# plai-group/latent-flexible-video-diffusion-modeling

Hardware: AMD Instinct MI355X
Metric: denoising steps/sec on 20-frame 4x16x16 latents (sampling; training reported alongside) (higher is better)
Workload: dtype f32

## Files before the change

include/lfvdm_hip.h:

```cpp
#ifndef LFVDM_HIP_H
#define LFVDM_HIP_H

#include <stddef.h>
#include <stdint.h>

#ifdef __cplusplus
extern "C" {
#endif

#define LFVDM_OK 0
#define LFVDM_E_SHAPE 1
#define LFVDM_E_LAUNCH 2
#define LFVDM_E_UNSUPPORTED 3

#define LFVDM_ACT_NONE 0
#define LFVDM_ACT_SILU 1

#define LFVDM_OUT_ROWS 0
#define LFVDM_OUT_NCHW 1

int lfvdm_abi_version(void);

typedef struct lfvdm_conv_args {
    const float* src0;
    const float* src1;
    int32_t C0, C1;
    int32_t N;
    int32_t Hs, Ws;
    int32_t up;
    int32_t stride;
    int32_t ksize;
    int32_t Ho, Wo;
    const float* coefA;
    const float* coefB;
    int32_t act;
    const float* W;
    const float* bias;
    int32_t Cout;
    const float* s2src0;
    const float* s2src1;
    int32_t s2C0, s2C1;
    const float* W2;
    const float* bias2;
    const float* res;
    int32_t ldr;
    const float* resA;
    const float* resB;
    float* out;
    int32_t ldo;
    int32_t out_mode;
    int32_t tune;
    float* splitk_ws;
    int32_t* splitk_cnt;
    int64_t splitk_ws_floats;
    int64_t splitk_cnt_ints;
    const float* gn_gamma;
    const float* gn_beta;
    const float* gn_film;
    float* gn_out;
    int32_t gn_film_ld;
    int32_t gn_film_div;
    int32_t gn_act;
    int32_t gn_skip_raw;
    float gn_eps;
    int32_t gn_general;
    int32_t gn_gw;
    int32_t gn_ld;
} lfvdm_conv_args;

int lfvdm_conv_igemm(const lfvdm_conv_args* a, void* stream);
int lfvdm_conv_igemm_config(const lfvdm_conv_args* a, int* nt, int* nwaves);
int lfvdm_conv_igemm_candidates(const lfvdm_conv_args* a, int* codes, int max_codes);

typedef struct lfvdm_wgrad_job {
    lfvdm_conv_args a;
    int32_t msplit;
    int32_t task0;
} lfvdm_wgrad_job;
int lfvdm_conv_wgrad_grouped(const lfvdm_wgrad_job* jobs_dev, int njobs, int total_tasks, void* stream);

int lfvdm_pack_conv_weight(const float* w_oihw, float* w_packed, int Cout, int Cin, int ksize, void* stream);
int lfvdm_pack_conv_weight_up2x(const float* w_oihw, float* w_packed, int Cout, int Cin, void* stream);

int lfvdm_conv_wgrad(const lfvdm_conv_args* a, void* stream);

int lfvdm_det_reduce(float* dst, const float* slab, long n, long parts, void* stream);
int lfvdm_pack_conv_weight_t(const float* w_oihw, float* w_packed_t, int Cout, int Cin, int ksize, void* stream);
int lfvdm_unpack_conv_grad(const float* g_packed, float* g_oihw, int Cout, int Cin, int ksize, int accumulate, void* stream);

typedef struct lfvdm_pack_job {
    const float* src;
    float* dst;
    int32_t Cout, Cin, taps, transposed, blk0;
    int32_t ld;
} lfvdm_pack_job;
int lfvdm_pack_conv_weights(const lfvdm_pack_job* jobs_dev, int njobs, int total_blocks, void* stream);

typedef struct lfvdm_unpack_job {
    float* gp;
    float* g;
    int32_t Cout, Cin, taps, row0;
    int32_t ldp;
    int32_t pad_;
} lfvdm_unpack_job;
int lfvdm_unpack_conv_grads(const lfvdm_unpack_job* jobs_dev, int njobs, int total_rows, int max_row_floats, void* stream);

int lfvdm_conv_in(const float* x, const float* x0, const float* obs, const float* w, const float* bias,
                  float* out, int N, int C, int H, int W, int Cout, void* stream);
int lfvdm_conv_in_tick(const float* x, const float* x0, const float* obs, const float* w, const float* bias, float* out,
                       int N, int C, int H, int W, int Cout, int64_t* t, const float* model_timestep_table, float* model_t,
                       int B, const float* rows_all, int rows_ld, float* rows, int row_floats, void* stream);

int lfvdm_gn_coef(const float* src0, const float* src1, int C0, int C1, int N, int P,
                  const float* gamma, const float* beta, const float* film, int film_div, int film_ld,
                  float eps, float* coefA, float* coefB, void* stream);

int lfvdm_gn_apply(const float* src0, const float* src1, int C0, int C1, int N, int P,
                   const float* gamma, const float* beta, const float* film, int film_div, int film_ld,
                   float eps, int act, float* out, float* coefA, float* coefB, float* stats, void* stream);
int lfvdm_gn_apply_part(const float* src, int C, int N, int P, int cg, const float* gamma, const float* beta, float eps, int act,
                        float* out, int ldo, void* stream);
long lfvdm_gn_apply_ws_floats(int C, int N, int P);
int lfvdm_gn_apply_ws(const float* src0, const float* src1, int C0, int C1, int N, int P, const float* gamma,
                      const float* beta, const float* film, int film_div, int film_ld, float eps, int act, float* out,
                      float* coefA, float* coefB, float* stats, float* ws, long ws_floats, void* stream);

int lfvdm_gn_coef_stats(const float* src0, const float* src1, int C0, int C1, int N, int P,
                        const float* gamma, const float* beta, const float* film, int film_div, int film_ld,
                        float eps, float* coefA, float* coefB, float* stats, void* stream);

int lfvdm_gn_bwd_stats(const float* da, const float* src0, const float* src1, int C0, int C1, int N, int P,
                       const float* coefA, const float* coefB, const float* stats, int act, float* sums, void* stream);
int lfvdm_gn_bwd_apply(const float* da, const float* src0, const float* src1, int C0, int C1, int N, int P,
                       const float* coefA, const float* coefB, const float* stats, const float* sums, int act,
                       float* out0, float* out1, int acc0, int acc1, void* stream);
int lfvdm_gn_bwd_apply_params(const float* da, const float* src0, const float* src1, int C0, int C1, int N, int P,
                              const float* coefA, const float* coefB, const float* stats, const float* sums, int act,
                              float* out0, float* out1, int acc0, int acc1, const float* gamma, const float* beta,
                              const float* film, int film_ld, int T, float* dgamma, float* dbeta, float* dfilm,
                              int dfilm_ld, const float* add, int add_ld, void* stream);
typedef struct lfvdm_gn_bwd_args {
    const float* da;
    const float* src0;
    const float* src1;
    const float* coefA;
    const float* coefB;
    const float* stats;
    float* out0;
    float* out1;
    const float* add;
    const float* add2;
    const float* gamma;
    const float* beta;
    const float* film;
    float* dgamma;
    float* dbeta;
    float* dfilm;
    float* sums_out;
    float* ws;
    int64_t ws_floats;
    int32_t C0, C1, N, P, act;
    int32_t add_ld, add2_ld, film_ld, T, dfilm_ld;
} lfvdm_gn_bwd_args;
long lfvdm_gn_bwd_ws_floats(int C, int N, int P);
int lfvdm_gn_bwd(const lfvdm_gn_bwd_args* a, void* stream);
int lfvdm_gn_param_grads(const float* sums, const float* gamma, const float* beta, const float* film, int film_ld, int T,
                         float* dgamma, float* dbeta, float* dfilm, int dfilm_ld, int N, int C, void* stream);
int lfvdm_gn_temporal_bwd(const float* x, const float* dy, const float* gamma, float eps, float* dx, float* dgamma,
                          float* dbeta, int B, int T, int P, int C, int accumulate, void* stream);
int lfvdm_gn_temporal_bwd_det(const float* x, const float* dy, const float* gamma, float eps, float* dx, float* dgamma,
                              float* dbeta, int B, int T, int P, int C, int accumulate, float* det_ws, int64_t det_ws_floats,
                              void* stream);

int lfvdm_gn_temporal(const float* x, const float* gamma, const float* beta, float eps, float* y,
                      int B, int T, int P, int C, void* stream);

int lfvdm_gn_temporal_qkv_ok(int B, int T, int P, int C);
int lfvdm_gn_temporal_qkv(const float* x, const float* gamma, const float* beta, float eps, float* xn_out,
                          const float* Wqkv, const float* bqkv, float* qkv, int B, int T, int P, int C, void* stream);

int lfvdm_proj_gn_ok(int N, int P, int C);
int lfvdm_proj_gn(const float* o, const float* W, const float* bias, const float* res, const float* gamma, const float* beta,
                  float eps, int act, float* out, float* raw_out, int N, int P, int C, void* stream);

typedef struct lfvdm_rowdot_job {
    const float* W;
    const float* b;
    const float* in;
    float* out;
    int32_t K, O, M, ldin, ldout, in_mode;
    int32_t row0;
    int32_t pad_;
} lfvdm_rowdot_job;

int lfvdm_rowdot(const lfvdm_rowdot_job* jobs_dev, int njobs, int total_rows, void* stream);
int lfvdm_silu(const float* in, float* out, int64_t n, void* stream);

typedef struct lfvdm_rowdot_bwd_job {
    const float* W;
    const float* in;
    const float* dout;
    float* dW;
    float* db;
    float* din;
    int32_t K, O, M, ldin, lddout, lddin, in_mode, task0;
} lfvdm_rowdot_bwd_job;
int lfvdm_rowdot_bwd(const lfvdm_rowdot_bwd_job* jobs_dev, int njobs, int total_tasks, void* stream);
int lfvdm_rowdot_bwd_det(const lfvdm_rowdot_bwd_job* jobs_dev, int njobs, int total_tasks, float* din_base, int64_t din_n,
                         float* det_ws, int64_t det_ws_floats, void* stream);

typedef struct lfvdm_rpe_job {
    const float* tproj;
    const float* Wd;
    const float* bd;
    const float* Wout;
    const float* bout;
    float* R;
    int32_t C;
    int32_t tile0;
    int32_t tproj_ld;
    int32_t pad_;
    float* act;
} lfvdm_rpe_job;

int lfvdm_rpe_nets(const lfvdm_rpe_job* jobs_dev, int njobs, int total_tiles, const int64_t* frame_indices_i64,
                   int B, int T, void* stream);
int lfvdm_rpe_nets_maxc(const lfvdm_rpe_job* jobs_dev, int njobs, int total_tiles, const int64_t* frame_indices_i64,
                        int B, int T, int max_channels, void* stream);

typedef struct lfvdm_rpe_bwd_job {
    const float* tproj;
    const float* Wd;
    const float* bd;
    const float* Wout_t;
    const float* dR;
    float* dtproj;
    float* dWd;
    float* dbd;
    int32_t C;
    int32_t tile0;
    int32_t tproj_ld;
    int32_t dtproj_ld;
} lfvdm_rpe_bwd_job;

int lfvdm_rpe_nets_bwd(const lfvdm_rpe_bwd_job* jobs_dev, int njobs, int total_tiles, const int64_t* frame_indices_i64,
                       int B, int T, void* stream);
int lfvdm_rpe_nets_bwd_det(const lfvdm_rpe_bwd_job* jobs_dev, int njobs, int total_tiles, const int64_t* frame_indices_i64,
                           int B, int T, float* det_ws, int64_t det_ws_floats, void* stream);

int lfvdm_rpe_front(const float* tproj, int tproj_ld, const float* feats, const float* Wd, const float* bd, float* act, int B,
                    int rows_per_b, int C, void* stream);
int lfvdm_rpe_front_bwd(const float* tproj, int tproj_ld, const float* feats, const float* Wd, const float* bd,
                        const float* d_act, float* dtproj, int dtproj_ld, float* dWd, float* dbd, int B, int rows_per_b,
                        int C, void* stream);

int lfvdm_attn_spatial(const float* qkv, float* o, float* attn_out, float* lse_out, int N, int P, int C, int heads,
                       void* stream);

int lfvdm_attn_spatial_fused_ok(int N, int P, int C, int heads);
int lfvdm_attn_spatial_fused(const float* xn, const float* Wqkv, const float* bqkv, float* o, int N, int P, int C, int heads,
                             void* stream);

int lfvdm_attn_spatial_bwd(const float* qkv, const float* o, const float* d_o, const float* lse, float* delta_ws,
                           float* dqkv, int N, int P, int C, int heads, void* stream);

int lfvdm_attn_temporal(const float* qkv, const float* Rq, const float* Rk, const float* Rv,
                        const float* mask , float* o, float* attn_out,
                        int B, int T, int P, int C, int heads, void* stream);
int lfvdm_attn_temporal_sel(const float* qkv, const float* Rq, const float* Rk, const float* Rv, const float* mask,
                            float* o, float* attn_out, int B, int T, int P, int C, int heads, const int64_t* rsel,
                            void* stream);
int lfvdm_attn_temporal_ring(const float* qkv, const float* Rq, const float* Rk, const float* Rv, const float* mask,
                             float* o, float* attn_out, int B, int T, int P, int C, int heads, const int64_t* rsel,
                             int ring, void* stream);

int lfvdm_attn_temporal_bwd(const float* qkv, const float* d_o, const float* Rq, const float* Rk, const float* Rv,
                            const float* mask, float* ws_p, float* ws_ds, float* dqkv, float* dRq, float* dRk,
                            float* dRv, int B, int T, int P, int C, int heads, void* stream);

int lfvdm_q_sample(const float* x0, const float* noise, const int64_t* t, const float* sqrt_acp,
                   const float* sqrt_1macp, float* out, int B, int inner, void* stream);
#define LFVDM_RULE_ANCESTRAL 0
#define LFVDM_RULE_DDIM 1
#define LFVDM_MEAN_EPS 0
#define LFVDM_MEAN_X0 1
int lfvdm_update_x0(const float* x, const float* model_out, const float* noise, const int64_t* t, const float* sqrt_recip_acp,
                    const float* sqrt_recipm1_acp, const float* c1, const float* c2, const float* sg, int rule, int mean_type,
                    int clip, float* sample, float* pred_xstart, float* mean_out, int B, int inner, void* stream);
int lfvdm_update_rng_x0(const float* x, const float* model_out, float* noise_out, const int64_t* t, const float* sqrt_recip_acp,
                        const float* sqrt_recipm1_acp, const float* c1, const float* c2, const float* sg, int rule,
                        int mean_type, int clip, float* sample, float* pred_xstart, float* mean_out, int B, int inner,
                        const int64_t* seed, void* stream);
int lfvdm_conv_out_psample_ok(int N, int H, int W, int C, int Cout);
int lfvdm_conv_out_update_x0(const float* act, const float* Wp, const float* bias, float* out, const float* x,
                             const float* noise_in, float* noise_out, const int64_t* t, const float* sqrt_recip_acp,
                             const float* sqrt_recipm1_acp, const float* c1, const float* c2, const float* sg, int rule,
                             int mean_type, int clip, float* sample, float* pred_xstart, float* mean_out, int B, int T, int H,
                             int W, int C, int Cout, const int64_t* seed, void* stream);
int lfvdm_update_ms_x0(const float* x, const float* model_out, const float* hist, const int64_t* t, const float* sqrt_recip_acp,
                       const float* sqrt_recipm1_acp, const float* k1, const float* k2, const float* k3, int mean_type, int clip,
                       float* sample, float* pred_xstart, int B, int inner, void* stream);
int lfvdm_conv_out_update_ms_x0(const float* act, const float* Wp, const float* bias, float* out, const float* x,
                                const float* hist, const int64_t* t, const float* sqrt_recip_acp, const float* sqrt_recipm1_acp,
                                const float* k1, const float* k2, const float* k3, int mean_type, int clip, float* sample,
                                float* pred_xstart, int B, int T, int H, int W, int C, int Cout, void* stream);
int lfvdm_known_blend(float* x, const float* known, const float* mask, const float* eps, float* noise_out, const int64_t* t,
                      const float* sqrt_acp_prev, const float* sqrt_1macp_prev, const int64_t* seed, int B, int T, int C,
                      int HW, void* stream);
int lfvdm_renoise(float* x, float* noise_out, const int64_t* t, const float* sqrt_1mbeta, const float* sqrt_beta,
                  const int64_t* seed, int B, int inner, void* stream);
int lfvdm_dyn_threshold_workspace(int B, int64_t inner, size_t* bytes);
int lfvdm_dyn_threshold(const float* x, const float* model_out, const int64_t* t, const float* sqrt_recip_acp,
                        const float* sqrt_recipm1_acp, int mean_type, int x0hat_fma, const float* frame_mask, int B, int T,
                        int64_t frame_inner, double percentile, float max_value, float* xhat, float* stats, void* workspace,
                        void* stream);
int lfvdm_noise_prior_factor(const int64_t* frame_indices, double a, double c, double rho, float* L_out, int B, int T,
                             void* stream);
int lfvdm_noise_prior_fill(const float* L, const float* xi, const int64_t* seed, const int64_t* t, float* out, int B, int T,
                           int64_t E, void* stream);
int lfvdm_sampler_tick(int64_t* t, const float* model_timestep_table, float* model_t, int B, void* stream);
int lfvdm_sampler_tick_fetch(int64_t* t, const float* model_timestep_table, float* model_t, int B, const float* rows_all,
                             int rows_ld, float* rows, int row_floats, void* stream);
int lfvdm_masked_mse(const float* a, const float* b, const float* mask, float* out, int B, int T,
                     int frame_inner, void* stream);
int lfvdm_masked_mse_bwd(const float* target, const float* pred, const float* mask, const float* g, float* dpred, int B, int T,
                         int frame_inner, void* stream);

int lfvdm_train_loss(const float* target, const float* pred, const float* mask, const float* eval_mask, const int64_t* t,
                     const float* wtab, int n_t, float* mse, float* eval_mse, float* loss, int B, int T, int frame_inner,
                     void* stream);
int lfvdm_train_loss_bwd(const float* target, const float* pred, const float* mask, const int64_t* t, const float* wtab, int n_t,
                         const float* g, float* dpred, int B, int T, int frame_inner, void* stream);

int lfvdm_vb_terms(const float* x_start, const float* x_t, const float* model_out, const float* noise, const int64_t* t,
                   const float* sqrt_recip_acp, const float* sqrt_recipm1_acp, const float* c1, const float* c2,
                   const float* post_log_var, const float* model_log_var, const float* mask, int mean_type, int clip, float* vb,
                   float* xstart_mse, float* eps_mse, float* pred_xstart, int B, int T, int frame_inner, int out_ld,
                   int col_base, void* stream);
int lfvdm_vb_terms_bwd(const float* x_start, const float* x_t, const float* model_out, const int64_t* t,
                       const float* sqrt_recip_acp, const float* sqrt_recipm1_acp, const float* c1, const float* c2,
                       const float* model_log_var, const float* mask, const float* g, int mean_type, int clip, float* d_out,
                       int B, int T, int frame_inner, void* stream);

#define LFVDM_PIX_F32 0
#define LFVDM_PIX_U8 1
int lfvdm_frame_metrics(const void* pred, const void* truth, int dtype, float scale, float shift, int K, int N, int C, int H,
                        int W, float* mse, float* ssim, float* partials, long partials_floats, void* stream);
long lfvdm_frame_metrics_workspace(int K, int N, int C, int H, int W);

int lfvdm_frame_dist_rows(const float* x, int B, int T, int C, int H, int W, int L, const int32_t* new_idx, int n_new,
                          const int32_t* cand_idx, int n_cand, float* dist, void* stream);
int lfvdm_fps_select(const float* dist, int B, int T, const int32_t* cand_idx, int n_cand, const int32_t* forced_pos, int n_forced,
                     int n, int32_t* picks, void* stream);

typedef struct lfvdm_adamw_args {
    float* p;
    const float* g;
    float* m;
    float* v;
    float* ema[4];
    float ema_rate[4];
    int32_t n_ema;
    int64_t n;
    float lr, beta1, beta2, eps, weight_decay;
    float bias_corr1, bias_corr2_sqrt;
    float grad_scale;
    float* grad_sqsum;
    const int32_t* skip_flag;
    const int32_t* skip_flag2;
} lfvdm_adamw_args;

int lfvdm_adamw_ema(const lfvdm_adamw_args* a, void* stream);

#define LFVDM_GRAD_NORM_MAX_PARTS 512
int lfvdm_grad_norm_nparts(int64_t n);
int lfvdm_grad_norm_partials(const float* g, int64_t n, float grad_scale, float* partials, int nparts, void* stream);
int lfvdm_grad_norm_finalize(const float* partials, int nparts, float max_norm, float* stat, void* stream);
int lfvdm_adamw_ema_clip(const lfvdm_adamw_args* a, const float* stat, void* stream);

int lfvdm_prepare_batch(const float* pool, const int32_t* table, float* batch, int64_t* frame_indices, float* obs_mask,
                        float* latent_mask, int B, int F, int Tp, int frame_elems, void* stream);

#define LFVDM_WAVELET_RANGE 0
#define LFVDM_WAVELET_ORTHONORMAL 1
int lfvdm_wavelet_encode(const void* pix, int dtype, float scale, float shift, float* coef, const float* mean,
                         const float* rstd, int N, int C, int H, int W, int levels, int norm, void* stream);
int lfvdm_wavelet_decode(const float* coef, const float* mean, const float* std, void* pix, int dtype, int N, int C, int H,
                         int W, int levels, int norm, void* stream);
int lfvdm_prepare_batch_wavelet(const void* pool, int dtype, float scale, float shift, const int32_t* table, float* batch,
                                int64_t* frame_indices, float* obs_mask, float* latent_mask, const float* mean,
                                const float* rstd, int B, int F, int Tp, int C, int H, int W, int levels, int norm,
                                void* stream);

int lfvdm_shapes_trajectories(const int64_t* video_idx, int32_t* traj, int32_t* consts, uint64_t seed, int split, int n_videos,
                              int T, int n_shapes, int H, int W, int stochastic, void* stream);
int lfvdm_shapes_render(const int32_t* traj, const int32_t* consts, const int32_t* table, const float* lut, void* out, int dtype,
                        int64_t* frame_indices, float* obs_mask, float* latent_mask, int B, int F, int Tp, int T, int n_shapes,
                        int H, int W, void* stream);

#define LFVDM_SLOT_PAD 0
#define LFVDM_SLOT_OBS 1
#define LFVDM_SLOT_LATENT 2
int lfvdm_search_assemble(const float* pool, const int32_t* table, const int32_t* role, float* x0, float* x_start,
                          float* obs_mask, float* latent_mask, float* mask, int64_t* frame_indices, int W, int K, int V, int Tv,
                          int frame_elems, void* stream);
int lfvdm_search_noise_qsample(const float* x_start, const int32_t* table, const int64_t* t_list, int32_t* ctl,
                               const int64_t* key, const float* sqrt_acp, const float* sqrt_1macp, float* noise, float* x_t,
                               int64_t* t_buf, int W, int K, int V, int frame_elems, void* stream);
int lfvdm_search_noise_fill(const int32_t* table, uint64_t seed, int step, int j, float* noise, int W, int K, int V,
                            int frame_elems, void* stream);
int lfvdm_search_scores(const float* terms, const int64_t* t_list, float* scores, int G, int V, int n_t, int ld, int col_base,
                        void* stream);

int lfvdm_compose_rows(const float* x, const float* x0, const float* obs, float* rows, int N, int Cx, int H, int W, int ld,
                       void* stream);

#define LFVDM_CHAIN_CONV 0
#define LFVDM_CHAIN_GN 1
#define LFVDM_CHAIN_LOCAL 2
#define LFVDM_CHAIN_MAX_DEPS 64
#define LFVDM_CHAIN_CTL_EPOCH 0
#define LFVDM_CHAIN_CTL_EXIT 32
#define LFVDM_CHAIN_CTL_ABORT 64
#define LFVDM_CHAIN_CTL_INTS 96

typedef struct lfvdm_gn_args {
    const float* src0;
    const float* src1;
    int32_t C0, C1, N, P;
    const float* gamma;
    const float* beta;
    const float* film;
    int32_t film_div, film_ld;
    float eps;
    int32_t act;
    float* out;
    int32_t cg;
    int32_t ldo;
    float* out_base;
    int32_t out_col;
    int32_t pad_;
} lfvdm_gn_args;

typedef struct lfvdm_chain_stage {
    int32_t kind;
    int32_t n_items;
    int32_t flag_base;
    int32_t n_flags;
    int32_t dep_base;
    int32_t dep_stride;
    int32_t cfg;
    int32_t kz;
    int32_t nt2;
    int32_t wg_off;
    int32_t side;
    int32_t wg_lo;
    int32_t wg_count;
    int64_t ws_off;
    int64_t cnt_off;
    lfvdm_conv_args conv;
    lfvdm_gn_args gn;
} lfvdm_chain_stage;

int lfvdm_chain_plan(lfvdm_chain_stage* stages, int n_stages, int32_t* deps, int64_t deps_cap, int64_t* deps_used,
                     int32_t* n_flags, int64_t* ws_floats, int64_t* cnt_ints, int32_t* grid, int32_t* lds_bytes);
int lfvdm_chain_conv_ok(const lfvdm_conv_args* a);
int lfvdm_chain_gn_ok(int C0, int C1, int N, int P);
int lfvdm_chain_local_ok(const lfvdm_conv_args* a, int row_tiles);
int lfvdm_chain_capacity(int lds_bytes);
int lfvdm_level_chain(const lfvdm_chain_stage* stages_dev, int n_stages, const int32_t* deps_dev, int32_t* flags, int32_t* ctl,
                      int grid, int lds_bytes, double timeout_s, void* stream);

int lfvdm_flag_add(int32_t* flag, void* stream);
int lfvdm_flag_wait(const int32_t* flag, int32_t target, double timeout_s, int32_t* timed_out, void* stream);
int lfvdm_flag_wait2(const int32_t* flag, int32_t target, double timeout_s, int32_t* timed_out, float* timed_out_f32, void* stream);

#ifdef __cplusplus
}
#endif
#endif
```

latent-flexible-video-diffusion-modeling_amd/csrc/attention_temporal.h:

```cpp
#pragma once
#include "common_hip.h"

constexpr int TEMPORAL_MAXT = 32;
constexpr int TEMPORAL_MAXT_LONG = 64;

struct TemporalFwd {
    const float *qkv, *Rq, *Rk, *Rv, *mask;
    float *o, *attn_out;
    int B, T, P, C, heads;
    RSel rsel;
    hipStream_t s;
};
struct TemporalBwd {
    const float *qkv, *d_o, *Rq, *Rk, *Rv, *mask;
    float *ws_p, *ws_ds, *dqkv;
    int B, T, P, C, heads;
    hipStream_t s;
};

int lfvdm_attn_temporal2_try(const TemporalFwd& a);
int lfvdm_attn_temporal2_bwd_rows_try(const TemporalBwd& a);
int lfvdm_attn_temporal_long(const TemporalFwd& a);
int lfvdm_attn_temporal_long_bwd(const TemporalBwd& a);
```

latent-flexible-video-diffusion-modeling_amd/csrc/attention_temporal2.hip:

```cpp
#include "attention_temporal.h"
#include "common_hip.h"

namespace {

struct T2Geom {
    int T, P, C, heads, B;
    int TG, TGN, PPW, NW;
    int strips;
    int NL, HL, XPG;
};

template <int F, int TCAP>
struct T2Cfg {
    static constexpr int NQ = F / 4;
    static constexpr int RS = (TCAP * NQ + 15) / 16 * 16;
};

__device__ __forceinline__ void t2_decode(const T2Geom& g, int& b, int& h, int& tg, int& strip) {
    {
        const int id = blockIdx.x;
        if (g.XPG > 0) {
            const int x = id & 7, r = id >> 3;
            const int grp = x % g.NL, sub = x / g.NL;
            const int inner = r % (g.HL * g.TG), sblk = r / (g.HL * g.TG);
            strip = sblk * g.XPG + sub;
            const int hl = inner % g.HL;
            tg = inner / g.HL;
            const int hpb = g.heads / g.HL;
            b = grp / hpb;
            h = (grp % hpb) * g.HL + hl;
        } else {
            const int NP = g.B * g.heads;
            const int pair = id % NP, rest = id / NP;
            b = pair / g.heads;
            h = pair % g.heads;
            tg = rest % g.TG;
            strip = rest / g.TG;
        }
    }
}

template <int F, int TCAP>
__device__ __forceinline__ void t2_stage(const float* __restrict__ qkv, const float* __restrict__ Rq, const float* __restrict__ Rk,
                                         const float* __restrict__ Rv, RSel rsel, const T2Geom& g, int b, int h,
                                         int tq0, int p0, int wave, int lane, float* Rimg, float* KVimg) {
    using CF = T2Cfg<F, TCAP>;
    constexpr int NQ = CF::NQ, RS = CF::RS;
    const int T = g.T, P = g.P, C = g.C;
    const int NPX = g.NW * g.PPW;
    const float invRS = 1.0f / (float)RS;
    {
        const size_t rb = rsel.slice(b, g.B);
        const float* Rsrc[3] = {Rk + rb * T * T * C + h * F, Rq + rb * T * T * C + h * F, Rv + rb * T * T * C + h * F};
        const float* kvsrc = qkv + (size_t)b * T * P * 3 * C + C + h * F;
        const int vpx = min(NPX, P - p0);
        const int nR = (min(g.TGN, T - tq0) * 3 * RS + 63) >> 6, nKV = (vpx * 2 * RS + 63) >> 6;
        const int TNQ = T * NQ;
        auto dma = [](const float* src, float* dst) {
            __builtin_amdgcn_global_load_lds((const __attribute__((address_space(1))) void*)src,
                                             (__attribute__((address_space(3))) void*)dst, 16, 0, 0);
        };
        for (int pc = wave; pc < nR; pc += g.NW) {
            const int ps = pc * 64 + lane;
            const int row3 = (int)(((float)ps + 0.5f) * invRS);
            const int w = ps - row3 * RS;
            const int tq = (int)(((float)row3 + 0.5f) * (1.0f / 3.0f)), arr = row3 - 3 * tq;
            const int c = w ^ (tq & 15);
            const int s = c / NQ, u = c - s * NQ;
            const int t = tq0 + tq;
            const bool ok = tq < g.TGN && t < T && c < TNQ;
            const int row = arr == 1 ? s * T + t : t * T + s;
            const float* base = arr == 0 ? Rsrc[0] : (arr == 1 ? Rsrc[1] : Rsrc[2]);
            dma(ok ? base + (size_t)row * C + 4 * u : qkv, Rimg + (size_t)pc * 256);
        }
        for (int pc = wave; pc < nKV; pc += g.NW) {
            const int ps = pc * 64 + lane;
            const int row2 = (int)(((float)ps + 0.5f) * invRS);
            const int w = ps - row2 * RS;
            const int jw = row2 >> 1, arr = row2 & 1;
            const int c = w ^ (jw & 15);
            const int s = c / NQ, u = c - s * NQ;
            const int p = p0 + jw;
            const bool ok = jw < NPX && p < P && c < TNQ;
            dma(ok ? kvsrc + ((size_t)s * P + p) * 3 * C + arr * C + 4 * u : qkv, KVimg + (size_t)pc * 256);
        }
    }

}

template <int F, int TCAP>
__global__ __launch_bounds__(256, 3)
void attn_temporal2_kernel(const float* __restrict__ qkv, const float* __restrict__ Rq, const float* __restrict__ Rk,
                           const float* __restrict__ Rv, const float* __restrict__ mask, float* __restrict__ o,
                           float* __restrict__ attn_out, RSel rsel, T2Geom g) {
    using CF = T2Cfg<F, TCAP>;
    constexpr int NQ = CF::NQ, RS = CF::RS;
    extern __shared__ __attribute__((aligned(16))) float t2_smem[];
    const int T = g.T, P = g.P, C = g.C;
    const int tid = threadIdx.x, lane = tid & 63;
    const int wave = __builtin_amdgcn_readfirstlane(tid >> 6);
    const int NPX = g.NW * g.PPW;
    int b, h, tg, strip;
    t2_decode(g, b, h, tg, strip);
    if (strip >= g.strips) return;
    const int tq0 = tg * g.TGN;
    const int p0 = strip * NPX;
    float* Rimg = t2_smem;
    float* KVimg = t2_smem + (size_t)((g.TGN * 3 * RS + 63) & ~63) * 4;
    const float invRS = 1.0f / (float)RS;

    t2_stage<F, TCAP>(qkv, Rq, Rk, Rv, rsel, g, b, h, tq0, p0, wave, lane, Rimg, KVimg);

    const float invN = 1.0f / (float)g.TGN;
    const int sq = lane & 3, pair = lane >> 2;
    const int j = (int)(((float)pair + 0.5f) * invN), tq = pair - j * g.TGN;
    const int jw = wave * g.PPW + j;
    const int t = tq0 + tq, p = p0 + jw;
    const bool active = j < g.PPW && p < P && t < T;
    const float scale = rsqrtf((float)F);
    const size_t ld = (size_t)3 * C;
    const float* qrow = active ? qkv + ((size_t)(b * T + t) * P + p) * ld + h * F : qkv;
    f32x4 q4[NQ];
#pragma unroll
    for (int u = 0; u < NQ; ++u) q4[u] = ld4(qrow + 4 * u) * scale;
    constexpr int KQ = (TCAP + 3) / 4;
    constexpr int ISTRIDE = 4 * NQ * 4;
    int kb[NQ], rbs[NQ];
    {
        const int jr = active ? jw : 0, tr = active ? tq : 0;
#pragma unroll
        for (int u = 0; u < NQ; ++u) {
            const int low = (NQ * sq + u) & 15, high = (NQ * sq + u) & ~15;
            kb[u] = (jr * 2 * RS + high + (low ^ (jr & 15))) * 4;
            rbs[u] = (tr * 3 * RS + high + (low ^ (tr & 15))) * 4;
        }
    }
    asm volatile("s_waitcnt vmcnt(0)" ::: "memory");
    __syncthreads();

    auto quad_x1 = [](float v) { return __builtin_bit_cast(float, __builtin_amdgcn_mov_dpp(__builtin_bit_cast(int, v), 0xB1, 0xF, 0xF, true)); };
    auto quad_x2 = [](float v) { return __builtin_bit_cast(float, __builtin_amdgcn_mov_dpp(__builtin_bit_cast(int, v), 0x4E, 0xF, 0xF, true)); };

    {
        float logit[KQ];
#pragma unroll
        for (int i = 0; i < KQ; ++i) {
            f32x2 a0 = {0.f, 0.f}, a1 = {0.f, 0.f};
#pragma unroll
            for (int u = 0; u < NQ; ++u) {
                const f32x4 k4 = ld4(KVimg + kb[u] + i * ISTRIDE);
                const f32x4 r4 = ld4(Rimg + rbs[u] + i * ISTRIDE);
                const f32x4 g4 = ld4(Rimg + rbs[u] + RS * 4 + i * ISTRIDE);
                a0 = __builtin_elementwise_fma(q4[u].xy, k4.xy + r4.xy, a0);
                a0 = __builtin_elementwise_fma(q4[u].zw, k4.zw + r4.zw, a0);
                a1 = __builtin_elementwise_fma(k4.xy, g4.xy, a1);
                a1 = __builtin_elementwise_fma(k4.zw, g4.zw, a1);
            }
            logit[i] = (a0.x + a0.y) + (a1.x + a1.y) * scale;
            asm volatile("" : "+v"(logit[i]) : : "memory");
            __builtin_amdgcn_sched_barrier(0);
        }
        const int tm = active ? t : 0;
        const float mt = mask ? mask[b * T + tm] : 1.f;
        float mx = -INFINITY;
#pragma unroll
        for (int i = 0; i < KQ; ++i) {
            const int sk = sq + 4 * i;
            float v = -INFINITY;
            if (sk < T) {
                v = logit[i];
                if (mask) {
                    const float ms = mask[b * T + sk];
                    const float pen = 1.f - (mt * ms + (1.f - mt) * (1.f - ms));
                    v -= (pen == 1.f) ? INFINITY : pen;
                }
            }
            logit[i] = v;
            mx = fmaxf(mx, v);
        }
        mx = fmaxf(mx, quad_x1(mx));
        mx = fmaxf(mx, quad_x2(mx));
        float sum = 0.f;
#pragma unroll
        for (int i = 0; i < KQ; ++i) {
            const float e = (logit[i] == -INFINITY) ? 0.f : __expf(logit[i] - mx);
            logit[i] = e;
            sum += e;
        }
        sum += quad_x1(sum);
        sum += quad_x2(sum);
        const float inv = 1.0f / sum;
#pragma unroll
        for (int i = 0; i < KQ; ++i) logit[i] *= inv;
        if (attn_out && active) {
            float* ar = attn_out + ((((size_t)b * P + p) * g.heads + h) * T + t) * T;
#pragma unroll
            for (int i = 0; i < KQ; ++i)
                if (sq + 4 * i < T) ar[sq + 4 * i] = logit[i];
        }
        f32x4 acc[NQ];
#pragma unroll
        for (int u = 0; u < NQ; ++u) acc[u] = (f32x4){0.f, 0.f, 0.f, 0.f};
#pragma unroll
        for (int i = 0; i < KQ; ++i) {
            const f32x2 pr = {logit[i], logit[i]};
#pragma unroll
            for (int u = 0; u < NQ; ++u) {
                const f32x4 v4 = ld4(KVimg + kb[u] + RS * 4 + i * ISTRIDE);
                const f32x4 r4 = ld4(Rimg + rbs[u] + 2 * RS * 4 + i * ISTRIDE);
                f32x2 lo = acc[u].xy, hi = acc[u].zw;
                lo = __builtin_elementwise_fma(pr, v4.xy + r4.xy, lo);
                hi = __builtin_elementwise_fma(pr, v4.zw + r4.zw, hi);
                acc[u] = (f32x4){lo.x, lo.y, hi.x, hi.y};
                asm volatile("" : "+v"(acc[u]) : : "memory");
            }
            __builtin_amdgcn_sched_barrier(0);
        }
#pragma unroll
        for (int u = 0; u < NQ; ++u) {
#pragma unroll
            for (int e = 0; e < 4; ++e) {
                float v = acc[u][e];
                v += quad_x1(v);
                v += quad_x2(v);
                acc[u][e] = v;
            }
        }
        if (active) {
            float* orow = o + ((size_t)(b * T + t) * P + p) * C + h * F;
#pragma unroll
            for (int u = 0; u < NQ; ++u)
                if ((u & 3) == sq) st4(orow + 4 * u, acc[u]);
        }
    }
}

template <int F, int TCAP>
__global__ __launch_bounds__(256, 2)
void attn_temporal2_bwd_rows_kernel(const float* __restrict__ qkv, const float* __restrict__ dO, const float* __restrict__ Rq,
                                    const float* __restrict__ Rk, const float* __restrict__ Rv, const float* __restrict__ mask,
                                    float* __restrict__ dqkv, float* __restrict__ Pg, float* __restrict__ dSg, T2Geom g) {
    using CF = T2Cfg<F, TCAP>;
    constexpr int NQ = CF::NQ, RS = CF::RS;
    extern __shared__ __attribute__((aligned(16))) float t2_smem[];
    const int T = g.T, P = g.P, C = g.C;
    const int tid = threadIdx.x, lane = tid & 63;
    const int wave = __builtin_amdgcn_readfirstlane(tid >> 6);
    const int NPX = g.NW * g.PPW;
    int b, h, tg, strip;
    t2_decode(g, b, h, tg, strip);
    if (strip >= g.strips) return;
    const int tq0 = tg * g.TGN;
    const int p0 = strip * NPX;
    float* Rimg = t2_smem;
    float* KVimg = t2_smem + (size_t)((g.TGN * 3 * RS + 63) & ~63) * 4;
    t2_stage<F, TCAP>(qkv, Rq, Rk, Rv, RSel{nullptr, 0}, g, b, h, tq0, p0, wave, lane, Rimg, KVimg);

    const float invN = 1.0f / (float)g.TGN;
    const int sq = lane & 3, pair = lane >> 2;
    const int j = (int)(((float)pair + 0.5f) * invN), tq = pair - j * g.TGN;
    const int jw = wave * g.PPW + j;
    const int t = tq0 + tq, p = p0 + jw;
    const bool active = j < g.PPW && p < P && t < T;
    const float scale = rsqrtf((float)F);
    const size_t ld = (size_t)3 * C;
    const size_t tok = active ? (size_t)(b * T + t) * P + p : 0;
    const float* qrow = qkv + tok * ld + h * F;
    const float* dorow = dO + tok * C + h * F;
    f32x4 q4[NQ];
#pragma unroll
    for (int u = 0; u < NQ; ++u) q4[u] = ld4(qrow + 4 * u) * scale;
    constexpr int KQ = (TCAP + 3) / 4;
    constexpr int ISTRIDE = 4 * NQ * 4;
    int kb[NQ], rbs[NQ];
    {
        const int jr = active ? jw : 0, tr = active ? tq : 0;
#pragma unroll
        for (int u = 0; u < NQ; ++u) {
            const int low = (NQ * sq + u) & 15, high = (NQ * sq + u) & ~15;
            kb[u] = (jr * 2 * RS + high + (low ^ (jr & 15))) * 4;
            rbs[u] = (tr * 3 * RS + high + (low ^ (tr & 15))) * 4;
        }
    }
    asm volatile("s_waitcnt vmcnt(0)" ::: "memory");
    __syncthreads();

    auto quad_x1 = [](float v) { return __builtin_bit_cast(float, __builtin_amdgcn_mov_dpp(__builtin_bit_cast(int, v), 0xB1, 0xF, 0xF, true)); };
    auto quad_x2 = [](float v) { return __builtin_bit_cast(float, __builtin_amdgcn_mov_dpp(__builtin_bit_cast(int, v), 0x4E, 0xF, 0xF, true)); };

    float pr[KQ];
#pragma unroll
    for (int i = 0; i < KQ; ++i) {
        f32x2 a0 = {0.f, 0.f}, a1 = {0.f, 0.f};
#pragma unroll
        for (int u = 0; u < NQ; ++u) {
            const f32x4 k4 = ld4(KVimg + kb[u] + i * ISTRIDE);
            const f32x4 r4 = ld4(Rimg + rbs[u] + i * ISTRIDE);
            const f32x4 g4 = ld4(Rimg + rbs[u] + RS * 4 + i * ISTRIDE);
            a0 = __builtin_elementwise_fma(q4[u].xy, k4.xy + r4.xy, a0);
            a0 = __builtin_elementwise_fma(q4[u].zw, k4.zw + r4.zw, a0);
            a1 = __builtin_elementwise_fma(k4.xy, g4.xy, a1);
            a1 = __builtin_elementwise_fma(k4.zw, g4.zw, a1);
        }
        pr[i] = (a0.x + a0.y) + (a1.x + a1.y) * scale;
        asm volatile("" : "+v"(pr[i]) : : "memory");
        __builtin_amdgcn_sched_barrier(0);
    }
    {
        const int tm = active ? t : 0;
        const float mt = mask ? mask[b * T + tm] : 1.f;
        float mx = -INFINITY;
#pragma unroll
        for (int i = 0; i < KQ; ++i) {
            const int sk = sq + 4 * i;
            float v = -INFINITY;
            if (sk < T) {
                v = pr[i];
                if (mask) {
                    const float ms = mask[b * T + sk];
                    const float pen = 1.f - (mt * ms + (1.f - mt) * (1.f - ms));
                    v -= (pen == 1.f) ? INFINITY : pen;
                }
            }
            pr[i] = v;
            mx = fmaxf(mx, v);
        }
        mx = fmaxf(mx, quad_x1(mx));
        mx = fmaxf(mx, quad_x2(mx));
        float sum = 0.f;
#pragma unroll
        for (int i = 0; i < KQ; ++i) {
            const float e = (pr[i] == -INFINITY) ? 0.f : __expf(pr[i] - mx);
            pr[i] = e;
            sum += e;
        }
        sum += quad_x1(sum);
        sum += quad_x2(sum);
        const float inv = 1.0f / sum;
#pragma unroll
        for (int i = 0; i < KQ; ++i) pr[i] *= inv;
    }
    f32x4 d4[NQ];
#pragma unroll
    for (int u = 0; u < NQ; ++u) d4[u] = ld4(dorow + 4 * u);
    float dp[KQ];
#pragma unroll
    for (int i = 0; i < KQ; ++i) {
        f32x2 a0 = {0.f, 0.f};
#pragma unroll
        for (int u = 0; u < NQ; ++u) {
            const f32x4 v4 = ld4(KVimg + kb[u] + RS * 4 + i * ISTRIDE);
            const f32x4 r4 = ld4(Rimg + rbs[u] + 2 * RS * 4 + i * ISTRIDE);
            a0 = __builtin_elementwise_fma(d4[u].xy, v4.xy + r4.xy, a0);
            a0 = __builtin_elementwise_fma(d4[u].zw, v4.zw + r4.zw, a0);
        }
        dp[i] = a0.x + a0.y;
        asm volatile("" : "+v"(dp[i]) : : "memory");
        __builtin_amdgcn_sched_barrier(0);
    }
    float dsum = 0.f;
#pragma unroll
    for (int i = 0; i < KQ; ++i) dsum += pr[i] * dp[i];
    dsum += quad_x1(dsum);
    dsum += quad_x2(dsum);
    {
        const size_t wid = ((size_t)b * P + (active ? p : 0)) * g.heads + h;
        float* prow = Pg + (wid * T + (active ? t : 0)) * T;
        float* srow = dSg + (wid * T + (active ? t : 0)) * T;
#pragma unroll
        for (int i = 0; i < KQ; ++i) {
            dp[i] = pr[i] * (dp[i] - dsum);
            if (active && sq + 4 * i < T) {
                prow[sq + 4 * i] = pr[i];
                srow[sq + 4 * i] = dp[i];
            }
        }
    }
    f32x4 acc[NQ];
#pragma unroll
    for (int u = 0; u < NQ; ++u) acc[u] = (f32x4){0.f, 0.f, 0.f, 0.f};
#pragma unroll
    for (int i = 0; i < KQ; ++i) {
        const f32x2 w = {dp[i], dp[i]};
#pragma unroll
        for (int u = 0; u < NQ; ++u) {
            const f32x4 k4 = ld4(KVimg + kb[u] + i * ISTRIDE);
            const f32x4 r4 = ld4(Rimg + rbs[u] + i * ISTRIDE);
            f32x2 lo = acc[u].xy, hi = acc[u].zw;
            lo = __builtin_elementwise_fma(w, k4.xy + r4.xy, lo);
            hi = __builtin_elementwise_fma(w, k4.zw + r4.zw, hi);
            acc[u] = (f32x4){lo.x, lo.y, hi.x, hi.y};
            asm volatile("" : "+v"(acc[u]) : : "memory");
        }
        __builtin_amdgcn_sched_barrier(0);
    }
#pragma unroll
    for (int u = 0; u < NQ; ++u) {
#pragma unroll
        for (int e = 0; e < 4; ++e) {
            float v = acc[u][e];
            v += quad_x1(v);
            v += quad_x2(v);
            acc[u][e] = v * scale;
        }
    }
    if (active) {
        float* orow = dqkv + tok * ld + h * F;
#pragma unroll
        for (int u = 0; u < NQ; ++u)
            if ((u & 3) == sq) st4(orow + 4 * u, acc[u]);
    }
}

inline size_t t2_lds_bytes(int TGN, int NPX, int RS) {
    return ((size_t)((TGN * 3 * RS + 63) & ~63) + (size_t)((NPX * 2 * RS + 63) & ~63)) * 16;
}

inline unsigned t2_geometry(T2Geom& g, int F, int RS, size_t& lds) {
    const int B = g.B, T = g.T, P = g.P, heads = g.heads;
    int best_tg = (T + 4) / 5, best_nw = 0;
    {
        const int TGN = (T + best_tg - 1) / best_tg, PPW = 16 / TGN;
        for (int NW = 4; NW >= 1 && best_nw == 0; NW /= 2)
            if (t2_lds_bytes(TGN, NW * PPW, RS) <= 160 * 1024) best_nw = NW;
        if (best_nw == 0) best_tg = 0;
    }
    if (best_tg == 0) return 0;
    g.TG = best_tg; g.NW = best_nw;
    g.TGN = (T + g.TG - 1) / g.TG;
    g.PPW = 16 / g.TGN;
    const int NPX = g.NW * g.PPW;
    g.strips = (P + NPX - 1) / NPX;
    lds = t2_lds_bytes(g.TGN, NPX, RS);
    g.HL = F >= 32 ? 1 : 32 / F;
    if (g.HL > heads || heads % g.HL) g.HL = 1;
    g.NL = B * (heads / g.HL);
    g.XPG = (g.NL <= 8 && 8 % g.NL == 0) ? 8 / g.NL : 0;
    if (g.XPG > 0) {
        const int sblks = (g.strips + g.XPG - 1) / g.XPG;
        return 8u * (unsigned)(g.HL * g.TG) * (unsigned)sblks;
    }
    return (unsigned)(B * heads) * (unsigned)g.TG * (unsigned)g.strips;
}

template <int F, int TCAP>
int launch_t2(const TemporalFwd& a) {
    T2Geom g = {a.T, a.P, a.C, a.heads, a.B};
    size_t lds;
    const unsigned grid = t2_geometry(g, F, T2Cfg<F, TCAP>::RS, lds);
    if (!grid) return LFVDM_E_UNSUPPORTED;
    static DynLdsLimit limit;
    if (int rc = limit.ensure(reinterpret_cast<const void*>(&attn_temporal2_kernel<F, TCAP>), lds)) return rc;
    hipLaunchKernelGGL((attn_temporal2_kernel<F, TCAP>), dim3(grid), dim3(64 * g.NW), lds, a.s, a.qkv, a.Rq, a.Rk, a.Rv, a.mask, a.o,
                       a.attn_out, a.rsel, g);
    LFVDM_CHECK_LAUNCH();
    return LFVDM_OK;
}

template <int F, int TCAP>
int launch_t2(const TemporalBwd& a) {
    T2Geom g = {a.T, a.P, a.C, a.heads, a.B};
    size_t lds;
    const unsigned grid = t2_geometry(g, F, T2Cfg<F, TCAP>::RS, lds);
    if (!grid) return LFVDM_E_UNSUPPORTED;
    static DynLdsLimit limit;
    if (int rc = limit.ensure(reinterpret_cast<const void*>(&attn_temporal2_bwd_rows_kernel<F, TCAP>), lds)) return rc;
    hipLaunchKernelGGL((attn_temporal2_bwd_rows_kernel<F, TCAP>), dim3(grid), dim3(64 * g.NW), lds, a.s, a.qkv, a.d_o, a.Rq, a.Rk,
                       a.Rv, a.mask, a.dqkv, a.ws_p, a.ws_ds, g);
    LFVDM_CHECK_LAUNCH();
    return LFVDM_OK;
}

template <int F, class Args>
int launch_t2_t(const Args& a) {
    if (a.T <= 8) return launch_t2<F, 8>(a);
    if (a.T <= 16) return launch_t2<F, 16>(a);
    if (a.T <= 20) return launch_t2<F, 20>(a);
    if (a.T <= 24) return launch_t2<F, 24>(a);
    return launch_t2<F, 32>(a);
}

template <class Args>
int launch_t2_f(const Args& a) {
    const int F = a.C / a.heads;
    if (F == 16) return launch_t2_t<16>(a);
    if (F == 32) return launch_t2_t<32>(a);
    if (F == 64) return launch_t2_t<64>(a);
    return LFVDM_E_UNSUPPORTED;
}

}

int lfvdm_attn_temporal2_try(const TemporalFwd& a) {
    if ((long)a.B * a.P * (a.C / a.heads) >= 16384) return LFVDM_E_UNSUPPORTED;
    return launch_t2_f(a);
}

int lfvdm_attn_temporal2_bwd_rows_try(const TemporalBwd& a) {
    if (a.T > TEMPORAL_MAXT) return LFVDM_E_UNSUPPORTED;
    return launch_t2_f(a);
}
```

latent-flexible-video-diffusion-modeling_amd/csrc/gn_temporal_qkv.hip:

```cpp
#include <cstdlib>
#include <type_traits>

#include "common_hip.h"

namespace {

constexpr int TQ_TF = 3;

struct TqGeom {
    int B, T, P;
    int NSPLIT, NCT;
    int ngroups;
};

template <int C_>
struct TqCfg {
    static constexpr int SPR = C_ / 4;
    static constexpr int NSL = SPR > 32 ? SPR / 32 : 1;
    static constexpr int PX = 32 * NSL / SPR;
    static constexpr int RT = (PX * 24 + 15) / 16;
    static constexpr int KG = C_ / 16;
    static constexpr int CG = C_ / 32;
};

__device__ __forceinline__ float tq_dpp_b1(float v) { return __builtin_bit_cast(float, __builtin_amdgcn_mov_dpp(__builtin_bit_cast(int, v), 0xB1, 0xF, 0xF, true)); }
__device__ __forceinline__ float tq_dpp_4e(float v) { return __builtin_bit_cast(float, __builtin_amdgcn_mov_dpp(__builtin_bit_cast(int, v), 0x4E, 0xF, 0xF, true)); }
__device__ __forceinline__ float tq_dpp_hm(float v) { return __builtin_bit_cast(float, __builtin_amdgcn_mov_dpp(__builtin_bit_cast(int, v), 0x141, 0xF, 0xF, true)); }
__device__ __forceinline__ float tq_dpp_r8(float v) { return __builtin_bit_cast(float, __builtin_amdgcn_mov_dpp(__builtin_bit_cast(int, v), 0x128, 0xF, 0xF, true)); }

template <int CG>
__device__ __forceinline__ float tq_reduce(float v) {
    v += tq_dpp_b1(v);
    v += tq_dpp_4e(v);
    v += tq_dpp_hm(v);
    if constexpr (CG == 8) v += tq_dpp_r8(v);
    return v;
}

template <int CG>
__device__ __forceinline__ f32x4 tq_group(f32x4 s) {
    if constexpr (CG == 2) {
        const float a = tq_reduce<CG>(s.x + s.y), b = tq_reduce<CG>(s.z + s.w);
        return (f32x4){a, a, b, b};
    } else {
        const float a = tq_reduce<CG>((s.x + s.y) + (s.z + s.w));
        return (f32x4){a, a, a, a};
    }
}

template <int C_>
__global__ __launch_bounds__(256) void gn_temporal_qkv_kernel(const float* __restrict__ x, const float* __restrict__ gamma,
                                                              const float* __restrict__ beta, float eps,
                                                              float* __restrict__ xn_out, const float* __restrict__ W,
                                                              const float* __restrict__ bias, float* __restrict__ qkv,
                                                              TqGeom g) {
    using CF = TqCfg<C_>;
    constexpr int SPR = CF::SPR, NSL = CF::NSL, PX = CF::PX, RT = CF::RT, KG = CF::KG, CG = CF::CG;
    __shared__ __attribute__((aligned(16))) float As[RT * 16 * C_];
    const int id = blockIdx.x;
    const int xcd = id & 7, r8 = id >> 3;
    const int grp = (r8 / g.NSPLIT) * 8 + xcd, sp = r8 % g.NSPLIT;
    if (grp >= g.ngroups) return;
    const int T = g.T, P = g.P;
    const int col0 = grp * PX;
    const int b = col0 / P, p0 = col0 - b * P;
    const int tid = threadIdx.x, lane = tid & 63;
    const int wave = __builtin_amdgcn_readfirstlane(tid >> 6);
    const int lq = lane & 15, kk = lane >> 4;

    const int tp = tid & 7, rest = tid >> 3;
    f32x4 xk[NSL][TQ_TF];
#pragma unroll
    for (int sl = 0; sl < NSL; ++sl) {
        const int s = rest + 32 * sl;
        const int quad = s % SPR, pix = s / SPR;
#pragma unroll
        for (int i = 0; i < TQ_TF; ++i) {
            const int t = tp + 8 * i;
            xk[sl][i] = t < T ? ld4(x + ((size_t)(b * T + t) * P + p0 + pix) * C_ + 4 * quad) : (f32x4){0.f, 0.f, 0.f, 0.f};
        }
    }
    const int NCT = g.NCT;
    auto wrow = [&](int ct) -> const float* { return W + (size_t)((sp * NCT + ct) * 16 + lq) * C_ + 4 * kk; };
    f32x4 wf[KG];
    {
        const float* wr = wrow(wave);
#pragma unroll
        for (int k = 0; k < KG; ++k) wf[k] = ld4(wr + 16 * k);
    }
    f32x4 gam[NSL], bet[NSL];
#pragma unroll
    for (int sl = 0; sl < NSL; ++sl) {
        const int quad = (rest + 32 * sl) % SPR;
        gam[sl] = ld4(gamma + 4 * quad);
        bet[sl] = ld4(beta + 4 * quad);
    }
    const float inv = 1.0f / (float)(CG * T);
#pragma unroll
    for (int sl = 0; sl < NSL; ++sl) {
        const int s = rest + 32 * sl;
        const int quad = s % SPR, pix = s / SPR;
        f32x4 a = {0.f, 0.f, 0.f, 0.f};
#pragma unroll
        for (int i = 0; i < TQ_TF; ++i) a += xk[sl][i];
        const f32x4 mu = tq_group<CG>(a) * inv;
        f32x4 q = {0.f, 0.f, 0.f, 0.f};
#pragma unroll
        for (int i = 0; i < TQ_TF; ++i) {
            if (tp + 8 * i < T) {
                const f32x4 d = xk[sl][i] - mu;
                q += d * d;
            }
        }
        const f32x4 var = tq_group<CG>(q) * inv;
        f32x4 rs;
        rs.x = 1.0f / sqrtf(var.x + eps);
        rs.z = CG == 2 ? 1.0f / sqrtf(var.z + eps) : rs.x;
        rs.y = rs.x;
        rs.w = rs.z;
#pragma unroll
        for (int i = 0; i < TQ_TF; ++i) {
            const int t = tp + 8 * i;
            if (t < T) {
                const f32x4 v = (xk[sl][i] - mu) * rs * gam[sl] + bet[sl];
                const int row = pix * T + t;
                st4(As + ((size_t)row * SPR + ((quad & ~15) | ((quad ^ row) & 15))) * 4, v);
                if (sp == 0 && xn_out != nullptr) st4(xn_out + ((size_t)(b * T + t) * P + p0 + pix) * C_ + 4 * quad, v);
            }
        }
    }
    __syncthreads();

    const int rows = PX * T;
    for (int ct = wave; ct < NCT; ct += 4) {
        f32x4 wn[KG];
        const bool more = ct + 4 < NCT;
        if (more) {
            const float* wr = wrow(ct + 4);
#pragma unroll
            for (int k = 0; k < KG; ++k) wn[k] = ld4(wr + 16 * k);
        }
        const int colq = (sp * NCT + ct) * 16 + 4 * kk;
        const f32x4 bv = ld4(bias + colq);
        f32x4 acc[RT];
#pragma unroll
        for (int rt = 0; rt < RT; ++rt) acc[rt] = (f32x4){0.f, 0.f, 0.f, 0.f};
#pragma unroll
        for (int k = 0; k < KG; ++k) {
            f32x4 a4[RT];
            const int s = 4 * k + kk;
#pragma unroll
            for (int rt = 0; rt < RT; ++rt) {
                const int row = 16 * rt + lq;
                a4[rt] = ld4(As + ((size_t)row * SPR + ((s & ~15) | ((s ^ row) & 15))) * 4);
            }
#pragma unroll
            for (int e = 0; e < 4; ++e)
#pragma unroll
                for (int rt = 0; rt < RT; ++rt) acc[rt] = __builtin_amdgcn_mfma_f32_16x16x4f32(wf[k][e], a4[rt][e], acc[rt], 0, 0, 0);
        }
#pragma unroll
        for (int rt = 0; rt < RT; ++rt) {
            const int row = 16 * rt + lq;
            if (row < rows) {
                const int pix = (PX > 1 && row >= T) ? 1 : 0;
                const int t = row - pix * T;
                st4(qkv + ((size_t)(b * T + t) * P + p0 + pix) * (3 * C_) + colq, acc[rt] + bv);
            }
        }
        if (more) {
#pragma unroll
            for (int k = 0; k < KG; ++k) wf[k] = wn[k];
        }
    }
}

int tq_split(int C, long ngroups, int& nct) {
    const int tiles = 3 * C / 16;
    int best = 1;
    static const int force = getenv("LFVDM_TQ_SPLIT") ? atoi(getenv("LFVDM_TQ_SPLIT")) : 0;
    for (int ns : {1, 2, 3, 6, 12}) {
        if (tiles % ns || (tiles / ns) % 4) continue;
        best = ns;
        if (force ? ns >= force : ngroups * ns >= 256) break;
    }
    nct = tiles / best;
    return best;
}

}

extern "C" int lfvdm_gn_temporal_qkv_ok(int B, int T, int P, int C) {
    if (B <= 0 || T <= 0 || P <= 0 || C <= 0) return LFVDM_E_SHAPE;
    if (C != 64 && C != 128 && C != 256) return LFVDM_E_UNSUPPORTED;
    const int PX = C == 64 ? 2 : 1;
    if (T > 24 || P % PX) return LFVDM_E_UNSUPPORTED;
    if ((long)B * T * P * 3 * C * 4 >= (1L << 31)) return LFVDM_E_UNSUPPORTED;
    const bool always = [] { const char* e = getenv("LFVDM_TQ_ALWAYS"); return e && e[0] == '1'; }();
    if (C != 64 && !always && 2.0 * B * T * P * 3.0 * C * C > 0.5e9) return LFVDM_E_UNSUPPORTED;
    return LFVDM_OK;
}

extern "C" int lfvdm_gn_temporal_qkv(const float* x, const float* gamma, const float* beta, float eps, float* xn_out,
                                     const float* Wqkv, const float* bqkv, float* qkv, int B, int T, int P, int C, void* stream) {
    if (!x || !gamma || !beta || !Wqkv || !bqkv || !qkv || x == xn_out) return LFVDM_E_SHAPE;
    if (B <= 0 || T <= 0 || P <= 0) return LFVDM_E_SHAPE;
    if (C != 64 && C != 128 && C != 256) return LFVDM_E_UNSUPPORTED;
    const int PX = C == 64 ? 2 : 1;
    if (T > 24 || P % PX || (long)B * T * P * 3 * C * 4 >= (1L << 31)) return LFVDM_E_UNSUPPORTED;
    TqGeom g;
    g.B = B; g.T = T; g.P = P;
    g.ngroups = B * P / PX;
    g.NSPLIT = tq_split(C, g.ngroups, g.NCT);
    const unsigned grid = 8u * (unsigned)((g.ngroups + 7) / 8) * (unsigned)g.NSPLIT;
    hipStream_t s = (hipStream_t)stream;
    if (C == 64) hipLaunchKernelGGL(gn_temporal_qkv_kernel<64>, dim3(grid), dim3(256), 0, s, x, gamma, beta, eps, xn_out, Wqkv, bqkv, qkv, g);
    else if (C == 128) hipLaunchKernelGGL(gn_temporal_qkv_kernel<128>, dim3(grid), dim3(256), 0, s, x, gamma, beta, eps, xn_out, Wqkv, bqkv, qkv, g);
    else hipLaunchKernelGGL(gn_temporal_qkv_kernel<256>, dim3(grid), dim3(256), 0, s, x, gamma, beta, eps, xn_out, Wqkv, bqkv, qkv, g);
    LFVDM_CHECK_LAUNCH();
    return LFVDM_OK;
}
```

latent-flexible-video-diffusion-modeling_amd/improved_diffusion/_engine.py:

```python
import ctypes as C
import json
import os
import sys
import weakref

import torch as th
import torch.nn as nn

from . import _chains, _native as nat
from ._chains import CHAIN_MAX_M, CHAIN_TIMEOUT_S, chain_local_enabled, level_chain_enabled
from .nn import timestep_freqs


def _p(t):
    return t.data_ptr()


def update_args(tables, ddim=None, predict_xstart=False):
    if ddim is not None and "k3" in ddim:
        c1, c2, sg, rule = ddim["k1"], ddim["k2"], ddim["k3"], nat.RULE_DPMPP2M
    elif ddim is not None:
        c1, c2, sg, rule = ddim["k1"], ddim["k2"], ddim["sigma"], nat.RULE_DDIM
    else:
        c1, c2, sg = tables["posterior_mean_coef1"], tables["posterior_mean_coef2"], tables["model_log_variance"]
        rule = nat.RULE_ANCESTRAL
    if predict_xstart:
        return None, None, c1, c2, sg, rule, nat.MEAN_X0
    return tables["sqrt_recip_alphas_cumprod"], tables["sqrt_recipm1_alphas_cumprod"], c1, c2, sg, rule, nat.MEAN_EPS


SPATIAL_FUSED = os.environ.get("LFVDM_SPATIAL_FUSED", "1") != "0"
PROJ_GN = os.environ.get("LFVDM_PROJ_GN", "1") != "0"
TEMPORAL_QKV = os.environ.get("LFVDM_TEMPORAL_QKV", "1") != "0"
GN_EPILOGUE = os.environ.get("LFVDM_GN_EPILOGUE", "1") != "0"
NEXT_GN_EPILOGUE = os.environ.get("LFVDM_NEXT_GN_EPILOGUE", "1") != "0"
MAX_FRAMES = 64


class _TableBudget:

    def __init__(self):
        self._held = {}
        self._logged = set()

    def limit(self):
        return float(os.environ.get("LFVDM_TIME_TABLE_GB", "12")) * 2 ** 30

    def used(self):
        return sum(self._held.values())

    def remaining(self):
        return max(0.0, self.limit() - self.used())

    def reserve(self, plan, nbytes):
        if nbytes > self.remaining():
            import gc
            gc.collect()
        if nbytes > self.remaining():
            return False
        key = id(plan)
        self._held[key] = nbytes
        weakref.finalize(plan, self._held.pop, key, None)
        return True

    def log(self, msg):
        if os.environ.get("LFVDM_QUIET", "0") != "1" and msg not in self._logged:
            self._logged.add(msg)
            print("[lfvdm] " + msg, file=sys.stderr, flush=True)


_table_budget = _TableBudget()


class Plan:

    def __init__(self, engine, B, T, H, W, want_attn, time_steps=None):
        self.time_steps = int(time_steps) if time_steps else 0
        self.engine = engine
        self.model = engine.model
        self.B, self.T, self.H, self.W = B, T, H, W
        self.want_attn = want_attn
        self.dev = next(self.model.parameters()).device
        self.keep = []
        self.steps = []
        self.packs = []
        self.attn_t, self.attn_s = [], []
        self.chains = []
        self.chains_off = False
        self.skip_side = []
        self.part_bases = {}
        self._build()

    def buf(self, *shape, dtype=th.float32):
        t = th.empty(*shape, device=self.dev, dtype=dtype)
        self.keep.append(t)
        return t

    def scratch(self, key, rows, cols):
        if level_chain_enabled() and rows <= CHAIN_MAX_M:
            return self.buf(rows * cols).view(rows, cols)
        pool = self.__dict__.setdefault("_scratch", {})
        t = pool.get(key)
        if t is None or t.numel() < rows * cols:
            t = pool[key] = self.buf(rows * cols)
        return t[:rows * cols].view(rows, cols)

    def gn_apply(self, a, b, C0, C1, N, P, gn, film, act, key):
        out = self.scratch(key, N * P, C0 + C1)
        fkw = dict(film=_p(film), film_div=self.T, film_ld=self.rows_ld) if film is not None else {}
        fn, args = nat.gn_fwd_call(lambda need: _p(self.scratch("gn_ws", 1, need)), src0=_p(a), C0=C0, C1=C1, N=N, P=P,
                                   src1=_p(b) if b is not None else None, gamma=_p(gn.weight), beta=_p(gn.bias), eps=gn.eps,
                                   act=act, out=_p(out), **fkw)
        self.add(fn, *args)
        return out

    def packed(self, weight, c0=0, c1=None):
        Cout, Cin, k, _ = weight.shape
        c1 = Cin if c1 is None else c1
        out = self.buf(Cout, k * k, c1 - c0)
        self.packs.append((weight, out) if (c0, c1) == (0, Cin) else (weight, out, c0, c1))
        return out

    def packed_up2x(self, weight):
        Cout, Cin, k, _ = weight.shape
        assert k == 3
        out = self.buf(4, Cout, 4, Cin)
        self.packs.append((weight, out, "up2x"))
        return out

    def add(self, fn, *args):
        self.steps.append((fn, args))

    def add_conv(self, **kw):
        self.add_conv_args(self.conv_args(**kw))

    def add_conv_args(self, a):
        self.keep.append(a)
        self.add(nat.lib().lfvdm_conv_igemm, C.byref(a))

    def conv_fused_gn(self, **kw):
        if not GN_EPILOGUE:
            return False
        a = self.conv_args(**kw)
        nt, nw = C.c_int(), C.c_int()
        if nat.lib().lfvdm_conv_igemm_config(C.byref(a), C.byref(nt), C.byref(nw)) != 0:
            return False
        self.add_conv_args(a)
        return True

    def conv_args(self, **kw):
        a = nat.ConvArgs()
        g = kw.get
        a.src0 = _p(kw["src0"]); a.src1 = _p(g("src1")) if g("src1") is not None else None
        a.C0 = kw["C0"]; a.C1 = g("C1", 0); a.N = kw["N"]; a.Hs = kw["Hs"]; a.Ws = kw["Ws"]
        a.up = g("up", 0); a.stride = g("stride", 1); a.ksize = g("ksize", 3); a.Ho = kw["Ho"]; a.Wo = kw["Wo"]
        a.coefA = _p(g("coefA")) if g("coefA") is not None else None
        a.coefB = _p(g("coefB")) if g("coefB") is not None else None
        a.act = g("act", nat.ACT_NONE)
        a.W = _p(kw["W"]); a.bias = _p(g("bias")) if g("bias") is not None else None; a.Cout = kw["Cout"]
        a.s2src0 = _p(g("s2src0")) if g("s2src0") is not None else None
        a.s2src1 = _p(g("s2src1")) if g("s2src1") is not None else None
        a.s2C0 = g("s2C0", 0); a.s2C1 = g("s2C1", 0)
        a.W2 = _p(g("W2")) if g("W2") is not None else None
        a.bias2 = _p(g("bias2")) if g("bias2") is not None else None
        a.res = _p(g("res")) if g("res") is not None else None
        a.ldr = g("ldr", kw["Cout"])
        a.resA = _p(g("resA")) if g("resA") is not None else None
        a.resB = _p(g("resB")) if g("resB") is not None else None
        a.out = _p(kw["out"]); a.ldo = kw["ldo"]; a.out_mode = g("out_mode", nat.OUT_ROWS)
        if g("gn_out") is not None:
            gn, film = kw["gn"], g("gn_film")
            a.gn_gamma, a.gn_beta, a.gn_out = _p(gn.weight), _p(gn.bias), _p(kw["gn_out"])
            a.gn_film = _p(film) if film is not None else None
            a.gn_film_ld = self.rows_ld if film is not None else 0
            a.gn_film_div = self.T if film is not None else 1
            a.gn_act, a.gn_skip_raw, a.gn_eps = g("gn_act", nat.ACT_NONE), int(g("gn_skip_raw", 0)), gn.eps
            a.gn_gw, a.gn_ld = int(g("gn_gw", 0)), int(g("gn_ld", 0))
        if getattr(self, "splitk_ws", None) is None:
            self.splitk_ws = self.buf(2 * 1024 * 1024)
            self.splitk_cnt = self.buf(4096, dtype=th.int32).zero_()
        a.splitk_ws, a.splitk_cnt = _p(self.splitk_ws), _p(self.splitk_cnt)
        a.splitk_ws_floats, a.splitk_cnt_ints = self.splitk_ws.numel(), self.splitk_cnt.numel()
        return a

    def _build(self):
        m, L = self.model, nat.lib()
        B, T, H, W = self.B, self.T, self.H, self.W
        N = B * T
        if T > MAX_FRAMES:
            raise RuntimeError(f"native temporal attention supports at most {MAX_FRAMES} frames per window (got {T}); "
                               f"use --max_frames {MAX_FRAMES} or less")
        if m.dims != 2:
            raise NotImplementedError("only dims=2 is on the native path (the reference scripts use 2)")
        if not m.use_scale_shift_norm:
            raise NotImplementedError("use_scale_shift_norm=False is not on the native path (default True)")
        ch = m.model_channels
        ted = 4 * ch
        Cx = m.in_channels - 1

        self.x_in = self.buf(B, T, Cx, H, W)
        self.x0_in = self.buf(B, T, Cx, H, W)
        self.obs = self.buf(N)
        self.mask = self.buf(B, T)
        self.fi = self.buf(B, T, dtype=th.int64)
        half = ch // 2
        self.Bpad = (B + 3) // 4 * 4
        self.tin = self.buf(self.Bpad + half)
        self.tin.zero_()
        self.tin[self.Bpad:] = timestep_freqs(ch).to(self.dev)

        from .unet import ResBlock, FactorizedAttentionBlock
        e0, self.emb = self.buf(B, ted), self.buf(B, ted)
        te0, te2 = m.time_embed[0], m.time_embed[2]
        heads = []
        for mod in m.modules():
            if isinstance(mod, ResBlock):
                heads.append((mod, mod.emb_layers[1], 1))
        self.film_floats = sum(lin.weight.shape[0] for _, lin, _ in heads)
        for mod in m.modules():
            if isinstance(mod, FactorizedAttentionBlock):
                ta = mod.temporal_attention
                for r in (ta.rpe_q, ta.rpe_k, ta.rpe_v):
                    heads.append((r, r.rpe_net.embed_diffusion_time, 0))
        self.rows_ld = sum(lin.weight.shape[0] for _, lin, _ in heads)
        assert self.film_floats % 4 == 0 and self.rows_ld % 4 == 0
        self.rows = self.buf(B, self.rows_ld)
        self.film, self.tproj, self.row_off = {}, {}, {}
        off = 0
        for key, lin, mode in heads:
            O = lin.weight.shape[0]
            (self.film if mode == 1 else self.tproj)[key] = self.rows[:, off:off + O]
            self.row_off[key] = off
            off += O
        self._heads = heads

        def emb_jobs(M, tin, ldin, e0_, emb_, rows_, se0_=None, semb_=None):
            j0 = [nat.RowdotJob(_p(te0.weight), _p(te0.bias), _p(tin), _p(e0_), ch, ted, M, ldin, ted, 2, 0, 0)]
            j1 = [nat.RowdotJob(_p(te2.weight), _p(te2.bias), _p(se0_ if se0_ is not None else e0_), _p(emb_), ted, ted, M, ted, ted,
                                0 if se0_ is not None else 1, 0, 0)]
            jg, row0 = [], 0
            for key, lin, mode in heads:
                O = lin.weight.shape[0]
                src, md = (semb_, 0) if (mode == 1 and semb_ is not None) else (emb_, mode)
                jg.append(nat.RowdotJob(_p(lin.weight), _p(lin.bias), _p(src), _p(rows_) + 4 * self.row_off[key], ted, O, M, ted,
                                        self.rows_ld, md, row0, 0))
                row0 += O
            return [nat.jobs_to_device(j, self.dev) for j in (j0, j1, jg)], len(jg), row0

        self._emb_jobs = emb_jobs

        def rpe_jobs(Bn, tproj_base, R_of):
            jobs, tile0 = [], 0
            tiles_per = (Bn * T * T + 31) // 32
            for mod in m.modules():
                if isinstance(mod, FactorizedAttentionBlock):
                    ta = mod.temporal_attention
                    for r in (ta.rpe_q, ta.rpe_k, ta.rpe_v):
                        net = r.rpe_net
                        jobs.append(nat.RpeJob(_p(tproj_base) + 4 * self.row_off[r], _p(net.embed_distances.weight),
                                               _p(net.embed_distances.bias), _p(net.out.weight), _p(net.out.bias), _p(R_of[r]),
                                               net.channels, tile0, self.rows_ld, 0, None))
                        tile0 += tiles_per
            return (nat.jobs_to_device(jobs, self.dev) if jobs else None), len(jobs), tile0

        self._rpe_jobs = rpe_jobs
        rpe_mods = [r for mod in m.modules() if isinstance(mod, FactorizedAttentionBlock)
                    for r in (mod.temporal_attention.rpe_q, mod.temporal_attention.rpe_k, mod.temporal_attention.rpe_v)]
        for r in rpe_mods:
            if r.rpe_net.channels > 512:
                raise RuntimeError("RPE nets support at most 512 channels natively")

        self._time_params = [te0.weight, te0.bias, te2.weight, te2.bias] + [t for _, lin, _ in heads for t in (lin.weight, lin.bias)]
        for r in rpe_mods:
            net = r.rpe_net
            self._time_params += [net.embed_distances.weight, net.embed_distances.bias, net.out.weight, net.out.bias]

        self.t_sel = None
        self.time_table_bytes = 0
        self.time_table_fallback = None
        self.time_ring = 0
        if self.time_steps:
            ring = int(os.environ.get("LFVDM_TIME_RING", "128")) // 16 * 16
            if 0 < ring < self.time_steps:
                self.time_ring = ring
            Bv = self.time_steps * B
            table_bytes = 4 * B * (self.time_steps * self.rows_ld +
                                   (self.time_ring or self.time_steps) * T * T * sum(r.rpe_net.channels for r in rpe_mods))
            if os.environ.get("LFVDM_TIME_TABLES", "1") == "0":
                self.time_table_fallback = "disabled (LFVDM_TIME_TABLES=0)"
            elif B > 64:
                self.time_table_fallback = "batch > 64"
            elif not _table_budget.reserve(self, table_bytes):
                self.time_table_fallback = (f"{table_bytes / 2 ** 30:.1f} GiB of tables do not fit the remaining "
                                            f"{_table_budget.remaining() / 2 ** 30:.1f} GiB of LFVDM_TIME_TABLE_GB")
            if self.time_table_fallback:
                self.time_steps = 0
                _table_budget.log(f"timestep tables off for plan (B={B}, T={T}, {H}x{W}): {self.time_table_fallback}; "
                                  "+4 launches per step")
            else:
                self.time_table_bytes = table_bytes
                _table_budget.log(f"timestep tables on for plan (B={B}, T={T}, {H}x{W}): {table_bytes / 2 ** 30:.2f} GiB "
                                  f"({_table_budget.used() / 2 ** 30:.2f} of {_table_budget.limit() / 2 ** 30:.1f} GiB in use)")
        self.R = {}
        if self.time_steps:
            Bv = self.time_steps * B
            self.t_sel = self.buf(B, dtype=th.int64).zero_()
            self.rows_all = self.buf(Bv, self.rows_ld)
            for r in rpe_mods:
                self.R[r] = self.buf((self.time_ring or self.time_steps) * B, T, T, r.rpe_net.channels)
            self.tables_sig = None
            self._fill_jobs = {}
            self._loaded = {}
            self._fi_rep = None
        else:
            (j0, j1, jg), n_g, rows_g = emb_jobs(B, self.tin, self.Bpad, e0, self.emb, self.rows)
            self.keep += [j0, j1, jg]
            self.add(L.lfvdm_rowdot, _p(j0), 1, ted)
            self.add(L.lfvdm_rowdot, _p(j1), 1, ted)
            self.add(L.lfvdm_rowdot, _p(jg), n_g, rows_g)
            for r in rpe_mods:
                self.R[r] = self.buf(B, T, T, r.rpe_net.channels)
            jr, n_r, tiles_r = rpe_jobs(B, self.rows, self.R)
            if jr is not None:
                self.keep.append(jr)
                self.add(L.lfvdm_rpe_nets_maxc, _p(jr), n_r, tiles_r, _p(self.fi), B, T, max(r.rpe_net.channels for r in rpe_mods))

        maxC = max(mod.channels for mod in m.modules() if isinstance(mod, FactorizedAttentionBlock))
        maxCin = max(mod.channels for mod in m.modules() if isinstance(mod, ResBlock))
        Mmax = N * H * W
        self.s_qkv = self.buf(Mmax * 3 * maxC)
        self.s_o = self.buf(Mmax * maxC)
        self.s_xn = self.buf(Mmax * maxC)

        conv0 = m.input_blocks[0][0]
        conv_in_lds = (Cx + 1) * 9 * (ch + 4) * 4
        if conv_in_lds > 64 * 1024:
            raise NotImplementedError(
                f"the native input convolution holds (in_channels + 1) * 9 * (model_channels + 4) floats in 64 KiB of LDS; "
                f"in_channels={Cx} with model_channels={ch} needs {conv_in_lds} bytes.  A two-level wavelet space on RGB "
                "(48 channels) is over that limit: use wavelet_levels=1 (12 channels, up to 128 filters)")
        h0 = self.buf(N * H * W, ch)
        self.add(L.lfvdm_conv_in, _p(self.x_in), _p(self.x0_in), _p(self.obs), _p(conv0.weight), _p(conv0.bias), _p(h0),
                 N, Cx, H, W, ch)
        cur = dict(parts=[(h0, ch)], H=H, W=W)
        hs = [cur]
        stages = list(m.input_blocks)[1:] + [m.middle_block]
        outs = list(m.output_blocks)
        for i, blk in enumerate(stages):
            nxt = stages[i + 1][0] if i + 1 < len(stages) else None
            if blk is m.middle_block:
                cur = self._stage(blk, cur, after_cat=(outs[0][0], hs[-1]) if outs else None)
            else:
                cur = self._stage(blk, cur, after=nxt)
                hs.append(dict(parts=cur["parts"], H=cur["H"], W=cur["W"]))
        for i, blk in enumerate(outs):
            skip = hs.pop()
            assert skip["H"] == cur["H"] and len(cur["parts"]) == 1 and len(skip["parts"]) == 1
            cat_act = cur.get("act1cat")
            nxt_cat = (outs[i + 1][0], hs[-1]) if i + 1 < len(outs) and hs else None
            last_blk = i + 1 == len(outs)
            cur = self._stage(blk, dict(parts=cur["parts"] + skip["parts"], H=cur["H"], W=cur["W"],
                                        **({"act1": cat_act} if cat_act is not None else {})), after_cat=nxt_cat,
                              after_gn=m.out[0] if last_blk and NEXT_GN_EPILOGUE else None)
            if not last_blk:
                cur.pop("act1", None)
        (hb, hc), = cur["parts"]
        gn, conv = m.out[0], m.out[2]
        self.out = self.buf(B, T, m.out_channels, H, W)
        act = cur.get("act1")
        if act is None:
            act = self.gn_apply(hb, None, hc, 0, N, H * W, gn, None, nat.ACT_SILU, "act1")
        wp = self.packed(conv.weight)
        self.add_conv(src0=act, C0=hc, N=N, Hs=H, Ws=W, Ho=H, Wo=W, W=wp, bias=conv.bias,
                      Cout=m.out_channels, out=self.out, ldo=m.out_channels, out_mode=nat.OUT_NCHW)
        self.head = dict(act=act, Wp=wp, bias=conv.bias, C=hc, Cout=m.out_channels, step=len(self.steps) - 1)
        self.head_fused = False

    def _stage(self, blk, cur, after=None, after_cat=None, after_gn=None):
        from .unet import ResBlock, FactorizedAttentionBlock, Downsample, Upsample
        layers = list(blk)
        for i, layer in enumerate(layers):
            last = i + 1 == len(layers)
            nxt = layers[i + 1] if not last else after
            ngn = nxt.in_layers[0] if (isinstance(nxt, ResBlock) and NEXT_GN_EPILOGUE) else None
            if last and after_gn is not None:
                ngn = after_gn
            self._cat_next = None
            if last and after_cat is not None and isinstance(after_cat[0], ResBlock) and NEXT_GN_EPILOGUE:
                self._cat_next = after_cat
            if isinstance(layer, ResBlock):
                cur = self._res(layer, cur, ngn)
            elif isinstance(layer, FactorizedAttentionBlock):
                cur = self._attn(layer, cur, ngn)
            elif isinstance(layer, Downsample):
                cur = self._resample(layer.op, cur, True, ngn)
            elif isinstance(layer, Upsample):
                cur = self._resample(layer.conv, cur, False, None)
            else:
                raise NotImplementedError(type(layer))
        self._cat_next = None
        return cur

    def _final_conv(self, kw, next_gn, M):
        if next_gn is not None and next_gn.weight.shape[0] == kw["Cout"]:
            actn = self.scratch("actn", M, kw["Cout"])
            if self.conv_fused_gn(gn=next_gn, gn_out=actn, gn_act=nat.ACT_SILU, gn_skip_raw=0, **kw):
                return actn
            P = kw["Ho"] * kw["Wo"]
            if (PROJ_GN and kw.get("ksize") == 1 and kw.get("res") is not None and kw.get("ldr") == kw["Cout"]
                    and kw.get("ldo") == kw["Cout"] and kw["C0"] == kw["Cout"] and not kw.get("src1") and not kw.get("s2src0")
                    and kw["Hs"] * kw["Ws"] == P and nat.lib().lfvdm_proj_gn_ok(kw["N"], P, kw["Cout"]) == 0):
                self.add(nat.lib().lfvdm_proj_gn, _p(kw["src0"]), _p(kw["W"]), _p(kw["bias"]), _p(kw["res"]), _p(next_gn.weight),
                         _p(next_gn.bias), next_gn.eps, nat.ACT_SILU, _p(actn), _p(kw["out"]), kw["N"], P, kw["Cout"])
                return actn
        cat = getattr(self, "_cat_next", None)
        if cat is not None and self._final_conv_cat(kw, cat, M):
            return None
        self.add_conv(**kw)
        return None

    def _final_conv_cat(self, kw, cat, M):
        rb, skip = cat
        (sb, C1), = skip["parts"]
        C0, L = kw["Cout"], nat.lib()
        N, P = kw["N"], kw["Ho"] * kw["Wo"]
        Ccat = C0 + C1
        gw = Ccat // 32
        gn = rb.in_layers[0]
        if (not level_chain_enabled() or M > CHAIN_MAX_M or gn.weight.shape[0] != Ccat or Ccat % 32 or C0 % gw or C1 % gw
                or gw not in (2, 4, 8, 16) or C1 % 64 or P > 256 or skip["H"] * skip["W"] != P):
            return False
        if self._cat_split_ok(rb, C0, C1, N, kw["Ho"], kw["Wo"]):
            actL, actR = self.buf(M, C0), self.buf(M, C1)
            a = self.conv_args(gn=gn, gn_out=actL, gn_act=nat.ACT_SILU, gn_skip_raw=0, gn_gw=gw, gn_ld=C0, **kw)
            nt, nw = C.c_int(), C.c_int()
            if GN_EPILOGUE and L.lfvdm_conv_igemm_config(C.byref(a), C.byref(nt), C.byref(nw)) == 0:
                self.part_bases[_p(actR)] = (_p(actR), 0)
                self.add(L.lfvdm_gn_apply_part, _p(sb), C1, N, P, gw, _p(gn.weight) + 4 * C0, _p(gn.bias) + 4 * C0, gn.eps,
                         nat.ACT_SILU, _p(actR), C1)
                self.skip_side.append((self.steps[-1], _p(sb)))
                self.add_conv_args(a)
                self._cat_done = (actL, actR)
                return True
        act = self.buf(M, Ccat)
        a = self.conv_args(gn=gn, gn_out=act, gn_act=nat.ACT_SILU, gn_skip_raw=0, gn_gw=gw, gn_ld=Ccat, **kw)
        nt, nw = C.c_int(), C.c_int()
        if not GN_EPILOGUE or L.lfvdm_conv_igemm_config(C.byref(a), C.byref(nt), C.byref(nw)) != 0:
            return False
        out_ptr = _p(act) + 4 * C0
        self.part_bases[out_ptr] = (_p(act), C0)
        self.add(L.lfvdm_gn_apply_part, _p(sb), C1, N, P, gw, _p(gn.weight) + 4 * C0, _p(gn.bias) + 4 * C0, gn.eps, nat.ACT_SILU,
                 out_ptr, Ccat)
        self.add_conv_args(a)
        self._cat_done = act
        return True

    def _cat_split_ok(self, rb, C0, C1, N, H, W):
        if not (chain_local_enabled() and level_chain_enabled()) or os.environ.get("LFVDM_CAT_SPLIT", "1") == "0":
            return False
        L = nat.lib()

        def ok(Cin):
            a = nat.ConvArgs()
            a.src0, a.W, a.out = 0x1000, 0x1000, 0x1000
            a.C0, a.N, a.Hs, a.Ws, a.Ho, a.Wo, a.stride, a.ksize, a.Cout, a.ldo, a.ldr = Cin, N, H, W, H, W, 1, 3, rb.out_channels, rb.out_channels, rb.out_channels
            a.out_mode = nat.OUT_ROWS
            return any(L.lfvdm_chain_local_ok(C.byref(a), rt) == 0 for rt in (1, 2))

        return N * H * W <= CHAIN_MAX_M and not ok(C0 + C1) and ok(C0) and ok(C1)

    def _res(self, rb, cur, next_gn=None):
        L = nat.lib()
        N, H, W = self.B * self.T, cur["H"], cur["W"]
        P = H * W
        parts = cur["parts"]
        (a, C0) = parts[0]
        (b, C1) = parts[1] if len(parts) > 1 else (None, 0)
        Cin, Cout = C0 + C1, rb.out_channels
        assert Cin == rb.channels
        if rb.use_conv:
            raise NotImplementedError("ResBlock(use_conv=True) skip is not used by the reference factory")
        gn1, conv1 = rb.in_layers[0], rb.in_layers[2]
        gn2, conv2 = rb.out_layers[0], rb.out_layers[3]
        pb = _p(b) if b is not None else None
        h1 = self.buf(N * P, Cout)
        film = self.film[rb]
        out = self.buf(N * P, Cout)
        act1 = cur.get("act1")
        if act1 is None:
            act1 = self.gn_apply(a, b, C0, C1, N, P, gn1, None, nat.ACT_SILU, "act1")
        if isinstance(act1, tuple):
            actL, actR = act1
            part = self.buf(N * P, Cout)
            self.add_conv(src0=actR, C0=C1, N=N, Hs=H, Ws=W, Ho=H, Wo=W, W=self.packed(conv1.weight, C0, C0 + C1), Cout=Cout,
                          out=part, ldo=Cout)
            self.skip_side.append((self.steps[-1], _p(actR)))
            c1 = dict(src0=actL, C0=C0, N=N, Hs=H, Ws=W, Ho=H, Wo=W, W=self.packed(conv1.weight, 0, C0), bias=conv1.bias,
                      Cout=Cout, out=h1, ldo=Cout, res=part, ldr=Cout)
        else:
            c1 = dict(src0=act1, C0=Cin, N=N, Hs=H, Ws=W, Ho=H, Wo=W, W=self.packed(conv1.weight), bias=conv1.bias,
                      Cout=Cout, out=h1, ldo=Cout)
        act2 = self.scratch("act2", N * P, Cout)
        if not self.conv_fused_gn(gn=gn2, gn_film=film, gn_out=act2, gn_act=nat.ACT_SILU, gn_skip_raw=1, **c1):
            self.add_conv(**c1)
            act2 = self.gn_apply(h1, None, Cout, 0, N, P, gn2, film, nat.ACT_SILU, "act2")
        kw = dict(src0=act2, C0=Cout, N=N, Hs=H, Ws=W, Ho=H, Wo=W, W=self.packed(conv2.weight), bias=conv2.bias,
                  Cout=Cout, out=out, ldo=Cout)
        if isinstance(rb.skip_connection, nn.Identity):
            assert b is None
            kw.update(res=a, ldr=Cout)
        else:
            sk = rb.skip_connection
            kw.update(s2src0=a, s2src1=b, s2C0=C0, s2C1=C1, W2=sk.weight, bias2=sk.bias)
        nact = self._final_conv(kw, next_gn, N * P)
        res = dict(parts=[(out, Cout)], H=H, W=W)
        if nact is not None:
            res["act1"] = nact
        if getattr(self, "_cat_done", None) is not None:
            res["act1cat"], self._cat_done = self._cat_done, None
        return res

    def _attn(self, ab, cur, next_gn=None):
        L = nat.lib()
        B, T = self.B, self.T
        N, H, W = B * T, cur["H"], cur["W"]
        P = H * W
        (x, Cc), = cur["parts"]
        M = N * P
        heads = ab.num_heads
        ta, sa = ab.temporal_attention, ab.spatial_attention
        if TEMPORAL_QKV and L.lfvdm_gn_temporal_qkv_ok(B, T, P, Cc) == 0:
            self.add(L.lfvdm_gn_temporal_qkv, _p(x), _p(ta.norm.weight), _p(ta.norm.bias), ta.norm.eps, _p(self.s_xn),
                     _p(ta.qkv.weight), _p(ta.qkv.bias), _p(self.s_qkv), B, T, P, Cc)
        else:
            self.add(L.lfvdm_gn_temporal, _p(x), _p(ta.norm.weight), _p(ta.norm.bias), ta.norm.eps, _p(self.s_xn), B, T, P, Cc)
            self.add_conv(src0=self.s_xn, C0=Cc, N=N, Hs=P, Ws=1, Ho=P, Wo=1, ksize=1, W=ta.qkv.weight, bias=ta.qkv.bias,
                          Cout=3 * Cc, out=self.s_qkv, ldo=3 * Cc)
        at = None
        if self.want_attn:
            at = self.buf(B * P, heads, T, T)
            self.attn_t.append(at)
        if self.time_steps:
            self.add(L.lfvdm_attn_temporal_ring, _p(self.s_qkv), _p(self.R[ta.rpe_q]), _p(self.R[ta.rpe_k]), _p(self.R[ta.rpe_v]),
                     _p(self.mask), _p(self.s_o), _p(at) if at is not None else None, B, T, P, Cc, heads, _p(self.t_sel),
                     self.time_ring)
        else:
            self.add(L.lfvdm_attn_temporal, _p(self.s_qkv), _p(self.R[ta.rpe_q]), _p(self.R[ta.rpe_k]), _p(self.R[ta.rpe_v]),
                     _p(self.mask), _p(self.s_o), _p(at) if at is not None else None, B, T, P, Cc, heads)
        yt = self.buf(M, Cc)
        proj = dict(src0=self.s_o, C0=Cc, N=N, Hs=P, Ws=1, Ho=P, Wo=1, ksize=1, W=ta.proj_out.weight,
                    bias=ta.proj_out.bias, Cout=Cc, res=self.s_xn, ldr=Cc, out=yt, ldo=Cc)
        ysn = self.scratch("act1", M, Cc)
        if PROJ_GN and M > CHAIN_MAX_M and L.lfvdm_proj_gn_ok(N, P, Cc) == 0:
            self.add(L.lfvdm_proj_gn, _p(self.s_o), _p(ta.proj_out.weight), _p(ta.proj_out.bias), _p(self.s_xn),
                     _p(sa.norm.weight), _p(sa.norm.bias), sa.norm.eps, nat.ACT_NONE, _p(ysn), None, N, P, Cc)
        elif not self.conv_fused_gn(gn=sa.norm, gn_out=ysn, gn_act=nat.ACT_NONE, gn_skip_raw=1, **proj):
            self.add_conv(**proj)
            ysn = self.gn_apply(yt, None, Cc, 0, N, P, sa.norm, None, nat.ACT_NONE, "act1")
        fused_sa = (SPATIAL_FUSED and not self.want_attn and L.lfvdm_attn_spatial_fused_ok(N, P, Cc, heads) == 0)
        if fused_sa:
            self.add(L.lfvdm_attn_spatial_fused, _p(ysn), _p(sa.qkv.weight), _p(sa.qkv.bias), _p(self.s_o), N, P, Cc, heads)
        else:
            self.add_conv(src0=ysn, C0=Cc, N=N, Hs=P, Ws=1, Ho=P, Wo=1, ksize=1, W=sa.qkv.weight, bias=sa.qkv.bias,
                          Cout=3 * Cc, out=self.s_qkv, ldo=3 * Cc)
            asp = None
            if self.want_attn:
                asp = self.buf(N, heads, P, P)
                self.attn_s.append(asp)
            self.add(L.lfvdm_attn_spatial, _p(self.s_qkv), _p(self.s_o), _p(asp) if asp is not None else None, None, N, P, Cc, heads)
        ys = self.buf(M, Cc)
        nact = self._final_conv(dict(src0=self.s_o, C0=Cc, N=N, Hs=P, Ws=1, Ho=P, Wo=1, ksize=1, W=sa.proj_out.weight,
                                     bias=sa.proj_out.bias, Cout=Cc, res=ysn, ldr=Cc, out=ys, ldo=Cc), next_gn, M)
        res = dict(parts=[(ys, Cc)], H=H, W=W)
        if nact is not None:
            res["act1"] = nact
        if getattr(self, "_cat_done", None) is not None:
            res["act1cat"], self._cat_done = self._cat_done, None
        return res

    def _resample(self, conv, cur, down, next_gn=None):
        if not isinstance(conv, nn.Conv2d):
            raise NotImplementedError("conv_resample=False (pooling) is not on the native path")
        N, H, W = self.B * self.T, cur["H"], cur["W"]
        (x, Cc), = cur["parts"]
        Ho, Wo = (((H + 2 - 3) // 2 + 1, (W + 2 - 3) // 2 + 1) if down else (2 * H, 2 * W))
        out = self.buf(N * Ho * Wo, Cc)
        kw = dict(src0=x, C0=Cc, N=N, Hs=H, Ws=W, up=0 if down else 1, stride=2 if down else 1, Ho=Ho, Wo=Wo, bias=conv.bias,
                  Cout=Cc, out=out, ldo=Cc)
        if not down and N * Ho * Wo > CHAIN_MAX_M:
            codes = (C.c_int * 4)()
            if nat.lib().lfvdm_conv_igemm_candidates(C.byref(self.conv_args(**dict(kw, up=3, W=x))), codes, 4) > 0:
                kw.update(up=3, W=self.packed_up2x(conv.weight))
        if "W" not in kw:
            kw["W"] = self.packed(conv.weight)
        nact = self._final_conv(kw, next_gn, N * Ho * Wo)
        res = dict(parts=[(out, Cc)], H=Ho, W=Wo)
        if nact is not None:
            res["act1"] = nact
        if getattr(self, "_cat_done", None) is not None:
            res["act1cat"], self._cat_done = self._cat_done, None
        return res

    def build_time_tables(self, ts_table):
        L, m = nat.lib(), self.model
        n_t, B = self.time_steps, self.B
        assert ts_table.numel() == n_t
        Bv, ch = n_t * B, m.model_channels
        ted, half = 4 * ch, ch // 2
        Bvp = (Bv + 3) // 4 * 4
        tin = th.zeros(Bvp + half, device=self.dev, dtype=th.float32)
        tin[:Bv] = ts_table.to(self.dev, th.float32).repeat_interleave(B)
        tin[Bvp:] = timestep_freqs(ch).to(self.dev)
        e0, emb = th.empty(Bv, ted, device=self.dev), th.empty(Bv, ted, device=self.dev)
        se0, semb = th.empty_like(e0), th.empty_like(emb)
        (j0, j1, jg), n_g, rows_g = self._emb_jobs(Bv, tin, Bvp, e0, emb, self.rows_all, se0, semb)
        s = nat.stream()
        nat.check(L.lfvdm_rowdot(_p(j0), 1, ted, s), "lfvdm_rowdot")
        nat.check(L.lfvdm_silu(_p(e0), _p(se0), e0.numel(), s), "lfvdm_silu")
        nat.check(L.lfvdm_rowdot(_p(j1), 1, ted, s), "lfvdm_rowdot")
        nat.check(L.lfvdm_silu(_p(emb), _p(semb), emb.numel(), s), "lfvdm_silu")
        nat.check(L.lfvdm_rowdot(_p(jg), n_g, rows_g, s), "lfvdm_rowdot")
        th.cuda.current_stream().synchronize()
        self.tables_sig = (self.time_signature(), tuple(ts_table.tolist()))

    def build_R_tables(self, frame_indices):
        if not self.R:
            return
        n_t, B, T = self.time_steps, self.B, self.T
        steps = (self.time_ring // 2) if self.time_ring else n_t
        self._fi_rep = frame_indices.to(self.dev, th.int64).reshape(B, T).repeat(steps, 1).contiguous()
        self._loaded = {}
        if not self.time_ring:
            self._fill_R(0, n_t, 0)

    def _fill_R(self, t0, t1, slot0):
        B, T = self.B, self.T
        key = (t0, t1, slot0)
        ent = self._fill_jobs.get(key)
        if ent is None:
            views = {r: buf[slot0 * B:] for r, buf in self.R.items()}
            ent = self._rpe_jobs((t1 - t0) * B, self.rows_all[t0 * B:], views)
            self._fill_jobs[key] = ent
        jr, n_r, tiles_r = ent
        nat.check(nat.lib().lfvdm_rpe_nets_maxc(_p(jr), n_r, tiles_r, _p(self._fi_rep), (t1 - t0) * B, T,
                                                max(r.rpe_net.channels for r in self.R), nat.stream()), "lfvdm_rpe_nets")

    def ensure_R(self, t_hi, t_lo=None):
        if not self.time_ring or not self.R:
            return
        H = self.time_ring // 2
        t_hi = min(max(int(t_hi), 0), self.time_steps - 1)
        t_lo = t_hi if t_lo is None else min(max(int(t_lo), 0), t_hi)
        assert t_hi - t_lo < H, "a graph launch walks less than half a ring of timesteps"
        for blk in {t_hi // H, t_lo // H}:
            if self._loaded.get(blk % 2) != blk:
                self._fill_R(blk * H, min((blk + 1) * H, self.time_steps), (blk % 2) * H)
                self._loaded[blk % 2] = blk

    def fill_whole_chain(self):
        if not self.R:
            return
        if not self.time_ring:
            self._fill_R(0, self.time_steps, 0)
            return
        H = self.time_ring // 2
        for blk in range((self.time_steps + H - 1) // H):
            self._fill_R(blk * H, min((blk + 1) * H, self.time_steps), (blk % 2) * H)
        self._loaded = {}

    def fuse_head_update(self, t_buf, tables, clip, seed, noise, pred, inject_noise, ddim=None, predict_xstart=False):
        L = nat.lib()
        h = self.head
        if self.head_fused:
            return True
        if h["step"] != len(self.steps) - 1 or L.lfvdm_conv_out_psample_ok(self.B * self.T, self.H, self.W, h["C"], h["Cout"]) != 0:
            return False
        self.keep.append((t_buf, tables, seed, noise, pred, ddim))
        recip, recipm1, c1, c2, sg, rule, mean_type = update_args(tables, ddim, predict_xstart)
        det, x0 = sg is None, recip is None
        if rule == nat.RULE_DPMPP2M:
            args = (_p(h["act"]), _p(h["Wp"]), _p(h["bias"]), _p(self.out), _p(self.x_in), _p(pred), _p(t_buf),
                    None if x0 else _p(recip), None if x0 else _p(recipm1), _p(c1), _p(c2), _p(sg), mean_type, int(bool(clip)),
                    _p(self.x_in), _p(pred), self.B, self.T, self.H, self.W, h["C"], h["Cout"])
            self.steps[h["step"]] = (L.lfvdm_conv_out_update_ms_x0, args)
            self.head_fused = True
            return True
        args = (_p(h["act"]), _p(h["Wp"]), _p(h["bias"]), _p(self.out), _p(self.x_in),
                _p(noise) if inject_noise and not det else None, None if inject_noise or det else _p(noise), _p(t_buf),
                None if x0 else _p(recip), None if x0 else _p(recipm1), _p(c1), _p(c2), None if det else _p(sg), rule, mean_type,
                int(bool(clip)), _p(self.x_in), _p(pred), None, self.B, self.T, self.H, self.W, h["C"], h["Cout"],
                None if det else _p(seed))
        self.steps[h["step"]] = (L.lfvdm_conv_out_update_x0, args)
        self.head_fused = True
        return True

    def tick(self, t_buf, ts_table):
        L = nat.lib()
        if self.time_steps:
            nat.check(L.lfvdm_sampler_tick_fetch(_p(t_buf), _p(ts_table), _p(self.tin), self.B, _p(self.rows_all), self.rows_ld,
                                                 _p(self.rows), self.film_floats, nat.stream()), "lfvdm_sampler_tick_fetch")
        else:
            nat.check(L.lfvdm_sampler_tick(_p(t_buf), _p(ts_table), _p(self.tin), self.B, nat.stream()), "lfvdm_sampler_tick")

    def autotune(self, rounds=3, reps=6):
        L = nat.lib()
        cache = nat.tune_cache()
        tuned = 0
        for fn, args in self.steps:
            if fn is not L.lfvdm_conv_igemm:
                continue
            a = args[0]._obj
            key = nat.tune_key(a)
            if _chains.tile_stage_candidate(a):
                ckey = key + (nat.TUNE_CHAIN,)
                if ckey not in cache:
                    cache[ckey] = nat.autotune_launch(a, rounds, reps, chain_only=True)
                if cache[ckey]:
                    a.tune = cache[ckey]
                    tuned += 1
                    continue
            if key not in cache:
                cache[key] = nat.autotune_launch(a, rounds, reps)
            a.tune = cache[key]
            tuned += 1
        self.tuned = True
        nat.tune_cache_save()
        n_chains = self.build_chains()
        for fn, args in self.steps:
            if fn is L.lfvdm_conv_igemm:
                a = args[0]._obj
                key = nat.tune_key(a)
                if cache.get(key + (nat.TUNE_CHAIN,)) and a.tune == cache[key + (nat.TUNE_CHAIN,)]:
                    if key not in cache:
                        cache[key] = nat.autotune_launch(a, rounds, reps)
                    a.tune = cache[key]
        nat.tune_cache_save()
        if n_chains and os.environ.get("LFVDM_CHAIN_TUNE", "1") != "0":
            self.tune_chains()
        return tuned

    build_chains, tune_chains = _chains.build, _chains.tune
    disable_chains, split_chains, chains_aborted = _chains.disable, _chains.split, _chains.aborted

    def weight_signature(self):
        return (self.engine.epoch,) + tuple(e[0]._version for e in self.packs)

    def time_signature(self):
        return self.weight_signature() + tuple(t._version for t in self._time_params)

    def refresh_weights(self):
        s = nat.stream()
        L = nat.lib()
        for w, out, *part in self.packs:
            if part == ["up2x"]:
                nat.check(L.lfvdm_pack_conv_weight_up2x(_p(w), _p(out), w.shape[0], w.shape[1], s), "pack_up2x")
                continue
            if part:
                w = w.detach()[:, part[0]:part[1]].contiguous()
            nat.check(L.lfvdm_pack_conv_weight(_p(w), _p(out), w.shape[0], w.shape[1], w.shape[2], s), "pack")
        self._sig = self.weight_signature()

    def launch(self, tick=None):
        L = nat.lib()
        s = nat.stream()
        for fn, args in self.steps:
            if tick is not None and fn is L.lfvdm_conv_in:
                rc = L.lfvdm_conv_in_tick(*args, _p(tick[0]), _p(tick[1]), _p(self.tin), self.B, _p(self.rows_all),
                                          self.rows_ld, _p(self.rows), self.film_floats, s)
                tick = None
            else:
                rc = fn(*args, s)
            if rc:
                nat.check(rc, getattr(fn, "__name__", "kernel"))
        assert tick is None, "the plan has no lfvdm_conv_in launch to carry the clock"

    def set_inputs(self, x, x0, timesteps, frame_indices, obs_mask, latent_mask):
        B, T = self.B, self.T
        if x.data_ptr() != self.x_in.data_ptr():
            self.x_in.copy_(x)
        if x0.data_ptr() != self.x0_in.data_ptr():
            self.x0_in.copy_(x0)
        ob = obs_mask.reshape(B, T).to(th.float32)
        self.obs.copy_(ob.reshape(-1))
        th.clamp(ob + latent_mask.reshape(B, T).to(th.float32), max=1.0, out=self.mask)
        self.fi.copy_(frame_indices)
        self.tin[:B].copy_(timesteps)


class Engine:

    def __init__(self, model):
        nat.lib()
        self.model = model
        self.plans = {}
        self.epoch = 0
        for p in model.parameters():
            if p.dtype != th.float32:
                raise RuntimeError("the native path is fp32 (use_fp16 is off in the reference defaults)")

    def plan(self, B, T, H, W, want_attn=False):
        key = (B, T, H, W, bool(want_attn))
        pl = self.plans.get(key)
        if pl is None:
            pl = Plan(self, B, T, H, W, bool(want_attn))
            pl.refresh_weights()
            self.plans[key] = pl
        elif pl._sig != pl.weight_signature():
            pl.refresh_weights()
        return pl

    def invalidate(self):
        self.epoch += 1
        nat.param_epoch[0] += 1

    def forward(self, x, x0, timesteps, frame_indices, obs_mask, latent_mask, return_attn_weights=False):
        B, T, Cx, H, W = x.shape
        grad_needed = th.is_grad_enabled() and (x.requires_grad or any(p.requires_grad for p in self.model.parameters()))
        if grad_needed or (self.model.training and self.model.dropout > 0):
            from ._autograd import unet_apply
            return unet_apply(self, x, x0, timesteps, frame_indices, obs_mask, latent_mask, return_attn_weights)
        pl = self.plan(B, T, H, W, return_attn_weights)
        pl.set_inputs(x.detach(), x0.detach(), timesteps, frame_indices, obs_mask, latent_mask)
        pl.launch()
        out = pl.out.clone()
        attns = None
        if return_attn_weights:
            attns = {"spatial": [a.mean(dim=1).abs() for a in pl.attn_s],
                     "temporal": [a.mean(dim=1).abs() for a in pl.attn_t], "mixed": []}
        return out, attns
```

latent-flexible-video-diffusion-modeling_amd/improved_diffusion/_native.py:

```python
import atexit
import ctypes as C
import json
import os

import torch

_HERE = os.path.dirname(os.path.abspath(__file__))
LIB_PATH = os.environ.get("LFVDM_LIB_PATH") or os.path.join(os.path.dirname(_HERE), "lib", "liblfvdm_hip.so")

ACT_NONE, ACT_SILU = 0, 1
OUT_ROWS, OUT_NCHW = 0, 1

_lib = None

c_fp = C.c_void_p
c_i = C.c_int


class ConvArgs(C.Structure):
    _fields_ = [
        ("src0", c_fp), ("src1", c_fp), ("C0", C.c_int32), ("C1", C.c_int32), ("N", C.c_int32),
        ("Hs", C.c_int32), ("Ws", C.c_int32), ("up", C.c_int32), ("stride", C.c_int32), ("ksize", C.c_int32),
        ("Ho", C.c_int32), ("Wo", C.c_int32), ("coefA", c_fp), ("coefB", c_fp), ("act", C.c_int32),
        ("W", c_fp), ("bias", c_fp), ("Cout", C.c_int32),
        ("s2src0", c_fp), ("s2src1", c_fp), ("s2C0", C.c_int32), ("s2C1", C.c_int32), ("W2", c_fp), ("bias2", c_fp),
        ("res", c_fp), ("ldr", C.c_int32), ("resA", c_fp), ("resB", c_fp),
        ("out", c_fp), ("ldo", C.c_int32), ("out_mode", C.c_int32), ("tune", C.c_int32),
        ("splitk_ws", c_fp), ("splitk_cnt", c_fp), ("splitk_ws_floats", C.c_int64), ("splitk_cnt_ints", C.c_int64),
        ("gn_gamma", c_fp), ("gn_beta", c_fp), ("gn_film", c_fp), ("gn_out", c_fp), ("gn_film_ld", C.c_int32),
        ("gn_film_div", C.c_int32), ("gn_act", C.c_int32), ("gn_skip_raw", C.c_int32), ("gn_eps", C.c_float),
        ("gn_general", C.c_int32), ("gn_gw", C.c_int32), ("gn_ld", C.c_int32),
    ]


class GnArgs(C.Structure):
    _fields_ = [("src0", c_fp), ("src1", c_fp), ("C0", C.c_int32), ("C1", C.c_int32), ("N", C.c_int32), ("P", C.c_int32),
                ("gamma", c_fp), ("beta", c_fp), ("film", c_fp), ("film_div", C.c_int32), ("film_ld", C.c_int32),
                ("eps", C.c_float), ("act", C.c_int32), ("out", c_fp), ("cg", C.c_int32), ("ldo", C.c_int32), ("out_base", c_fp),
                ("out_col", C.c_int32), ("pad_", C.c_int32)]


class GnBwdArgs(C.Structure):
    _fields_ = ([(n, c_fp) for n in ("da", "src0", "src1", "coefA", "coefB", "stats", "out0", "out1", "add", "add2", "gamma", "beta",
                                     "film", "dgamma", "dbeta", "dfilm", "sums_out", "ws")] + [("ws_floats", C.c_int64)]
                + [(n, C.c_int32) for n in ("C0", "C1", "N", "P", "act", "add_ld", "add2_ld", "film_ld", "T", "dfilm_ld")])


class ChainStage(C.Structure):
    _fields_ = [("kind", C.c_int32), ("n_items", C.c_int32), ("flag_base", C.c_int32), ("n_flags", C.c_int32),
                ("dep_base", C.c_int32), ("dep_stride", C.c_int32), ("cfg", C.c_int32), ("kz", C.c_int32), ("nt2", C.c_int32),
                ("wg_off", C.c_int32), ("side", C.c_int32), ("wg_lo", C.c_int32), ("wg_count", C.c_int32), ("ws_off", C.c_int64), ("cnt_off", C.c_int64), ("conv", ConvArgs), ("gn", GnArgs)]


CHAIN_CONV, CHAIN_GN, CHAIN_LOCAL = 0, 1, 2
CHAIN_CTL_EPOCH, CHAIN_CTL_EXIT, CHAIN_CTL_ABORT, CHAIN_CTL_INTS = 0, 32, 64, 96


class AdamWArgs(C.Structure):
    _fields_ = [("p", c_fp), ("g", c_fp), ("m", c_fp), ("v", c_fp), ("ema", c_fp * 4), ("ema_rate", C.c_float * 4),
                ("n_ema", C.c_int32), ("n", C.c_int64), ("lr", C.c_float), ("beta1", C.c_float), ("beta2", C.c_float),
                ("eps", C.c_float), ("weight_decay", C.c_float), ("bias_corr1", C.c_float), ("bias_corr2_sqrt", C.c_float),
                ("grad_scale", C.c_float), ("grad_sqsum", c_fp), ("skip_flag", c_fp), ("skip_flag2", c_fp)]


class RowdotJob(C.Structure):
    _fields_ = [("W", c_fp), ("b", c_fp), ("inp", c_fp), ("out", c_fp), ("K", C.c_int32), ("O", C.c_int32),
                ("M", C.c_int32), ("ldin", C.c_int32), ("ldout", C.c_int32), ("in_mode", C.c_int32),
                ("row0", C.c_int32), ("pad_", C.c_int32)]


class RowdotBwdJob(C.Structure):
    _fields_ = [("W", c_fp), ("inp", c_fp), ("dout", c_fp), ("dW", c_fp), ("db", c_fp), ("din", c_fp), ("K", C.c_int32),
                ("O", C.c_int32), ("M", C.c_int32), ("ldin", C.c_int32), ("lddout", C.c_int32), ("lddin", C.c_int32),
                ("in_mode", C.c_int32), ("task0", C.c_int32)]


class PackJob(C.Structure):
    _fields_ = [("src", c_fp), ("dst", c_fp), ("Cout", C.c_int32), ("Cin", C.c_int32), ("taps", C.c_int32),
                ("transposed", C.c_int32), ("blk0", C.c_int32), ("ld", C.c_int32)]


param_epoch = [0]


class UnpackJob(C.Structure):
    _fields_ = [("gp", c_fp), ("g", c_fp), ("Cout", C.c_int32), ("Cin", C.c_int32), ("taps", C.c_int32), ("row0", C.c_int32),
                ("ldp", C.c_int32), ("pad_", C.c_int32)]


class RpeJob(C.Structure):
    _fields_ = [("tproj", c_fp), ("Wd", c_fp), ("bd", c_fp), ("Wout", c_fp), ("bout", c_fp), ("R", c_fp),
                ("C", C.c_int32), ("tile0", C.c_int32), ("tproj_ld", C.c_int32), ("pad_", C.c_int32), ("act", c_fp)]


class RpeBwdJob(C.Structure):
    _fields_ = [("tproj", c_fp), ("Wd", c_fp), ("bd", c_fp), ("Wout_t", c_fp), ("dR", c_fp), ("dtproj", c_fp),
                ("dWd", c_fp), ("dbd", c_fp), ("C", C.c_int32), ("tile0", C.c_int32), ("tproj_ld", C.c_int32),
                ("dtproj_ld", C.c_int32)]


class WgradJob(C.Structure):
    _fields_ = [("a", ConvArgs), ("msplit", C.c_int32), ("task0", C.c_int32)]


_SIGS = {
    "lfvdm_abi_version": ([], c_i),
    "lfvdm_conv_igemm": ([C.POINTER(ConvArgs), c_fp], c_i),
    "lfvdm_conv_igemm_config": ([C.POINTER(ConvArgs), C.POINTER(c_i), C.POINTER(c_i)], c_i),
    "lfvdm_conv_igemm_candidates": ([C.POINTER(ConvArgs), C.POINTER(c_i), c_i], c_i),
    "lfvdm_pack_conv_weight": ([c_fp, c_fp, c_i, c_i, c_i, c_fp], c_i),
    "lfvdm_pack_conv_weight_up2x": ([c_fp, c_fp, c_i, c_i, c_fp], c_i),
    "lfvdm_conv_wgrad": ([C.POINTER(ConvArgs), c_fp], c_i),
    "lfvdm_pack_conv_weight_t": ([c_fp, c_fp, c_i, c_i, c_i, c_fp], c_i),
    "lfvdm_unpack_conv_grad": ([c_fp, c_fp, c_i, c_i, c_i, c_i, c_fp], c_i),
    "lfvdm_unpack_conv_grads": ([c_fp, c_i, c_i, c_i, c_fp], c_i),
    "lfvdm_pack_conv_weights": ([c_fp, c_i, c_i, c_fp], c_i),
    "lfvdm_conv_in": ([c_fp] * 6 + [c_i] * 5 + [c_fp], c_i),
    "lfvdm_gn_coef": ([c_fp, c_fp, c_i, c_i, c_i, c_i, c_fp, c_fp, c_fp, c_i, c_i, C.c_float, c_fp, c_fp, c_fp], c_i),
    "lfvdm_gn_coef_stats": ([c_fp, c_fp, c_i, c_i, c_i, c_i, c_fp, c_fp, c_fp, c_i, c_i, C.c_float, c_fp, c_fp, c_fp, c_fp], c_i),
    "lfvdm_gn_apply": ([c_fp, c_fp, c_i, c_i, c_i, c_i, c_fp, c_fp, c_fp, c_i, c_i, C.c_float, c_i, c_fp, c_fp, c_fp, c_fp, c_fp], c_i),
    "lfvdm_gn_apply_part": ([c_fp, c_i, c_i, c_i, c_i, c_fp, c_fp, C.c_float, c_i, c_fp, c_i, c_fp], c_i),
    "lfvdm_gn_apply_ws_floats": ([c_i, c_i, c_i], C.c_long),
    "lfvdm_gn_apply_ws": ([c_fp, c_fp, c_i, c_i, c_i, c_i, c_fp, c_fp, c_fp, c_i, c_i, C.c_float, c_i, c_fp, c_fp, c_fp, c_fp, c_fp,
                           C.c_long, c_fp], c_i),
    "lfvdm_compose_rows": ([c_fp, c_fp, c_fp, c_fp, c_i, c_i, c_i, c_i, c_i, c_fp], c_i),
    "lfvdm_conv_in_tick": ([c_fp, c_fp, c_fp, c_fp, c_fp, c_fp, c_i, c_i, c_i, c_i, c_i, c_fp, c_fp, c_fp, c_i, c_fp, c_i, c_fp, c_i,
                            c_fp], c_i),
    "lfvdm_conv_out_psample_ok": ([c_i] * 5, c_i),
    "lfvdm_update_x0": ([c_fp] * 9 + [c_i, c_i, c_i] + [c_fp] * 3 + [c_i, c_i, c_fp], c_i),
    "lfvdm_update_rng_x0": ([c_fp] * 9 + [c_i, c_i, c_i] + [c_fp] * 3 + [c_i, c_i, c_fp, c_fp], c_i),
    "lfvdm_conv_out_update_x0": ([c_fp] * 13 + [c_i, c_i, c_i] + [c_fp] * 3 + [c_i] * 6 + [c_fp, c_fp], c_i),
    "lfvdm_update_ms_x0": ([c_fp] * 9 + [c_i, c_i] + [c_fp] * 2 + [c_i, c_i, c_fp], c_i),
    "lfvdm_conv_out_update_ms_x0": ([c_fp] * 12 + [c_i, c_i] + [c_fp] * 2 + [c_i] * 6 + [c_fp], c_i),
    "lfvdm_known_blend": ([c_fp] * 9 + [c_i] * 4 + [c_fp], c_i),
    "lfvdm_renoise": ([c_fp] * 6 + [c_i, c_i, c_fp], c_i),
    "lfvdm_dyn_threshold_workspace": ([c_i, C.c_int64, C.POINTER(C.c_size_t)], c_i),
    "lfvdm_dyn_threshold": ([c_fp] * 5 + [c_i, c_i, c_fp, c_i, c_i, C.c_int64, C.c_double, C.c_float] + [c_fp] * 4, c_i),
    "lfvdm_noise_prior_factor": ([c_fp, C.c_double, C.c_double, C.c_double, c_fp, c_i, c_i, c_fp], c_i),
    "lfvdm_noise_prior_fill": ([c_fp] * 5 + [c_i, c_i, C.c_int64, c_fp], c_i),
    "lfvdm_masked_mse_bwd": ([c_fp, c_fp, c_fp, c_fp, c_fp, c_i, c_i, c_i, c_fp], c_i),
    "lfvdm_vb_terms": ([c_fp] * 12 + [c_i, c_i] + [c_fp] * 4 + [c_i] * 5 + [c_fp], c_i),
    "lfvdm_vb_terms_bwd": ([c_fp] * 11 + [c_i, c_i, c_fp, c_i, c_i, c_i, c_fp], c_i),
    "lfvdm_frame_metrics": ([c_fp, c_fp, c_i, C.c_float, C.c_float] + [c_i] * 5 + [c_fp, c_fp, c_fp, C.c_long, c_fp], c_i),
    "lfvdm_frame_metrics_workspace": ([c_i] * 5, C.c_long),
    "lfvdm_frame_dist_rows": ([c_fp] + [c_i] * 6 + [c_fp, c_i, c_fp, c_i, c_fp, c_fp], c_i),
    "lfvdm_fps_select": ([c_fp, c_i, c_i, c_fp, c_i, c_fp, c_i, c_i, c_fp, c_fp], c_i),
    "lfvdm_gn_bwd_stats": ([c_fp, c_fp, c_fp, c_i, c_i, c_i, c_i, c_fp, c_fp, c_fp, c_i, c_fp, c_fp], c_i),
    "lfvdm_gn_bwd_apply": ([c_fp, c_fp, c_fp, c_i, c_i, c_i, c_i, c_fp, c_fp, c_fp, c_fp, c_i, c_fp, c_fp, c_i, c_i, c_fp], c_i),
    "lfvdm_gn_bwd_apply_params": ([c_fp, c_fp, c_fp, c_i, c_i, c_i, c_i, c_fp, c_fp, c_fp, c_fp, c_i, c_fp, c_fp, c_i, c_i,
                                   c_fp, c_fp, c_fp, c_i, c_i, c_fp, c_fp, c_fp, c_i, c_fp, c_i, c_fp], c_i),
    "lfvdm_gn_bwd_ws_floats": ([c_i, c_i, c_i], C.c_long),
    "lfvdm_gn_bwd": ([C.POINTER(GnBwdArgs), c_fp], c_i),
    "lfvdm_gn_param_grads": ([c_fp, c_fp, c_fp, c_fp, c_i, c_i, c_fp, c_fp, c_fp, c_i, c_i, c_i, c_fp], c_i),
    "lfvdm_rowdot_bwd": ([c_fp, c_i, c_i, c_fp], c_i),
    "lfvdm_gn_temporal_bwd": ([c_fp, c_fp, c_fp, C.c_float, c_fp, c_fp, c_fp, c_i, c_i, c_i, c_i, c_i, c_fp], c_i),
    "lfvdm_gn_temporal": ([c_fp, c_fp, c_fp, C.c_float, c_fp, c_i, c_i, c_i, c_i, c_fp], c_i),
    "lfvdm_gn_temporal_qkv_ok": ([c_i, c_i, c_i, c_i], c_i),
    "lfvdm_proj_gn_ok": ([c_i, c_i, c_i], c_i),
    "lfvdm_proj_gn": ([c_fp, c_fp, c_fp, c_fp, c_fp, c_fp, C.c_float, c_i, c_fp, c_fp, c_i, c_i, c_i, c_fp], c_i),
    "lfvdm_gn_temporal_qkv": ([c_fp, c_fp, c_fp, C.c_float, c_fp, c_fp, c_fp, c_fp, c_i, c_i, c_i, c_i, c_fp], c_i),
    "lfvdm_rowdot": ([c_fp, c_i, c_i, c_fp], c_i),
    "lfvdm_silu": ([c_fp, c_fp, C.c_int64, c_fp], c_i),
    "lfvdm_rpe_nets": ([c_fp, c_i, c_i, c_fp, c_i, c_i, c_fp], c_i),
    "lfvdm_rpe_nets_maxc": ([c_fp, c_i, c_i, c_fp, c_i, c_i, c_i, c_fp], c_i),
    "lfvdm_rpe_nets_bwd": ([c_fp, c_i, c_i, c_fp, c_i, c_i, c_fp], c_i),
    "lfvdm_conv_wgrad_grouped": ([c_fp, c_i, c_i, c_fp], c_i),
    "lfvdm_attn_spatial": ([c_fp, c_fp, c_fp, c_fp, c_i, c_i, c_i, c_i, c_fp], c_i),
    "lfvdm_attn_spatial_fused_ok": ([c_i, c_i, c_i, c_i], c_i),
    "lfvdm_attn_spatial_fused": ([c_fp, c_fp, c_fp, c_fp, c_i, c_i, c_i, c_i, c_fp], c_i),
    "lfvdm_det_reduce": ([c_fp, c_fp, C.c_long, C.c_long, c_fp], c_i),
    "lfvdm_gn_temporal_bwd_det": ([c_fp, c_fp, c_fp, C.c_float, c_fp, c_fp, c_fp, c_i, c_i, c_i, c_i, c_i, c_fp, C.c_int64, c_fp], c_i),
    "lfvdm_rowdot_bwd_det": ([c_fp, c_i, c_i, c_fp, C.c_int64, c_fp, C.c_int64, c_fp], c_i),
    "lfvdm_rpe_nets_bwd_det": ([c_fp, c_i, c_i, c_fp, c_i, c_i, c_fp, C.c_int64, c_fp], c_i),
    "lfvdm_rpe_front": ([c_fp, c_i, c_fp, c_fp, c_fp, c_fp, c_i, c_i, c_i, c_fp], c_i),
    "lfvdm_rpe_front_bwd": ([c_fp, c_i, c_fp, c_fp, c_fp, c_fp, c_fp, c_i, c_fp, c_fp, c_i, c_i, c_i, c_fp], c_i),
    "lfvdm_sampler_tick": ([c_fp, c_fp, c_fp, c_i, c_fp], c_i),
    "lfvdm_sampler_tick_fetch": ([c_fp, c_fp, c_fp, c_i, c_fp, c_i, c_fp, c_i, c_fp], c_i),
    "lfvdm_attn_temporal_sel": ([c_fp] * 7 + [c_i] * 5 + [c_fp, c_fp], c_i),
    "lfvdm_attn_temporal_ring": ([c_fp] * 7 + [c_i] * 5 + [c_fp, c_i, c_fp], c_i),
    "lfvdm_attn_temporal_bwd": ([c_fp] * 12 + [c_i] * 5 + [c_fp], c_i),
    "lfvdm_attn_spatial_bwd": ([c_fp] * 6 + [c_i, c_i, c_i, c_i, c_fp], c_i),
    "lfvdm_attn_temporal": ([c_fp] * 7 + [c_i] * 5 + [c_fp], c_i),
    "lfvdm_adamw_ema": ([C.POINTER(AdamWArgs), c_fp], c_i),
    "lfvdm_grad_norm_nparts": ([C.c_int64], c_i),
    "lfvdm_grad_norm_partials": ([c_fp, C.c_int64, C.c_float, c_fp, c_i, c_fp], c_i),
    "lfvdm_grad_norm_finalize": ([c_fp, c_i, C.c_float, c_fp, c_fp], c_i),
    "lfvdm_adamw_ema_clip": ([C.POINTER(AdamWArgs), c_fp, c_fp], c_i),
    "lfvdm_q_sample": ([c_fp] * 6 + [c_i, c_i, c_fp], c_i),
    "lfvdm_masked_mse": ([c_fp] * 4 + [c_i, c_i, c_i, c_fp], c_i),
    "lfvdm_train_loss": ([c_fp] * 6 + [c_i] + [c_fp] * 3 + [c_i, c_i, c_i, c_fp], c_i),
    "lfvdm_train_loss_bwd": ([c_fp] * 5 + [c_i, c_fp, c_fp, c_i, c_i, c_i, c_fp], c_i),
    "lfvdm_prepare_batch": ([c_fp] * 6 + [c_i] * 4 + [c_fp], c_i),
    "lfvdm_wavelet_encode": ([c_fp, c_i, C.c_float, C.c_float, c_fp, c_fp, c_fp] + [c_i] * 6 + [c_fp], c_i),
    "lfvdm_wavelet_decode": ([c_fp, c_fp, c_fp, c_fp] + [c_i] * 7 + [c_fp], c_i),
    "lfvdm_prepare_batch_wavelet": ([c_fp, c_i, C.c_float, C.c_float] + [c_fp] * 7 + [c_i] * 8 + [c_fp], c_i),
    "lfvdm_shapes_trajectories": ([c_fp, c_fp, c_fp, C.c_uint64] + [c_i] * 7 + [c_fp], c_i),
    "lfvdm_shapes_render": ([c_fp] * 5 + [c_i] + [c_fp] * 3 + [c_i] * 7 + [c_fp], c_i),
    "lfvdm_search_assemble": ([c_fp] * 9 + [c_i] * 5 + [c_fp], c_i),
    "lfvdm_search_noise_qsample": ([c_fp] * 10 + [c_i] * 4 + [c_fp], c_i),
    "lfvdm_search_noise_fill": ([c_fp, C.c_uint64, c_i, c_i, c_fp] + [c_i] * 4 + [c_fp], c_i),
    "lfvdm_search_scores": ([c_fp, c_fp, c_fp] + [c_i] * 5 + [c_fp], c_i),
    "lfvdm_chain_plan": ([C.POINTER(ChainStage), c_i, C.POINTER(C.c_int32), C.c_int64, C.POINTER(C.c_int64), C.POINTER(C.c_int32),
                          C.POINTER(C.c_int64), C.POINTER(C.c_int64), C.POINTER(C.c_int32), C.POINTER(C.c_int32)], c_i),
    "lfvdm_chain_conv_ok": ([C.POINTER(ConvArgs)], c_i),
    "lfvdm_chain_gn_ok": ([c_i, c_i, c_i, c_i], c_i),
    "lfvdm_chain_local_ok": ([C.POINTER(ConvArgs), c_i], c_i),
    "lfvdm_chain_capacity": ([c_i], c_i),
    "lfvdm_level_chain": ([c_fp, c_i, c_fp, c_fp, c_fp, c_i, c_i, C.c_double, c_fp], c_i),
    "lfvdm_flag_add": ([c_fp, c_fp], c_i),
    "lfvdm_flag_wait": ([c_fp, c_i, C.c_double, c_fp, c_fp], c_i),
    "lfvdm_flag_wait2": ([c_fp, c_i, C.c_double, c_fp, c_fp, c_fp], c_i),
}

EXPORTS = tuple(_SIGS)

GN_APPLY_ARGS = ("src0", "src1", "C0", "C1", "N", "P", "gamma", "beta", "film", "film_div", "film_ld", "eps", "act", "out",
                 "coefA", "coefB", "stats")
GN_APPLY_PART_ARGS = ("src0", "C0", "N", "P", "cg", "gamma", "beta", "eps", "act", "out", "ldo")


def gn_fwd_call(alloc_ws=None, **kw):
    L = lib()
    kw = dict(dict(src1=None, C1=0, film=None, film_div=1, film_ld=0, act=ACT_NONE, out=None, coefA=None, coefB=None,
                   stats=None), **kw)
    if kw["out"] is None:
        return L.lfvdm_gn_coef_stats, tuple(kw[k] for k in GN_APPLY_ARGS if k not in ("act", "out"))
    args = tuple(kw[k] for k in GN_APPLY_ARGS)
    need = int(L.lfvdm_gn_apply_ws_floats(kw["C0"] + kw["C1"], kw["N"], kw["P"]))
    return (L.lfvdm_gn_apply_ws, args + (alloc_ws(need), need)) if need else (L.lfvdm_gn_apply, args)


def lib():
    global _lib
    if _lib is None:
        if not os.path.exists(LIB_PATH):
            raise RuntimeError(
                f"native library {LIB_PATH} is missing - build it with "
                "`python latent-flexible-video-diffusion-modeling_amd/build.py` (there is no fallback path)")
        L = C.CDLL(LIB_PATH)
        for name, (argt, rest) in _SIGS.items():
            fn = getattr(L, name)
            fn.argtypes = argt
            fn.restype = rest
        _lib = L
    return _lib


_ERR = {1: "invalid shape", 2: "HIP launch error", 3: "unsupported configuration"}


def check(rc, what):
    if rc != 0:
        raise RuntimeError(f"{what} failed: {_ERR.get(rc, rc)}")


def stream():
    return torch.cuda.current_stream().cuda_stream


def ptr(t, dtype=torch.float32):
    if t is None:
        return None
    if not t.is_cuda:
        raise RuntimeError("native ops need device (HIP) tensors; the product has no CPU path")
    if t.dtype != dtype:
        raise RuntimeError(f"expected {dtype}, got {t.dtype}")
    if not t.is_contiguous():
        raise RuntimeError("expected a contiguous tensor")
    return t.data_ptr()


def conv_igemm(**kw):
    a = fill_conv_args(**kw)
    ws, cnt = splitk_workspace(kw["out"].device)
    a.splitk_ws, a.splitk_cnt, a.splitk_ws_floats, a.splitk_cnt_ints = ws.data_ptr(), cnt.data_ptr(), ws.numel(), cnt.numel()
    a.tune = tuned_code(a)
    check(lib().lfvdm_conv_igemm(C.byref(a), stream()), "lfvdm_conv_igemm")


_splitk = {}


def splitk_workspace(device):
    ent = _splitk.get(device)
    if ent is None:
        ent = _splitk[device] = (torch.empty(2 * 1024 * 1024, device=device, dtype=torch.float32),
                                 torch.zeros(4096, device=device, dtype=torch.int32))
    return ent


_tune = None
_tune_saved = 0


TUNE_CHAIN, TUNE_IN_CHAIN, TUNE_LOCAL_RT = -101, -102, -103


def tune_key(a):
    return (a.N, a.Hs, a.Ws, a.up, a.stride, a.ksize, a.Ho, a.Wo, a.C0, a.C1, a.Cout, a.s2C0, a.s2C1, bool(a.coefA), a.act,
            bool(a.res), bool(a.resA), a.out_mode, bool(a.splitk_ws),
            (1 + bool(a.gn_film) + 2 * bool(a.gn_skip_raw) + 4 * bool(a.gn_gw)) if a.gn_out else 0)


def tune_cache():
    global _tune, _tune_saved
    if _tune is None:
        _tune = {}
        for path in (os.environ.get("LFVDM_TUNE_CACHE", ""), os.environ.get("LFVDM_TUNE_CACHE_OUT", "")):
            if path and os.path.exists(path):
                try:
                    with open(path) as f:
                        blob = json.load(f)
                    if blob.get("abi") == int(lib().lfvdm_abi_version()):
                        _tune.update({tuple(json.loads(k)): int(v) for k, v in blob["entries"].items()})
                except (OSError, ValueError, KeyError):
                    pass
        _tune_saved = len(_tune)
        atexit.register(tune_cache_save)
    return _tune


def tune_cache_save():
    global _tune_saved
    path = os.environ.get("LFVDM_TUNE_CACHE_OUT", "")
    if not path or _tune is None or len(_tune) == _tune_saved or os.environ.get("RANK", "0") != "0":
        return
    try:
        os.makedirs(os.path.dirname(os.path.abspath(path)), exist_ok=True)
        tmp = f"{path}.{os.getpid()}.tmp"
        with open(tmp, "w") as f:
            json.dump({"abi": int(lib().lfvdm_abi_version()),
                       "entries": {json.dumps([int(x) for x in k]): int(v) for k, v in sorted(_tune.items())}}, f, indent=0)
        os.replace(tmp, path)
        _tune_saved = len(_tune)
    except OSError:
        pass


def autotune_launch(a, rounds=3, reps=6, chain_only=False):
    rounds = int(os.environ.get("LFVDM_TUNE_ROUNDS", rounds))
    reps = int(os.environ.get("LFVDM_TUNE_REPS", reps))
    L, s = lib(), stream()
    codes = (C.c_int * 256)()
    n = L.lfvdm_conv_igemm_candidates(C.byref(a), codes, 256)
    ev0, ev1 = torch.cuda.Event(enable_timing=True), torch.cuda.Event(enable_timing=True)
    best, best_t = 0, float("inf")
    for code in ([] if chain_only else [0]) + [codes[i] for i in range(n)]:
        a.tune = code
        if chain_only and L.lfvdm_chain_conv_ok(C.byref(a)) != 0:
            continue
        if L.lfvdm_conv_igemm(C.byref(a), s) != 0:
            continue
        t_min = float("inf")
        for _ in range(rounds):
            ev0.record()
            for _ in range(reps):
                L.lfvdm_conv_igemm(C.byref(a), s)
            ev1.record()
            ev1.synchronize()
            t_min = min(t_min, ev0.elapsed_time(ev1))
        if t_min < best_t * 0.98:
            best, best_t = code, t_min
    a.tune = best
    return best


def tuned_code(a):
    cache = tune_cache()
    key = tune_key(a)
    code = cache.get(key)
    if code is None:
        if os.environ.get("LFVDM_AUTOTUNE", "1") == "0" or torch.cuda.is_current_stream_capturing():
            return 0
        code = cache[key] = autotune_launch(a)
    return code


def fill_conv_args(**kw):
    a = ConvArgs()
    g = kw.get
    a.src0 = ptr(kw["src0"]); a.src1 = ptr(g("src1")); a.C0 = kw["C0"]; a.C1 = g("C1", 0)
    a.N = kw["N"]; a.Hs = kw["Hs"]; a.Ws = kw["Ws"]; a.up = g("up", 0); a.stride = g("stride", 1)
    a.ksize = g("ksize", 3); a.Ho = kw["Ho"]; a.Wo = kw["Wo"]
    a.coefA = ptr(g("coefA")); a.coefB = ptr(g("coefB")); a.act = g("act", ACT_NONE)
    a.W = ptr(g("W")); a.bias = ptr(g("bias")); a.Cout = kw["Cout"]
    a.s2src0 = ptr(g("s2src0")); a.s2src1 = ptr(g("s2src1")); a.s2C0 = g("s2C0", 0); a.s2C1 = g("s2C1", 0)
    a.W2 = ptr(g("W2")); a.bias2 = ptr(g("bias2"))
    a.res = ptr(g("res")); a.ldr = g("ldr", kw["Cout"]); a.resA = ptr(g("resA")); a.resB = ptr(g("resB"))
    a.out = ptr(kw["out"]); a.ldo = g("ldo", kw["Cout"]); a.out_mode = g("out_mode", OUT_ROWS)
    if g("gn_out") is not None:
        film = g("gn_film")
        a.gn_gamma = ptr(kw["gn_gamma"]); a.gn_beta = ptr(kw["gn_beta"]); a.gn_out = ptr(kw["gn_out"])
        a.gn_film = film.data_ptr() if film is not None else None
        a.gn_film_ld = film.stride(0) if film is not None else 0
        a.gn_film_div = g("gn_film_div", 1); a.gn_act = g("gn_act", ACT_NONE); a.gn_skip_raw = int(g("gn_skip_raw", 0))
        a.gn_eps = g("gn_eps", 1e-5)
    return a


def deterministic():
    return os.environ.get("LFVDM_DETERMINISTIC", "0") == "1"


_det_ws = {}


def det_workspace(device):
    ws = _det_ws.get(device)
    if ws is None:
        if torch.cuda.is_current_stream_capturing():
            raise RuntimeError("deterministic workspace missing under stream capture: run the step eagerly once first")
        ws = _det_ws[device] = torch.empty(int(os.environ.get("LFVDM_DET_WS_MB", "1024")) * 2 ** 18, device=device, dtype=torch.float32)
    return ws


def _wgrad_codes(a):
    Cin, M = a.C0 + a.C1, a.N * a.Ho * a.Wo
    if Cin % 64 or a.C0 % 64 or a.Cout < 64 or a.coefA:
        return []
    nchunks = (M + 31) // 32
    codes = []
    for tile, cot in ((1, 2), (2, 4), (3, 4)):
        if cot == 4 and a.Cout < 128:
            continue
        kt = 4 if tile == 3 else 2
        if tile == 3 and (Cin % 128 or a.C0 % 128):
            continue
        tiles = a.ksize * a.ksize * (Cin // (32 * kt)) * ((a.Cout + 32 * cot - 1) // (32 * cot))
        for stages in (2, 1, 3):
            for target in (256, 320, 384, 448, 512, 640, 768, 1024):
                ms = max(1, min((target + tiles - 1) // tiles, (nchunks // 2 if stages == 3 else nchunks) // 2))
                code = 1 + tile + 4 * stages + 16 * ms
                if code not in codes:
                    codes.append(code)
    HW = a.Ho * a.Wo
    if (a.ksize == 3 and a.stride == 1 and a.up == 0 and HW % 32 == 0 and (a.Wo % 32 == 0 or a.Wo in (8, 16))
            and a.Hs == a.Ho and a.Ws == a.Wo and a.out_mode == 0):
        for tile, rows in ((1, 3), (2, 1)):
            tiles = rows * (Cin // 64) * ((a.Cout + 63) // 64)
            for target in (128, 192, 256, 320, 384, 512):
                ms = max(1, min((target + tiles - 1) // tiles, (M // 32) // 2))
                code = 1 + tile + 16 * ms
                if code not in codes:
                    codes.append(code)
    return codes


def _capturing():
    return torch.cuda.is_available() and torch.cuda.is_current_stream_capturing()


def _tuned_wgrad_code(a, out_floats):
    cache = tune_cache()
    key = _wgrad_key(a)
    store = _rank_store()
    skey = "lfvdm/wgrad/" + json.dumps([int(x) for x in key])

    def publish(code):
        if store is not None and store[1] == 0 and key not in _wgrad_published:
            store[0].set(skey, str(int(code)))
            _wgrad_published.add(key)

    code = _wgrad_agreed.get(key)
    if code is not None:
        publish(code)
        return code
    if store is not None and store[1] != 0:
        if _capturing():
            return cache.get(key, 0)
        import datetime
        try:
            store[0].wait([skey], datetime.timedelta(seconds=float(os.environ.get("LFVDM_WGRAD_AGREE_S", "60"))))
            code = int(store[0].get(skey).decode())
        except Exception:
            code = cache.get(key, 0)
            import sys
            print(f"[lfvdm] rank {store[1]}: no weight-gradient launch code from rank 0 for {skey}; using {code}", file=sys.stderr,
                  flush=True)
        _wgrad_agreed[key] = code
        return code
    code = cache.get(key)
    if code is None:
        if _capturing() or os.environ.get("LFVDM_AUTOTUNE", "1") == "0" or deterministic():
            code = 0
        else:
            code = _measure_wgrad_code(a, out_floats)
            cache[key] = code
    _wgrad_agreed[key] = code
    publish(code)
    return code


_wgrad_agreed = {}
_wgrad_published = set()
_store_memo = []


def _wgrad_key(a):
    return (-1,) + tune_key(a) + (int(bool(a.bias)), int(a.ldr != a.Cout and a.ldr != 0))


def _rank_store():
    if not _store_memo:
        import torch.distributed as dist
        st = None
        if dist.is_available() and dist.is_initialized() and dist.get_world_size() > 1:
            try:
                st = (dist.distributed_c10d._get_default_store(), dist.get_rank())
            except Exception:
                st = None
        if not (dist.is_available() and dist.is_initialized()):
            return None
        _store_memo.append(st)
    return _store_memo[0]


def _measure_wgrad_code(a, out_floats):
    codes = _wgrad_codes(a)
    if not codes:
        return 0
    L, s = lib(), stream()
    dev = torch.device("cuda", torch.cuda.current_device())
    scratch, sb = torch.zeros(out_floats, device=dev), torch.zeros(max(a.Cout, 1), device=dev)
    real_out, real_bias = a.out, a.bias
    a.out = scratch.data_ptr()
    if real_bias:
        a.bias = sb.data_ptr()
    ev0, ev1 = torch.cuda.Event(enable_timing=True), torch.cuda.Event(enable_timing=True)
    best, best_t = 0, float("inf")
    for code in [0] + codes:
        a.tune = code
        if L.lfvdm_conv_wgrad(C.byref(a), s) != 0:
            continue
        t_min = float("inf")
        for _ in range(int(os.environ.get("LFVDM_TUNE_ROUNDS", 3))):
            ev0.record()
            for _ in range(int(os.environ.get("LFVDM_TUNE_REPS", 4))):
                L.lfvdm_conv_wgrad(C.byref(a), s)
            ev1.record()
            ev1.synchronize()
            t_min = min(t_min, ev0.elapsed_time(ev1))
        if t_min < best_t * 0.98:
            best, best_t = code, t_min
    a.out, a.bias, a.tune = real_out, real_bias, 0
    return best


def conv_wgrad(**kw):
    a = fill_conv_args(**kw)
    if deterministic():
        key = _wgrad_key(a)
        ws = det_workspace(kw["out"].device)
        a.splitk_ws, a.splitk_ws_floats = ws.data_ptr(), ws.numel()
        a.tune = tune_cache().get(key, 0)
    else:
        a.tune = _tuned_wgrad_code(a, kw["out"].numel())
    check(lib().lfvdm_conv_wgrad(C.byref(a), stream()), "lfvdm_conv_wgrad")


def pack_conv_weight_t(w, out):
    Cout, Cin, k = w.shape[0], w.shape[1], (w.shape[2] if w.dim() == 4 else 1)
    check(lib().lfvdm_pack_conv_weight_t(ptr(w), ptr(out), Cout, Cin, k, stream()), "lfvdm_pack_conv_weight_t")


def unpack_conv_grad(gp, g, accumulate):
    Cout, Cin, k = g.shape[0], g.shape[1], (g.shape[2] if g.dim() == 4 else 1)
    check(lib().lfvdm_unpack_conv_grad(ptr(gp), ptr(g), Cout, Cin, k, int(bool(accumulate)), stream()), "lfvdm_unpack_conv_grad")


def conv_igemm_struct(a):
    check(lib().lfvdm_conv_igemm(C.byref(a), stream()), "lfvdm_conv_igemm")


def pack_conv_weight(w, out):
    Cout, Cin, k, _ = w.shape
    check(lib().lfvdm_pack_conv_weight(ptr(w), ptr(out), Cout, Cin, k, stream()), "lfvdm_pack_conv_weight")


def pack_conv_weight_up2x(w, out):
    Cout, Cin, k, _ = w.shape
    if k != 3 or out.numel() != 16 * Cout * Cin:
        raise RuntimeError("lfvdm_pack_conv_weight_up2x needs a 3x3 weight and a [4][Cout][4][Cin] output")
    check(lib().lfvdm_pack_conv_weight_up2x(ptr(w), ptr(out), Cout, Cin, stream()), "lfvdm_pack_conv_weight_up2x")


def conv_in(x, x0, obs, w, bias, out, N, Cc, H, W, Cout):
    check(lib().lfvdm_conv_in(ptr(x), ptr(x0), ptr(obs), ptr(w), ptr(bias), ptr(out), N, Cc, H, W, Cout, stream()),
          "lfvdm_conv_in")


def gn_coef(src0, src1, C0, C1, N, P, gamma, beta, film, film_div, film_ld, eps, coefA, coefB):
    check(lib().lfvdm_gn_coef(ptr(src0), ptr(src1), C0, C1, N, P, ptr(gamma), ptr(beta), ptr(film), film_div, film_ld,
                              eps, ptr(coefA), ptr(coefB), stream()), "lfvdm_gn_coef")


def gn_temporal(x, gamma, beta, eps, y, B, T, P, Cc):
    check(lib().lfvdm_gn_temporal(ptr(x), ptr(gamma), ptr(beta), eps, ptr(y), B, T, P, Cc, stream()), "lfvdm_gn_temporal")


def rowdot(jobs_dev, njobs, total_rows):
    check(lib().lfvdm_rowdot(ptr(jobs_dev, torch.uint8), njobs, total_rows, stream()), "lfvdm_rowdot")


def rpe_nets(jobs_dev, njobs, total_tiles, frame_indices, B, T):
    check(lib().lfvdm_rpe_nets(ptr(jobs_dev, torch.uint8), njobs, total_tiles, ptr(frame_indices, torch.int64), B, T,
                               stream()), "lfvdm_rpe_nets")


def attn_spatial(qkv, o, attn_out, N, P, Cc, heads, lse=None):
    check(lib().lfvdm_attn_spatial(ptr(qkv), ptr(o), ptr(attn_out), ptr(lse), N, P, Cc, heads, stream()),
          "lfvdm_attn_spatial")


def attn_spatial_bwd(qkv, o, d_o, lse, delta_ws, dqkv, N, P, Cc, heads):
    check(lib().lfvdm_attn_spatial_bwd(ptr(qkv), ptr(o), ptr(d_o), ptr(lse), ptr(delta_ws), ptr(dqkv), N, P, Cc, heads,
                                       stream()), "lfvdm_attn_spatial_bwd")


def attn_temporal(qkv, Rq, Rk, Rv, mask, o, attn_out, B, T, P, Cc, heads):
    check(lib().lfvdm_attn_temporal(ptr(qkv), ptr(Rq), ptr(Rk), ptr(Rv), ptr(mask), ptr(o), ptr(attn_out), B, T, P, Cc,
                                    heads, stream()), "lfvdm_attn_temporal")


def attn_temporal_bwd(qkv, d_o, Rq, Rk, Rv, mask, ws_p, ws_ds, dqkv, dRq, dRk, dRv, B, T, P, Cc, heads):
    check(lib().lfvdm_attn_temporal_bwd(ptr(qkv), ptr(d_o), ptr(Rq), ptr(Rk), ptr(Rv), ptr(mask), ptr(ws_p), ptr(ws_ds),
                                        ptr(dqkv), ptr(dRq), ptr(dRk), ptr(dRv), B, T, P, Cc, heads, stream()),
          "lfvdm_attn_temporal_bwd")


def q_sample(x0, noise, t, sa, sb, out):
    B = x0.shape[0]
    check(lib().lfvdm_q_sample(ptr(x0), ptr(noise), ptr(t, torch.int64), ptr(sa), ptr(sb), ptr(out), B,
                               x0.numel() // B, stream()), "lfvdm_q_sample")


RULE_ANCESTRAL, RULE_DDIM = 0, 1
MEAN_EPS, MEAN_X0 = 0, 1
RULE_DPMPP2M = "dpmpp2m"


def update_x0(x, out, noise, t, recip, recipm1, c1, c2, sg, rule, mean_type, clip, sample, pred=None, mean=None):
    B = x.shape[0]
    check(lib().lfvdm_update_x0(ptr(x), ptr(out), ptr(noise), ptr(t, torch.int64), ptr(recip), ptr(recipm1), ptr(c1), ptr(c2),
                                ptr(sg), int(rule), int(mean_type), int(bool(clip)), ptr(sample), ptr(pred), ptr(mean), B,
                                x.numel() // B, stream()), "lfvdm_update_x0")


def update_rng_x0(x, out, noise_out, t, recip, recipm1, c1, c2, sg, rule, mean_type, clip, sample, seed, pred=None, mean=None):
    B = x.shape[0]
    check(lib().lfvdm_update_rng_x0(ptr(x), ptr(out), ptr(noise_out), ptr(t, torch.int64), ptr(recip), ptr(recipm1), ptr(c1),
                                    ptr(c2), ptr(sg), int(rule), int(mean_type), int(bool(clip)), ptr(sample), ptr(pred),
                                    ptr(mean), B, x.numel() // B, ptr(seed, torch.int64) if seed is not None else None, stream()),
          "lfvdm_update_rng_x0")


def conv_out_update_x0(act, wp, bias, out, x, noise_in, noise_out, t, recip, recipm1, c1, c2, sg, rule, mean_type, clip, sample,
                       seed, pred=None, mean=None):
    B, T, Cout, H, W = x.shape
    check(lib().lfvdm_conv_out_update_x0(ptr(act), ptr(wp), ptr(bias), ptr(out), ptr(x), ptr(noise_in), ptr(noise_out),
                                         ptr(t, torch.int64), ptr(recip), ptr(recipm1), ptr(c1), ptr(c2), ptr(sg), int(rule),
                                         int(mean_type), int(bool(clip)), ptr(sample), ptr(pred), ptr(mean), B, T, H, W,
                                         act.shape[-1], Cout, ptr(seed, torch.int64) if seed is not None else None, stream()),
          "lfvdm_conv_out_update_x0")


def update_ms_x0(x, out, hist, t, recip, recipm1, k1, k2, k3, mean_type, clip, sample, pred=None):
    B = x.shape[0]
    check(lib().lfvdm_update_ms_x0(ptr(x), ptr(out), ptr(hist), ptr(t, torch.int64), ptr(recip), ptr(recipm1), ptr(k1), ptr(k2),
                                   ptr(k3), int(mean_type), int(bool(clip)), ptr(sample), ptr(pred), B, x.numel() // B, stream()),
          "lfvdm_update_ms_x0")


def conv_out_update_ms_x0(act, wp, bias, out, x, hist, t, recip, recipm1, k1, k2, k3, mean_type, clip, sample, pred=None):
    B, T, Cout, H, W = x.shape
    check(lib().lfvdm_conv_out_update_ms_x0(ptr(act), ptr(wp), ptr(bias), ptr(out), ptr(x), ptr(hist), ptr(t, torch.int64),
                                            ptr(recip), ptr(recipm1), ptr(k1), ptr(k2), ptr(k3), int(mean_type), int(bool(clip)),
                                            ptr(sample), ptr(pred), B, T, H, W, act.shape[-1], Cout, stream()),
          "lfvdm_conv_out_update_ms_x0")


def known_blend(x, known, mask, t, a, s, eps=None, seed=None, noise_out=None):
    B, T, Cx, H, W = x.shape
    if known.shape != x.shape or tuple(mask.shape) != (B, T, H, W) or (eps is not None and eps.shape != x.shape):
        raise RuntimeError("known_blend: known / eps are shaped like x (B, T, C, H, W) and mask is (B, T, H, W)")
    check(lib().lfvdm_known_blend(ptr(x), ptr(known), ptr(mask), ptr(eps), ptr(noise_out), ptr(t, torch.int64), ptr(a), ptr(s),
                                  ptr(seed, torch.int64) if seed is not None else None, B, T, Cx, H * W, stream()),
          "lfvdm_known_blend")


def renoise(x, t, c, d, seed, noise_out=None):
    B = x.shape[0]
    check(lib().lfvdm_renoise(ptr(x), ptr(noise_out), ptr(t, torch.int64), ptr(c), ptr(d), ptr(seed, torch.int64), B,
                              x.numel() // B, stream()), "lfvdm_renoise")


def dyn_threshold_workspace(B, inner):
    n = C.c_size_t(0)
    check(lib().lfvdm_dyn_threshold_workspace(int(B), int(inner), C.byref(n)), "lfvdm_dyn_threshold_workspace")
    return int(n.value)


def dyn_threshold(x, out, t, recip, recipm1, mean_type, x0hat_fma, frame_mask, percentile, max_value, xhat, stats, workspace):
    B, T = x.shape[0], x.shape[1]
    if out.shape != x.shape or xhat.shape != x.shape or stats.numel() != 3 * B or (
            frame_mask is not None and frame_mask.numel() != B * T):
        raise RuntimeError("dyn_threshold: out / xhat are shaped like x (B, T, ...), frame_mask is (B, T), stats is (B, 3)")
    check(lib().lfvdm_dyn_threshold(ptr(x), ptr(out), ptr(t, torch.int64), ptr(recip), ptr(recipm1), int(mean_type),
                                    int(bool(x0hat_fma)), ptr(frame_mask), B, T, x.numel() // (B * T), float(percentile),
                                    float("inf") if max_value is None else float(max_value), ptr(xhat), ptr(stats),
                                    ptr(workspace, torch.uint8), stream()), "lfvdm_dyn_threshold")


def noise_prior_factor(frame_indices, a, c, rho, out=None):
    B, T = frame_indices.shape
    L = torch.empty(B, T, T, device=frame_indices.device) if out is None else out
    if L.numel() != B * T * T:
        raise RuntimeError("noise_prior_factor: L is (B, T, T)")
    check(lib().lfvdm_noise_prior_factor(ptr(frame_indices, torch.int64), float(a), float(c), float(rho), ptr(L), B, T, stream()),
          "lfvdm_noise_prior_factor")
    return L


def noise_prior_fill(L, out, xi=None, seed=None, t=None):
    B, T = out.shape[0], out.shape[1]
    if L.numel() != B * T * T or (xi is not None and xi.shape != out.shape):
        raise RuntimeError("noise_prior_fill: L is (B, T, T), xi is shaped like out (B, T, ...)")
    if xi is None and (seed is None or t is None or t.numel() != B):
        raise RuntimeError("noise_prior_fill: draw mode needs seed and t (B,)")
    check(lib().lfvdm_noise_prior_fill(ptr(L), ptr(xi), ptr(seed, torch.int64), ptr(t, torch.int64), ptr(out), B, T,
                                       out.numel() // (B * T), stream()), "lfvdm_noise_prior_fill")


def vb_terms(x_start, x_t, out, noise, t, recip, recipm1, c1, c2, post_logvar, model_logvar, mask, mean_type, clip, vb,
             xstart_mse=None, eps_mse=None, pred=None, col_base=-1):
    B, T = x_t.shape[0], x_t.shape[1]
    ld = vb.shape[1] if vb.dim() == 2 else 1
    check(lib().lfvdm_vb_terms(ptr(x_start), ptr(x_t), ptr(out), ptr(noise), ptr(t, torch.int64), ptr(recip), ptr(recipm1), ptr(c1),
                               ptr(c2), ptr(post_logvar), ptr(model_logvar), ptr(mask), int(mean_type), int(bool(clip)), ptr(vb),
                               ptr(xstart_mse), ptr(eps_mse), ptr(pred), B, T, x_t.numel() // (B * T), ld, int(col_base),
                               stream()), "lfvdm_vb_terms")


def vb_terms_bwd(x_start, x_t, out, t, recip, recipm1, c1, c2, model_logvar, mask, g, mean_type, clip, d_out):
    B, T = x_t.shape[0], x_t.shape[1]
    check(lib().lfvdm_vb_terms_bwd(ptr(x_start), ptr(x_t), ptr(out), ptr(t, torch.int64), ptr(recip), ptr(recipm1), ptr(c1), ptr(c2),
                                   ptr(model_logvar), ptr(mask), ptr(g), int(mean_type), int(bool(clip)), ptr(d_out), B, T,
                                   x_t.numel() // (B * T), stream()), "lfvdm_vb_terms_bwd")


PIX_F32, PIX_U8 = 0, 1
_PIX = {torch.float32: PIX_F32, torch.uint8: PIX_U8}


def frame_metrics_workspace(K, N, C, H, W):
    return int(lib().lfvdm_frame_metrics_workspace(K, N, C, H, W))


def frame_metrics(pred, truth, scale, shift, K, N, C, H, W, mse, ssim, partials):
    dt = pred.dtype
    if dt not in _PIX or truth.dtype != dt:
        raise RuntimeError(f"expected float32 or uint8 pixels of one dtype, got {pred.dtype} and {truth.dtype}")
    if pred.numel() != K * N * C * H * W or truth.numel() != N * C * H * W or mse.numel() != K * N or ssim.numel() != K * N:
        raise RuntimeError("frame_metrics: tensor sizes do not match (K, N, C, H, W)")
    check(lib().lfvdm_frame_metrics(ptr(pred, dt), ptr(truth, dt), _PIX[dt], float(scale), float(shift), K, N, C, H, W, ptr(mse),
                                    ptr(ssim), ptr(partials), partials.numel(), stream()), "lfvdm_frame_metrics")


def frame_dist_rows(x, B, T, C, H, W, levels, new_idx, cand_idx, dist):
    if x.numel() != B * T * C * H * W or dist.numel() != B * T * T:
        raise RuntimeError("frame_dist_rows: tensor sizes do not match (B, T, C, H, W)")
    n_cand = 0 if cand_idx is None else cand_idx.numel()
    check(lib().lfvdm_frame_dist_rows(ptr(x), B, T, C, H, W, int(levels), ptr(new_idx, torch.int32), new_idx.numel(),
                                      ptr(cand_idx, torch.int32) if n_cand else None, n_cand, ptr(dist), stream()),
          "lfvdm_frame_dist_rows")


def fps_select(dist, B, T, cand_idx, forced_pos, n, picks):
    if dist.numel() != B * T * T or picks.numel() != B * n:
        raise RuntimeError("fps_select: tensor sizes do not match (B, T, n)")
    check(lib().lfvdm_fps_select(ptr(dist), B, T, ptr(cand_idx, torch.int32), cand_idx.numel(), ptr(forced_pos, torch.int32),
                                 forced_pos.numel(), int(n), ptr(picks, torch.int32), stream()), "lfvdm_fps_select")


def prepare_batch(pool, table, batch, frame_indices, obs_mask, latent_mask):
    B, Tp = pool.shape[:2]
    F = table.shape[1]
    check(lib().lfvdm_prepare_batch(ptr(pool), ptr(table, torch.int32), ptr(batch), ptr(frame_indices, torch.int64), ptr(obs_mask),
                                    ptr(latent_mask), B, F, Tp, pool[0, 0].numel(), stream()), "lfvdm_prepare_batch")


WAVELET_NORMS = {"range": 0, "orthonormal": 1}
_U8_SCALE, _U8_SHIFT = 1.0 / 127.5, -1.0


def _pix_affine(dt):
    if dt not in _PIX:
        raise RuntimeError(f"expected float32 or uint8 pixels, got {dt}")
    return (_U8_SCALE, _U8_SHIFT) if dt == torch.uint8 else (1.0, 0.0)


def wavelet_encode(pix, coef, levels, norm, mean=None, rstd=None):
    N, Cc, H, W = pix.shape
    if coef.numel() != pix.numel():
        raise RuntimeError("wavelet_encode: coef does not hold as many elements as pix")
    scale, shift = _pix_affine(pix.dtype)
    check(lib().lfvdm_wavelet_encode(ptr(pix, pix.dtype), _PIX[pix.dtype], scale, shift, ptr(coef), ptr(mean), ptr(rstd), N, Cc, H,
                                     W, int(levels), WAVELET_NORMS[norm], stream()), "lfvdm_wavelet_encode")


def wavelet_decode(coef, pix, levels, norm, mean=None, std=None):
    N, Cc, H, W = pix.shape
    if coef.numel() != pix.numel() or pix.dtype not in _PIX:
        raise RuntimeError("wavelet_decode: pix must be float32 or uint8 with as many elements as coef")
    check(lib().lfvdm_wavelet_decode(ptr(coef), ptr(mean), ptr(std), ptr(pix, pix.dtype), _PIX[pix.dtype], N, Cc, H, W, int(levels),
                                     WAVELET_NORMS[norm], stream()), "lfvdm_wavelet_decode")


def prepare_batch_wavelet(pool, table, batch, frame_indices, obs_mask, latent_mask, levels, norm, mean=None, rstd=None):
    B, Tp, Cc, H, W = pool.shape
    F = table.shape[1]
    if batch.numel() != B * F * Cc * H * W:
        raise RuntimeError("prepare_batch_wavelet: batch does not hold B * F frames of the pool's size")
    scale, shift = _pix_affine(pool.dtype)
    check(lib().lfvdm_prepare_batch_wavelet(ptr(pool, pool.dtype), _PIX[pool.dtype], scale, shift, ptr(table, torch.int32), ptr(batch),
                                            ptr(frame_indices, torch.int64), ptr(obs_mask), ptr(latent_mask), ptr(mean), ptr(rstd),
                                            B, F, Tp, Cc, H, W, int(levels), WAVELET_NORMS[norm], stream()),
          "lfvdm_prepare_batch_wavelet")


def shapes_trajectories(video_idx, traj, consts, seed, split, stochastic, H, W):
    N, T, S = traj.shape[:3]
    if video_idx.numel() != N or tuple(traj.shape) != (N, T, S, 2) or tuple(consts.shape) != (N, S, 4):
        raise RuntimeError("shapes_trajectories: expected video_idx (N,), traj (N, T, S, 2), consts (N, S, 4)")
    check(lib().lfvdm_shapes_trajectories(ptr(video_idx, torch.int64), ptr(traj, torch.int32), ptr(consts, torch.int32),
                                          int(seed) % (1 << 64), int(split), N, T, S, int(H), int(W), int(bool(stochastic)),
                                          stream()), "lfvdm_shapes_trajectories")


def shapes_render(traj, consts, out, table=None, lut=None, frame_indices=None, obs_mask=None, latent_mask=None):
    N, T, S = traj.shape[:3]
    B, F, Cc, H, W = out.shape
    if Cc != 3 or N % B or N // B not in (1, 2) or tuple(consts.shape) != (N, S, 4) or out.dtype not in _PIX:
        raise RuntimeError("shapes_render: out (B, F, 3, H, W) float32 / uint8 over B or 2 B trajectory videos")
    if table is not None and tuple(table.shape) != (B, F, 4):
        raise RuntimeError("shapes_render: table must be (B, F, 4)")
    for m in (frame_indices, obs_mask, latent_mask):
        if m is not None and m.numel() != B * F:
            raise RuntimeError("shapes_render: index / mask tensors hold B * F elements")
    if lut is not None and lut.numel() != 256:
        raise RuntimeError("shapes_render: the uint8 -> float table has 256 entries")
    check(lib().lfvdm_shapes_render(ptr(traj, torch.int32), ptr(consts, torch.int32), ptr(table, torch.int32), ptr(lut),
                                    ptr(out, out.dtype), _PIX[out.dtype], ptr(frame_indices, torch.int64), ptr(obs_mask),
                                    ptr(latent_mask), B, F, (N // B) * T, T, S, H, W, stream()), "lfvdm_shapes_render")


def masked_mse(a, b, mask, out, B, T, frame_inner):
    check(lib().lfvdm_masked_mse(ptr(a), ptr(b), ptr(mask), ptr(out), B, T, frame_inner, stream()), "lfvdm_masked_mse")


def train_loss(target, pred, mask, eval_mask, t, wtab, mse, eval_mse, loss):
    B, T = pred.shape[0], pred.shape[1]
    check(lib().lfvdm_train_loss(ptr(target), ptr(pred), ptr(mask), ptr(eval_mask), ptr(t, torch.int64), ptr(wtab), wtab.numel(),
                                 ptr(mse), ptr(eval_mse), ptr(loss), B, T, pred.numel() // (B * T), stream()), "lfvdm_train_loss")


def train_loss_bwd(target, pred, mask, t, wtab, g, dpred):
    B, T = pred.shape[0], pred.shape[1]
    check(lib().lfvdm_train_loss_bwd(ptr(target), ptr(pred), ptr(mask), ptr(t, torch.int64), ptr(wtab), wtab.numel(), ptr(g),
                                     ptr(dpred), B, T, pred.numel() // (B * T), stream()), "lfvdm_train_loss_bwd")


def grad_norm_nparts(n):
    return int(lib().lfvdm_grad_norm_nparts(int(n)))


def grad_clip_stat(g, grad_scale, max_norm, partials, stat):
    n = g.numel()
    if partials.numel() != grad_norm_nparts(n) or stat.numel() != 4:
        raise RuntimeError("grad_clip_stat: partials must hold grad_norm_nparts(n) floats and stat four")
    check(lib().lfvdm_grad_norm_partials(ptr(g), n, float(grad_scale), ptr(partials), partials.numel(), stream()),
          "lfvdm_grad_norm_partials")
    check(lib().lfvdm_grad_norm_finalize(ptr(partials), partials.numel(), float(max_norm), ptr(stat), stream()),
          "lfvdm_grad_norm_finalize")


def adamw_ema_clip(a, stat):
    check(lib().lfvdm_adamw_ema_clip(C.byref(a), ptr(stat), stream()), "lfvdm_adamw_ema_clip")


class StreamFlags:

    def __init__(self, n, device):
        self.buf = torch.zeros(n + 1, 32, device=device, dtype=torch.int32)
        self.n = n

    def add(self, k):
        check(lib().lfvdm_flag_add(self.buf[k].data_ptr(), stream()), "lfvdm_flag_add")

    def wait(self, k, target, torch_stream, timeout_s=20.0, also_f32=None):
        wrapped = ((int(target) + 2 ** 31) % 2 ** 32) - 2 ** 31
        check(lib().lfvdm_flag_wait2(self.buf[k].data_ptr(), wrapped, float(timeout_s), self.buf[self.n].data_ptr(), also_f32,
                                     torch_stream.cuda_stream), "lfvdm_flag_wait2")

    def timed_out_ptr(self):
        return self.buf[self.n].data_ptr()

    def timed_out(self):
        return bool(self.buf[self.n, 0].item())


def jobs_to_device(jobs, device):
    if not jobs:
        return None
    arr = (type(jobs[0]) * len(jobs))(*jobs)
    raw = bytes(memoryview(arr))
    return torch.frombuffer(bytearray(raw), dtype=torch.uint8).to(device)


SLOT_PAD, SLOT_OBS, SLOT_LATENT = 0, 1, 2


def search_assemble(pool, table, role, x0, x_start, obs_mask, latent_mask, mask, frame_indices):
    V, Tv = pool.shape[:2]
    W, K = table.shape
    check(lib().lfvdm_search_assemble(ptr(pool), ptr(table, torch.int32), ptr(role, torch.int32), ptr(x0), ptr(x_start),
                                      ptr(obs_mask), ptr(latent_mask), ptr(mask), ptr(frame_indices, torch.int64), W, K, V, Tv,
                                      pool[0, 0].numel(), stream()), "lfvdm_search_assemble")


def search_noise_qsample(x_start, table, t_list, ctl, key, sa, sb, noise, x_t, t_buf, V):
    W, K = table.shape
    check(lib().lfvdm_search_noise_qsample(ptr(x_start), ptr(table, torch.int32), ptr(t_list, torch.int64), ptr(ctl, torch.int32),
                                           ptr(key, torch.int64), ptr(sa), ptr(sb), ptr(noise), ptr(x_t), ptr(t_buf, torch.int64),
                                           W, K, int(V), x_start[0, 0].numel(), stream()), "lfvdm_search_noise_qsample")


def search_noise_fill(table, seed, step, j, noise, V):
    W, K = table.shape
    check(lib().lfvdm_search_noise_fill(ptr(table, torch.int32), int(seed) & (2 ** 64 - 1), int(step), int(j), ptr(noise), W, K,
                                        int(V), noise[0, 0].numel(), stream()), "lfvdm_search_noise_fill")


def search_scores(terms, t_list, scores, G, V, col_base=-1):
    n_t = t_list.numel() if t_list is not None else terms.shape[1]
    check(lib().lfvdm_search_scores(ptr(terms), ptr(t_list, torch.int64) if t_list is not None else None, ptr(scores), int(G),
                                    int(V), n_t, terms.shape[1], int(col_base), stream()), "lfvdm_search_scores")
```

Before: 1265.

## Fuse temporal GroupNorm, QKV projection and temporal attention into one kernel

Adds a fused kernel that runs the temporal group norm, the QKV projection and the relative-position temporal attention in a single launch, so the qkv intermediate never goes through global memory. The engine selects it in sampling when attention maps are not requested and the batch-column count is below a threshold. Shared helpers move into the header so both kernels can reuse them. The trade-off is more LDS and register pressure per block and possibly less parallelism than two separate launches.

New measurement: 1264, median of 2. No clear change (-0.0%).

```diff
diff --git a/include/lfvdm_hip.h b/include/lfvdm_hip.h
--- a/include/lfvdm_hip.h
+++ b/include/lfvdm_hip.h
@@ -273,6 +273,12 @@
 int lfvdm_attn_temporal_ring(const float* qkv, const float* Rq, const float* Rk, const float* Rv, const float* mask,
                              float* o, float* attn_out, int B, int T, int P, int C, int heads, const int64_t* rsel,
                              int ring, void* stream);
+
+int lfvdm_attn_temporal_fused_ok(int B, int T, int P, int C, int heads);
+int lfvdm_attn_temporal_fused(const float* x, const float* gamma, const float* beta, float eps, float* xn_out,
+                              const float* Wqkv, const float* bqkv, const float* Rq, const float* Rk, const float* Rv,
+                              const float* mask, float* o, int B, int T, int P, int C, int heads, const int64_t* rsel,
+                              int ring, void* stream);
 
 int lfvdm_attn_temporal_bwd(const float* qkv, const float* d_o, const float* Rq, const float* Rk, const float* Rv,
                             const float* mask, float* ws_p, float* ws_ds, float* dqkv, float* dRq, float* dRk,
diff --git a/latent-flexible-video-diffusion-modeling_amd/csrc/attention_temporal.h b/latent-flexible-video-diffusion-modeling_amd/csrc/attention_temporal.h
--- a/latent-flexible-video-diffusion-modeling_amd/csrc/attention_temporal.h
+++ b/latent-flexible-video-diffusion-modeling_amd/csrc/attention_temporal.h
@@ -22,3 +22,330 @@
 int lfvdm_attn_temporal2_bwd_rows_try(const TemporalBwd& a);
 int lfvdm_attn_temporal_long(const TemporalFwd& a);
 int lfvdm_attn_temporal_long_bwd(const TemporalBwd& a);
+
+inline bool t2_small_launch(int B, int P, int F) { return (long)B * P * F < 16384; }
+
+namespace {
+
+constexpr int TQ_TF = 3;
+
+__device__ __forceinline__ float tq_dpp_b1(float v) { return __builtin_bit_cast(float, __builtin_amdgcn_mov_dpp(__builtin_bit_cast(int, v), 0xB1, 0xF, 0xF, true)); }
+__device__ __forceinline__ float tq_dpp_4e(float v) { return __builtin_bit_cast(float, __builtin_amdgcn_mov_dpp(__builtin_bit_cast(int, v), 0x4E, 0xF, 0xF, true)); }
+__device__ __forceinline__ float tq_dpp_hm(float v) { return __builtin_bit_cast(float, __builtin_amdgcn_mov_dpp(__builtin_bit_cast(int, v), 0x141, 0xF, 0xF, true)); }
+__device__ __forceinline__ float tq_dpp_r8(float v) { return __builtin_bit_cast(float, __builtin_amdgcn_mov_dpp(__builtin_bit_cast(int, v), 0x128, 0xF, 0xF, true)); }
+
+template <int CG>
+__device__ __forceinline__ float tq_reduce(float v) {
+    v += tq_dpp_b1(v);
+    v += tq_dpp_4e(v);
+    v += tq_dpp_hm(v);
+    if constexpr (CG == 8) v += tq_dpp_r8(v);
+    return v;
+}
+
+template <int CG>
+__device__ __forceinline__ f32x4 tq_group(f32x4 s) {
+    if constexpr (CG == 2) {
+        const float a = tq_reduce<CG>(s.x + s.y), b = tq_reduce<CG>(s.z + s.w);
+        return (f32x4){a, a, b, b};
+    } else {
+        const float a = tq_reduce<CG>((s.x + s.y) + (s.z + s.w));
+        return (f32x4){a, a, a, a};
+    }
+}
+
+template <int CG>
+__device__ __forceinline__ void tq_stats(const f32x4 (&xk)[TQ_TF], int tp, int T, float inv, float eps, f32x4& mu, f32x4& rs) {
+    f32x4 a = {0.f, 0.f, 0.f, 0.f};
+#pragma unroll
+    for (int i = 0; i < TQ_TF; ++i) a += xk[i];
+    mu = tq_group<CG>(a) * inv;
+    f32x4 q = {0.f, 0.f, 0.f, 0.f};
+#pragma unroll
+    for (int i = 0; i < TQ_TF; ++i) {
+        if (tp + 8 * i < T) {
+            const f32x4 d = xk[i] - mu;
+            q += d * d;
+        }
+    }
+    const f32x4 var = tq_group<CG>(q) * inv;
+    rs.x = 1.0f / sqrtf(var.x + eps);
+    rs.z = CG == 2 ? 1.0f / sqrtf(var.z + eps) : rs.x;
+    rs.y = rs.x;
+    rs.w = rs.z;
+}
+
+__device__ __forceinline__ f32x4 tq_apply(f32x4 x, f32x4 mu, f32x4 rs, f32x4 gam, f32x4 bet) { return (x - mu) * rs * gam + bet; }
+
+__device__ __forceinline__ size_t tq_slot(int row, int quad, int SPR) {
+    return ((size_t)row * SPR + ((quad & ~15) | ((quad ^ row) & 15))) * 4;
+}
+
+struct T2Geom {
+    int T, P, C, heads, B;
+    int TG, TGN, PPW, NW;
+    int strips;
+    int NL, HL, XPG;
+};
+
+template <int F, int TCAP>
+struct T2Cfg {
+    static constexpr int NQ = F / 4;
+    static constexpr int RS = (TCAP * NQ + 15) / 16 * 16;
+};
+
+__device__ __forceinline__ void t2_decode(const T2Geom& g, int& b, int& h, int& tg, int& strip) {
+    {
+        const int id = blockIdx.x;
+        if (g.XPG > 0) {
+            const int x = id & 7, r = id >> 3;
+            const int grp = x % g.NL, sub = x / g.NL;
+            const int inner = r % (g.HL * g.TG), sblk = r / (g.HL * g.TG);
+            strip = sblk * g.XPG + sub;
+            const int hl = inner % g.HL;
+            tg = inner / g.HL;
+            const int hpb = g.heads / g.HL;
+            b = grp / hpb;
+            h = (grp % hpb) * g.HL + hl;
+        } else {
+            const int NP = g.B * g.heads;
+            const int pair = id % NP, rest = id / NP;
+            b = pair / g.heads;
+            h = pair % g.heads;
+            tg = rest % g.TG;
+            strip = rest / g.TG;
+        }
+    }
+}
+
+__device__ __forceinline__ void t2_dma(const float* src, float* dst) {
+    __builtin_amdgcn_global_load_lds((const __attribute__((address_space(1))) void*)src,
+                                     (__attribute__((address_space(3))) void*)dst, 16, 0, 0);
+}
+
+template <int F, int TCAP>
+__device__ __forceinline__ void t2_stage_r(const float* __restrict__ filler, const float* __restrict__ Rq, const float* __restrict__ Rk,
+                                           const float* __restrict__ Rv, RSel rsel, const T2Geom& g, int b, int h,
+                                           int tq0, int wave, int nw, int lane, float* Rimg) {
+    using CF = T2Cfg<F, TCAP>;
+    constexpr int NQ = CF::NQ, RS = CF::RS;
+    const int T = g.T, C = g.C;
+    const float invRS = 1.0f / (float)RS;
+    const size_t rb = rsel.slice(b, g.B);
+    const float* Rsrc[3] = {Rk + rb * T * T * C + h * F, Rq + rb * T * T * C + h * F, Rv + rb * T * T * C + h * F};
+    const int nR = (min(g.TGN, T - tq0) * 3 * RS + 63) >> 6;
+    const int TNQ = T * NQ;
+    for (int pc = wave; pc < nR; pc += nw) {
+        const int ps = pc * 64 + lane;
+        const int row3 = (int)(((float)ps + 0.5f) * invRS);
+        const int w = ps - row3 * RS;
+        const int tq = (int)(((float)row3 + 0.5f) * (1.0f / 3.0f)), arr = row3 - 3 * tq;
+        const int c = w ^ (tq & 15);
+        const int s = c / NQ, u = c - s * NQ;
+        const int t = tq0 + tq;
+        const bool ok = tq < g.TGN && t < T && c < TNQ;
+        const int row = arr == 1 ? s * T + t : t * T + s;
+        const float* base = arr == 0 ? Rsrc[0] : (arr == 1 ? Rsrc[1] : Rsrc[2]);
+        t2_dma(ok ? base + (size_t)row * C + 4 * u : filler, Rimg + (size_t)pc * 256);
+    }
+}
+
+template <int F, int TCAP>
+__device__ __forceinline__ void t2_stage_kv(const float* __restrict__ qkv, const T2Geom& g, int b, int h, int p0, int wave,
+                                            int lane, float* KVimg) {
+    using CF = T2Cfg<F, TCAP>;
+    constexpr int NQ = CF::NQ, RS = CF::RS;
+    const int T = g.T, P = g.P, C = g.C;
+    const int NPX = g.NW * g.PPW;
+    const float invRS = 1.0f / (float)RS;
+    const float* kvsrc = qkv + (size_t)b * T * P * 3 * C + C + h * F;
+    const int vpx = min(NPX, P - p0);
+    const int nKV = (vpx * 2 * RS + 63) >> 6;
+    const int TNQ = T * NQ;
+    for (int pc = wave; pc < nKV; pc += g.NW) {
+        const int ps = pc * 64 + lane;
+        const int row2 = (int)(((float)ps + 0.5f) * invRS);
+        const int w = ps - row2 * RS;
+        const int jw = row2 >> 1, arr = row2 & 1;
+        const int c = w ^ (jw & 15);
+        const int s = c / NQ, u = c - s * NQ;
+        const int p = p0 + jw;
+        const bool ok = jw < NPX && p < P && c < TNQ;
+        t2_dma(ok ? kvsrc + ((size_t)s * P + p) * 3 * C + arr * C + 4 * u : qkv, KVimg + (size_t)pc * 256);
+    }
+}
+
+template <int F, int TCAP>
+__device__ __forceinline__ void t2_stage(const float* __restrict__ qkv, const float* __restrict__ Rq, const float* __restrict__ Rk,
+                                         const float* __restrict__ Rv, RSel rsel, const T2Geom& g, int b, int h,
+                                         int tq0, int p0, int wave, int lane, float* Rimg, float* KVimg) {
+    t2_stage_r<F, TCAP>(qkv, Rq, Rk, Rv, rsel, g, b, h, tq0, wave, g.NW, lane, Rimg);
+    t2_stage_kv<F, TCAP>(qkv, g, b, h, p0, wave, lane, KVimg);
+}
+
+template <int F, int TCAP>
+struct T2Lane {
+    int sq, jw, tq, t, p;
+    bool active;
+    int kb[F / 4], rbs[F / 4];
+};
+
+template <int F, int TCAP>
+__device__ __forceinline__ T2Lane<F, TCAP> t2_lane(const T2Geom& g, int wave, int lane, int tq0, int p0) {
+    constexpr int NQ = T2Cfg<F, TCAP>::NQ, RS = T2Cfg<F, TCAP>::RS;
+    T2Lane<F, TCAP> L;
+    const float invN = 1.0f / (float)g.TGN;
+    const int pair = lane >> 2;
+    L.sq = lane & 3;
+    const int j = (int)(((float)pair + 0.5f) * invN);
+    L.tq = pair - j * g.TGN;
+    L.jw = wave * g.PPW + j;
+    L.t = tq0 + L.tq;
+    L.p = p0 + L.jw;
+    L.active = j < g.PPW && L.p < g.P && L.t < g.T;
+    const int jr = L.active ? L.jw : 0, tr = L.active ? L.tq : 0;
+#pragma unroll
+    for (int u = 0; u < NQ; ++u) {
+        const int low = (NQ * L.sq + u) & 15, high = (NQ * L.sq + u) & ~15;
+        L.kb[u] = (jr * 2 * RS + high + (low ^ (jr & 15))) * 4;
+        L.rbs[u] = (tr * 3 * RS + high + (low ^ (tr & 15))) * 4;
+    }
+    return L;
+}
+
+template <int F, int TCAP>
+__device__ __forceinline__ void t2_core(const float* Rimg, const float* KVimg, const f32x4 (&q4)[F / 4], const T2Lane<F, TCAP>& L,
+                                        const float* __restrict__ mask, float* __restrict__ o, float* __restrict__ attn_out,
+                                        const T2Geom& g, int b, int h, float scale) {
+    using CF = T2Cfg<F, TCAP>;
+    constexpr int NQ = CF::NQ, RS = CF::RS;
+    constexpr int KQ = (TCAP + 3) / 4;
+    constexpr int ISTRIDE = 4 * NQ * 4;
+    const int T = g.T, P = g.P, C = g.C;
+    const int sq = L.sq, t = L.t, p = L.p;
+    const bool active = L.active;
+    const int (&kb)[NQ] = L.kb;
+    const int (&rbs)[NQ] = L.rbs;
+    auto quad_x1 = [](float v) { return __builtin_bit_cast(float, __builtin_amdgcn_mov_dpp(__builtin_bit_cast(int, v), 0xB1, 0xF, 0xF, true)); };
+    auto quad_x2 = [](float v) { return __builtin_bit_cast(float, __builtin_amdgcn_mov_dpp(__builtin_bit_cast(int, v), 0x4E, 0xF, 0xF, true)); };
+
+    {
+        float logit[KQ];
+#pragma unroll
+        for (int i = 0; i < KQ; ++i) {
+            f32x2 a0 = {0.f, 0.f}, a1 = {0.f, 0.f};
+#pragma unroll
+            for (int u = 0; u < NQ; ++u) {
+                const f32x4 k4 = ld4(KVimg + kb[u] + i * ISTRIDE);
+                const f32x4 r4 = ld4(Rimg + rbs[u] + i * ISTRIDE);
+                const f32x4 g4 = ld4(Rimg + rbs[u] + RS * 4 + i * ISTRIDE);
+                a0 = __builtin_elementwise_fma(q4[u].xy, k4.xy + r4.xy, a0);
+                a0 = __builtin_elementwise_fma(q4[u].zw, k4.zw + r4.zw, a0);
+                a1 = __builtin_elementwise_fma(k4.xy, g4.xy, a1);
+                a1 = __builtin_elementwise_fma(k4.zw, g4.zw, a1);
+            }
+            logit[i] = (a0.x + a0.y) + (a1.x + a1.y) * scale;
+            asm volatile("" : "+v"(logit[i]) : : "memory");
+            __builtin_amdgcn_sched_barrier(0);
+        }
+        const int tm = active ? t : 0;
+        const float mt = mask ? mask[b * T + tm] : 1.f;
+        float mx = -INFINITY;
+#pragma unroll
+        for (int i = 0; i < KQ; ++i) {
+            const int sk = sq + 4 * i;
+            float v = -INFINITY;
+            if (sk < T) {
+                v = logit[i];
+                if (mask) {
+                    const float ms = mask[b * T + sk];
+                    const float pen = 1.f - (mt * ms + (1.f - mt) * (1.f - ms));
+                    v -= (pen == 1.f) ? INFINITY : pen;
+                }
+            }
+            logit[i] = v;
+            mx = fmaxf(mx, v);
+        }
+        mx = fmaxf(mx, quad_x1(mx));
+        mx = fmaxf(mx, quad_x2(mx));
+        float sum = 0.f;
+#pragma unroll
+        for (int i = 0; i < KQ; ++i) {
+            const float e = (logit[i] == -INFINITY) ? 0.f : __expf(logit[i] - mx);
+            logit[i] = e;
+            sum += e;
+        }
+        sum += quad_x1(sum);
+        sum += quad_x2(sum);
+        const float inv = 1.0f / sum;
+#pragma unroll
+        for (int i = 0; i < KQ; ++i) logit[i] *= inv;
+        if (attn_out && active) {
+            float* ar = attn_out + ((((size_t)b * P + p) * g.heads + h) * T + t) * T;
+#pragma unroll
+            for (int i = 0; i < KQ; ++i)
+                if (sq + 4 * i < T) ar[sq + 4 * i] = logit[i];
+        }
+        f32x4 acc[NQ];
+#pragma unroll
+        for (int u = 0; u < NQ; ++u) acc[u] = (f32x4){0.f, 0.f, 0.f, 0.f};
+#pragma unroll
+        for (int i = 0; i < KQ; ++i) {
+            const f32x2 pr = {logit[i], logit[i]};
+#pragma unroll
+            for (int u = 0; u < NQ; ++u) {
+                const f32x4 v4 = ld4(KVimg + kb[u] + RS * 4 + i * ISTRIDE);
+                const f32x4 r4 = ld4(Rimg + rbs[u] + 2 * RS * 4 + i * ISTRIDE);
+                f32x2 lo = acc[u].xy, hi = acc[u].zw;
+                lo = __builtin_elementwise_fma(pr, v4.xy + r4.xy, lo);
+                hi = __builtin_elementwise_fma(pr, v4.zw + r4.zw, hi);
+                acc[u] = (f32x4){lo.x, lo.y, hi.x, hi.y};
+                asm volatile("" : "+v"(acc[u]) : : "memory");
+            }
+            __builtin_amdgcn_sched_barrier(0);
+        }
+#pragma unroll
+        for (int u = 0; u < NQ; ++u) {
+#pragma unroll
+            for (int e = 0; e < 4; ++e) {
+                float v = acc[u][e];
+                v += quad_x1(v);
+                v += quad_x2(v);
+                acc[u][e] = v;
+            }
+        }
+        if (active) {
+            float* orow = o + ((size_t)(b * T + t) * P + p) * C + h * F;
+#pragma unroll
+            for (int u = 0; u < NQ; ++u)
+                if ((u & 3) == sq) st4(orow + 4 * u, acc[u]);
+        }
+    }
+}
+
+inline void t2_frames(T2Geom& g) {
+    g.TG = (g.T + 4) / 5;
+    g.TGN = (g.T + g.TG - 1) / g.TG;
+    g.PPW = 16 / g.TGN;
+}
+
+inline unsigned t2_place(T2Geom& g, int F) {
+    const int B = g.B, heads = g.heads;
+    const int NPX = g.NW * g.PPW;
+    g.strips = (g.P + NPX - 1) / NPX;
+    g.HL = F >= 32 ? 1 : 32 / F;
+    if (g.HL > heads || heads % g.HL) g.HL = 1;
+    g.NL = B * (heads / g.HL);
+    g.XPG = (g.NL <= 8 && 8 % g.NL == 0) ? 8 / g.NL : 0;
+    if (g.XPG > 0) {
+        const int sblks = (g.strips + g.XPG - 1) / g.XPG;
+        return 8u * (unsigned)(g.HL * g.TG) * (unsigned)sblks;
+    }
+    return (unsigned)(B * heads) * (unsigned)g.TG * (unsigned)g.strips;
+}
+
+inline size_t t2_lds_bytes(int TGN, int NPX, int RS) {
+    return ((size_t)((TGN * 3 * RS + 63) & ~63) + (size_t)((NPX * 2 * RS + 63) & ~63)) * 16;
+}
+
+}
diff --git a/latent-flexible-video-diffusion-modeling_amd/csrc/attention_temporal2.hip b/latent-flexible-video-diffusion-modeling_amd/csrc/attention_temporal2.hip
--- a/latent-flexible-video-diffusion-modeling_amd/csrc/attention_temporal2.hip
+++ b/latent-flexible-video-diffusion-modeling_amd/csrc/attention_temporal2.hip
@@ -2,91 +2,6 @@
 #include "common_hip.h"
 
 namespace {
-
-struct T2Geom {
-    int T, P, C, heads, B;
-    int TG, TGN, PPW, NW;
-    int strips;
-    int NL, HL, XPG;
-};
-
-template <int F, int TCAP>
-struct T2Cfg {
-    static constexpr int NQ = F / 4;
-    static constexpr int RS = (TCAP * NQ + 15) / 16 * 16;
-};
-
-__device__ __forceinline__ void t2_decode(const T2Geom& g, int& b, int& h, int& tg, int& strip) {
-    {
-        const int id = blockIdx.x;
-        if (g.XPG > 0) {
-            const int x = id & 7, r = id >> 3;
-            const int grp = x % g.NL, sub = x / g.NL;
-            const int inner = r % (g.HL * g.TG), sblk = r / (g.HL * g.TG);
-            strip = sblk * g.XPG + sub;
-            const int hl = inner % g.HL;
-            tg = inner / g.HL;
-            const int hpb = g.heads / g.HL;
-            b = grp / hpb;
-            h = (grp % hpb) * g.HL + hl;
-        } else {
-            const int NP = g.B * g.heads;
-            const int pair = id % NP, rest = id / NP;
-            b = pair / g.heads;
-            h = pair % g.heads;
-            tg = rest % g.TG;
-            strip = rest / g.TG;
-        }
-    }
-}
-
-template <int F, int TCAP>
-__device__ __forceinline__ void t2_stage(const float* __restrict__ qkv, const float* __restrict__ Rq, const float* __restrict__ Rk,
-                                         const float* __restrict__ Rv, RSel rsel, const T2Geom& g, int b, int h,
-                                         int tq0, int p0, int wave, int lane, float* Rimg, float* KVimg) {
-    using CF = T2Cfg<F, TCAP>;
-    constexpr int NQ = CF::NQ, RS = CF::RS;
-    const int T = g.T, P = g.P, C = g.C;
-    const int NPX = g.NW * g.PPW;
-    const float invRS = 1.0f / (float)RS;
-    {
-        const size_t rb = rsel.slice(b, g.B);
-        const float* Rsrc[3] = {Rk + rb * T * T * C + h * F, Rq + rb * T * T * C + h * F, Rv + rb * T * T * C + h * F};
-        const float* kvsrc = qkv + (size_t)b * T * P * 3 * C + C + h * F;
-        const int vpx = min(NPX, P - p0);
-        const int nR = (min(g.TGN, T - tq0) * 3 * RS + 63) >> 6, nKV = (vpx * 2 * RS + 63) >> 6;
-        const int TNQ = T * NQ;
-        auto dma = [](const float* src, float* dst) {
-            __builtin_amdgcn_global_load_lds((const __attribute__((address_space(1))) void*)src,
-                                             (__attribute__((address_space(3))) void*)dst, 16, 0, 0);
-        };
-        for (int pc = wave; pc < nR; pc += g.NW) {
-            const int ps = pc * 64 + lane;
-            const int row3 = (int)(((float)ps + 0.5f) * invRS);
-            const int w = ps - row3 * RS;
-            const int tq = (int)(((float)row3 + 0.5f) * (1.0f / 3.0f)), arr = row3 - 3 * tq;
-            const int c = w ^ (tq & 15);
-            const int s = c / NQ, u = c - s * NQ;
-            const int t = tq0 + tq;
-            const bool ok = tq < g.TGN && t < T && c < TNQ;
-            const int row = arr == 1 ? s * T + t : t * T + s;
-            const float* base = arr == 0 ? Rsrc[0] : (arr == 1 ? Rsrc[1] : Rsrc[2]);
-            dma(ok ? base + (size_t)row * C + 4 * u : qkv, Rimg + (size_t)pc * 256);
-        }
-        for (int pc = wave; pc < nKV; pc += g.NW) {
-            const int ps = pc * 64 + lane;
-            const int row2 = (int)(((float)ps + 0.5f) * invRS);
-            const int w = ps - row2 * RS;
-            const int jw = row2 >> 1, arr = row2 & 1;
-            const int c = w ^ (jw & 15);
-            const int s = c / NQ, u = c - s * NQ;
-            const int p = p0 + jw;
-            const bool ok = jw < NPX && p < P && c < TNQ;
-            dma(ok ? kvsrc + ((size_t)s * P + p) * 3 * C + arr * C + 4 * u : qkv, KVimg + (size_t)pc * 256);
-        }
-    }
-
-}
 
 template <int F, int TCAP>
 __global__ __launch_bounds__(256, 3)
@@ -107,132 +22,19 @@
     const int p0 = strip * NPX;
     float* Rimg = t2_smem;
     float* KVimg = t2_smem + (size_t)((g.TGN * 3 * RS + 63) & ~63) * 4;
-    const float invRS = 1.0f / (float)RS;
 
     t2_stage<F, TCAP>(qkv, Rq, Rk, Rv, rsel, g, b, h, tq0, p0, wave, lane, Rimg, KVimg);
 
-    const float invN = 1.0f / (float)g.TGN;
-    const int sq = lane & 3, pair = lane >> 2;
-    const int j = (int)(((float)pair + 0.5f) * invN), tq = pair - j * g.TGN;
-    const int jw = wave * g.PPW + j;
-    const int t = tq0 + tq, p = p0 + jw;
-    const bool active = j < g.PPW && p < P && t < T;
+    const T2Lane<F, TCAP> L = t2_lane<F, TCAP>(g, wave, lane, tq0, p0);
     const float scale = rsqrtf((float)F);
     const size_t ld = (size_t)3 * C;
-    const float* qrow = active ? qkv + ((size_t)(b * T + t) * P + p) * ld + h * F : qkv;
+    const float* qrow = L.active ? qkv + ((size_t)(b * T + L.t) * P + L.p) * ld + h * F : qkv;
     f32x4 q4[NQ];
 #pragma unroll
     for (int u = 0; u < NQ; ++u) q4[u] = ld4(qrow + 4 * u) * scale;
-    constexpr int KQ = (TCAP + 3) / 4;
-    constexpr int ISTRIDE = 4 * NQ * 4;
-    int kb[NQ], rbs[NQ];
-    {
-        const int jr = active ? jw : 0, tr = active ? tq : 0;
-#pragma unroll
-        for (int u = 0; u < NQ; ++u) {
-            const int low = (NQ * sq + u) & 15, high = (NQ * sq + u) & ~15;
-            kb[u] = (jr * 2 * RS + high + (low ^ (jr & 15))) * 4;
-            rbs[u] = (tr * 3 * RS + high + (low ^ (tr & 15))) * 4;
-        }
-    }
     asm volatile("s_waitcnt vmcnt(0)" ::: "memory");
     __syncthreads();
-
-    auto quad_x1 = [](float v) { return __builtin_bit_cast(float, __builtin_amdgcn_mov_dpp(__builtin_bit_cast(int, v), 0xB1, 0xF, 0xF, true)); };
-    auto quad_x2 = [](float v) { return __builtin_bit_cast(float, __builtin_amdgcn_mov_dpp(__builtin_bit_cast(int, v), 0x4E, 0xF, 0xF, true)); };
-
-    {
-        float logit[KQ];
-#pragma unroll
-        for (int i = 0; i < KQ; ++i) {
-            f32x2 a0 = {0.f, 0.f}, a1 = {0.f, 0.f};
-#pragma unroll
-            for (int u = 0; u < NQ; ++u) {
-                const f32x4 k4 = ld4(KVimg + kb[u] + i * ISTRIDE);
-                const f32x4 r4 = ld4(Rimg + rbs[u] + i * ISTRIDE);
-                const f32x4 g4 = ld4(Rimg + rbs[u] + RS * 4 + i * ISTRIDE);
-                a0 = __builtin_elementwise_fma(q4[u].xy, k4.xy + r4.xy, a0);
-                a0 = __builtin_elementwise_fma(q4[u].zw, k4.zw + r4.zw, a0);
-                a1 = __builtin_elementwise_fma(k4.xy, g4.xy, a1);
-                a1 = __builtin_elementwise_fma(k4.zw, g4.zw, a1);
-            }
-            logit[i] = (a0.x + a0.y) + (a1.x + a1.y) * scale;
-            asm volatile("" : "+v"(logit[i]) : : "memory");
-            __builtin_amdgcn_sched_barrier(0);
-        }
-        const int tm = active ? t : 0;
-        const float mt = mask ? mask[b * T + tm] : 1.f;
-        float mx = -INFINITY;
-#pragma unroll
-        for (int i = 0; i < KQ; ++i) {
-            const int sk = sq + 4 * i;
-            float v = -INFINITY;
-            if (sk < T) {
-                v = logit[i];
-                if (mask) {
-                    const float ms = mask[b * T + sk];
-                    const float pen = 1.f - (mt * ms + (1.f - mt) * (1.f - ms));
-                    v -= (pen == 1.f) ? INFINITY : pen;
-                }
-            }
-            logit[i] = v;
-            mx = fmaxf(mx, v);
-        }
-        mx = fmaxf(mx, quad_x1(mx));
-        mx = fmaxf(mx, quad_x2(mx));
-        float sum = 0.f;
-#pragma unroll
-        for (int i = 0; i < KQ; ++i) {
-            const float e = (logit[i] == -INFINITY) ? 0.f : __expf(logit[i] - mx);
-            logit[i] = e;
-            sum += e;
-        }
-        sum += quad_x1(sum);
-        sum += quad_x2(sum);
-        const float inv = 1.0f / sum;
-#pragma unroll
-        for (int i = 0; i < KQ; ++i) logit[i] *= inv;
-        if (attn_out && active) {
-            float* ar = attn_out + ((((size_t)b * P + p) * g.heads + h) * T + t) * T;
-#pragma unroll
-            for (int i = 0; i < KQ; ++i)
-                if (sq + 4 * i < T) ar[sq + 4 * i] = logit[i];
-        }
-        f32x4 acc[NQ];
-#pragma unroll
-        for (int u = 0; u < NQ; ++u) acc[u] = (f32x4){0.f, 0.f, 0.f, 0.f};
-#pragma unroll
-        for (int i = 0; i < KQ; ++i) {
-            const f32x2 pr = {logit[i], logit[i]};
-#pragma unroll
-            for (int u = 0; u < NQ; ++u) {
-                const f32x4 v4 = ld4(KVimg + kb[u] + RS * 4 + i * ISTRIDE);
-                const f32x4 r4 = ld4(Rimg + rbs[u] + 2 * RS * 4 + i * ISTRIDE);
-                f32x2 lo = acc[u].xy, hi = acc[u].zw;
-                lo = __builtin_elementwise_fma(pr, v4.xy + r4.xy, lo);
-                hi = __builtin_elementwise_fma(pr, v4.zw + r4.zw, hi);
-                acc[u] = (f32x4){lo.x, lo.y, hi.x, hi.y};
-                asm volatile("" : "+v"(acc[u]) : : "memory");
-            }
-            __builtin_amdgcn_sched_barrier(0);
-        }
-#pragma unroll
-        for (int u = 0; u < NQ; ++u) {
-#pragma unroll
-            for (int e = 0; e < 4; ++e) {
-                float v = acc[u][e];
-                v += quad_x1(v);
-                v += quad_x2(v);
-                acc[u][e] = v;
-            }
-        }
-        if (active) {
-            float* orow = o + ((size_t)(b * T + t) * P + p) * C + h * F;
-#pragma unroll
-            for (int u = 0; u < NQ; ++u)
-                if ((u & 3) == sq) st4(orow + 4 * u, acc[u]);
-        }
-    }
+    t2_core<F, TCAP>(Rimg, KVimg, q4, L, mask, o, attn_out, g, b, h, scale);
 }
 
 template <int F, int TCAP>
@@ -412,35 +214,14 @@
     }
 }
 
-inline size_t t2_lds_bytes(int TGN, int NPX, int RS) {
-    return ((size_t)((TGN * 3 * RS + 63) & ~63) + (size_t)((NPX * 2 * RS + 63) & ~63)) * 16;
-}
-
 inline unsigned t2_geometry(T2Geom& g, int F, int RS, size_t& lds) {
-    const int B = g.B, T = g.T, P = g.P, heads = g.heads;
-    int best_tg = (T + 4) / 5, best_nw = 0;
-    {
-        const int TGN = (T + best_tg - 1) / best_tg, PPW = 16 / TGN;
-        for (int NW = 4; NW >= 1 && best_nw == 0; NW /= 2)
-            if (t2_lds_bytes(TGN, NW * PPW, RS) <= 160 * 1024) best_nw = NW;
-        if (best_nw == 0) best_tg = 0;
-    }
-    if (best_tg == 0) return 0;
-    g.TG = best_tg; g.NW = best_nw;
-    g.TGN = (T + g.TG - 1) / g.TG;
-    g.PPW = 16 / g.TGN;
-    const int NPX = g.NW * g.PPW;
-    g.strips = (P + NPX - 1) / NPX;
-    lds = t2_lds_bytes(g.TGN, NPX, RS);
-    g.HL = F >= 32 ? 1 : 32 / F;
-    if (g.HL > heads || heads % g.HL) g.HL = 1;
-    g.NL = B * (heads / g.HL);
-    g.XPG = (g.NL <= 8 && 8 % g.NL == 0) ? 8 / g.NL : 0;
-    if (g.XPG > 0) {
-        const int sblks = (g.strips + g.XPG - 1) / g.XPG;
-        return 8u * (unsigned)(g.HL * g.TG) * (unsigned)sblks;
-    }
-    return (unsigned)(B * heads) * (unsigned)g.TG * (unsigned)g.strips;
+    t2_frames(g);
+    g.NW = 0;
+    for (int NW = 4; NW >= 1 && g.NW == 0; NW /= 2)
+        if (t2_lds_bytes(g.TGN, NW * g.PPW, RS) <= 160 * 1024) g.NW = NW;
+    if (g.NW == 0) return 0;
+    lds = t2_lds_bytes(g.TGN, g.NW * g.PPW, RS);
+    return t2_place(g, F);
 }
 
 template <int F, int TCAP>
@@ -492,7 +273,7 @@
 }
 
 int lfvdm_attn_temporal2_try(const TemporalFwd& a) {
-    if ((long)a.B * a.P * (a.C / a.heads) >= 16384) return LFVDM_E_UNSUPPORTED;
+    if (!t2_small_launch(a.B, a.P, a.C / a.heads)) return LFVDM_E_UNSUPPORTED;
     return launch_t2_f(a);
 }
 
diff --git a/latent-flexible-video-diffusion-modeling_amd/csrc/attention_temporal_fused.hip b/latent-flexible-video-diffusion-modeling_amd/csrc/attention_temporal_fused.hip
--- /dev/null
+++ b/latent-flexible-video-diffusion-modeling_amd/csrc/attention_temporal_fused.hip
@@ -0,0 +1,264 @@
+#include <cstdlib>
+
+#include "attention_temporal.h"
+#include "common_hip.h"
+#include "lfvdm_hip.h"
+
+namespace {
+
+constexpr int TF_UNR = 3;
+constexpr int TF_RTC = 5;
+constexpr int TF_WAVES = 4;
+constexpr long TF_ADOPT_MAX_COLUMNS = 0;
+
+struct TfGeom {
+    int KVf, Qf, Xf;
+};
+
+template <int C_, int F, int TCAP>
+__global__ __launch_bounds__(64 * TF_WAVES, 3)
+void attn_temporal_fused_kernel(const float* __restrict__ x, const float* __restrict__ gamma, const float* __restrict__ beta,
+                                float eps, float* __restrict__ xn_out, const float* __restrict__ W,
+                                const float* __restrict__ bias, const float* __restrict__ Rq, const float* __restrict__ Rk,
+                                const float* __restrict__ Rv, const float* __restrict__ mask, float* __restrict__ o,
+                                RSel rsel, T2Geom g, TfGeom f) {
+    using CF = T2Cfg<F, TCAP>;
+    constexpr int NQ = CF::NQ, RS = CF::RS;
+    constexpr int SPR = C_ / 4, KG = C_ / 16, CG = C_ / 32, NCTH = F / 16;
+    static_assert(CG == 2 || CG == 4, "a statistics slot is eight lanes: 64 or 128 channels");
+    extern __shared__ __attribute__((aligned(16))) float tf_smem[];
+    const int T = g.T, P = g.P;
+    const int tid = threadIdx.x, lane = tid & 63;
+    const int wave = __builtin_amdgcn_readfirstlane(tid >> 6);
+    const int lq = lane & 15, kk = lane >> 4;
+    const int NPX = g.NW * g.PPW;
+    int b, h, tg, strip;
+    t2_decode(g, b, h, tg, strip);
+    if (strip >= g.strips) return;
+    const int tq0 = tg * g.TGN;
+    const int p0 = strip * NPX;
+    const int vpx = min(NPX, P - p0);
+    float* Rimg = tf_smem;
+    float* KVimg = tf_smem + f.KVf;
+    float* Qimg = tf_smem + f.Qf;
+    float* Ximg = tf_smem + f.Xf;
+
+    t2_stage_r<F, TCAP>(x, Rq, Rk, Rv, rsel, g, b, h, tq0, wave, TF_WAVES, lane, Rimg);
+
+    const int rkv = (vpx * T + 15) >> 4, ckv = (rkv + TF_RTC - 1) / TF_RTC;
+    const int rq = (vpx * g.TGN + 15) >> 4, cq = (rq + TF_RTC - 1) / TF_RTC;
+    const int nkv = 2 * NCTH * ckv, njobs = nkv + NCTH * cq;
+    auto job = [&](int jb, int& arr, int& cth, int& rc) {
+        if (jb < nkv) {
+            const int a = jb / ckv;
+            rc = jb - a * ckv;
+            arr = 1 + a / NCTH;
+            cth = a % NCTH;
+        } else {
+            cth = (jb - nkv) / cq;
+            rc = (jb - nkv) - cth * cq;
+            arr = 0;
+        }
+    };
+    auto wrow = [&](int jb) -> const float* {
+        int arr, cth, rc;
+        job(min(jb, njobs - 1), arr, cth, rc);
+        return W + (size_t)(arr * C_ + h * F + 16 * cth + lq) * C_ + 4 * kk;
+    };
+    f32x4 wf[KG];
+    {
+        const float* wr = wrow(wave);
+#pragma unroll
+        for (int k = 0; k < KG; ++k) wf[k] = ld4(wr + 16 * k);
+    }
+    for (int i = tid; i < (f.Qf - f.KVf) / 4; i += 64 * TF_WAVES) st4(KVimg + 4 * i, (f32x4){0.f, 0.f, 0.f, 0.f});
+
+    {
+        const int tp = tid & 7, unit = tid >> 3;
+        const int nslots = vpx * SPR;
+        const float inv = 1.0f / (float)(CG * T);
+        const bool wr_xn = h == 0 && tg == 0 && xn_out != nullptr;
+        for (int s0 = 0; s0 < nslots; s0 += 8 * TF_WAVES * TF_UNR) {
+            f32x4 xk[TF_UNR][TQ_TF], gam[TF_UNR], bet[TF_UNR];
+#pragma unroll
+            for (int sl = 0; sl < TF_UNR; ++sl) {
+                const int s = s0 + 8 * TF_WAVES * sl + unit;
+                const bool ok = s < nslots;
+                const int quad = s % SPR, pix = s / SPR;
+#pragma unroll
+                for (int i = 0; i < TQ_TF; ++i) {
+                    const int t = tp + 8 * i;
+                    xk[sl][i] = (ok && t < T) ? ld4(x + ((size_t)(b * T + t) * P + p0 + pix) * C_ + 4 * quad) : (f32x4){0.f, 0.f, 0.f, 0.f};
+                }
+                gam[sl] = ld4(gamma + 4 * quad);
+                bet[sl] = ld4(beta + 4 * quad);
+            }
+#pragma unroll
+            for (int sl = 0; sl < TF_UNR; ++sl) {
+                const int s = s0 + 8 * TF_WAVES * sl + unit;
+                const bool ok = s < nslots;
+                const int quad = s % SPR, pix = s / SPR;
+                f32x4 mu, rs;
+                tq_stats<CG>(xk[sl], tp, T, inv, eps, mu, rs);
+#pragma unroll
+                for (int i = 0; i < TQ_TF; ++i) {
+                    const int t = tp + 8 * i;
+                    if (ok && t < T) {
+                        const f32x4 v = tq_apply(xk[sl][i], mu, rs, gam[sl], bet[sl]);
+                        st4(Ximg + tq_slot(pix * T + t, quad, SPR), v);
+                        if (wr_xn) st4(xn_out + ((size_t)(b * T + t) * P + p0 + pix) * C_ + 4 * quad, v);
+                    }
+                }
+            }
+        }
+    }
+    __syncthreads();
+
+    for (int jb = wave; jb < njobs; jb += TF_WAVES) {
+        f32x4 wn[KG];
+        const bool more = jb + TF_WAVES < njobs;
+        if (more) {
+            const float* wr = wrow(jb + TF_WAVES);
+#pragma unroll
+            for (int k = 0; k < KG; ++k) wn[k] = ld4(wr + 16 * k);
+        }
+        int arr, cth, rc;
+        job(jb, arr, cth, rc);
+        const int colq = arr * C_ + h * F + 16 * cth + 4 * kk;
+        const f32x4 bv = ld4(bias + colq);
+        int xrow[TF_RTC], dst[TF_RTC];
+#pragma unroll
+        for (int rt = 0; rt < TF_RTC; ++rt) {
+            const int tile = rc * TF_RTC + rt;
+            const int r = 16 * tile + lq;
+            if (arr) {
+                const bool ok = tile < rkv && r < vpx * T;
+                const int jw = r / T, t = r - jw * T;
+                const int c = t * NQ + 4 * cth + kk;
+                xrow[rt] = tile < rkv ? r : 0;
+                dst[rt] = ok ? f.KVf + ((jw * 2 + (arr - 1)) * RS + (c ^ (jw & 15))) * 4 : -1;
+            } else {
+                const int jw = r / g.TGN, tq = r - jw * g.TGN;
+                const bool ok = tile < rq && jw < vpx && tq0 + tq < T;
+                xrow[rt] = ok ? jw * T + tq0 + tq : 0;
+                dst[rt] = ok ? f.Qf + r * F + 16 * cth + 4 * kk : -1;
+            }
+        }
+        f32x4 acc[TF_RTC];
+#pragma unroll
+        for (int rt = 0; rt < TF_RTC; ++rt) acc[rt] = (f32x4){0.f, 0.f, 0.f, 0.f};
+#pragma unroll
+        for (int k = 0; k < KG; ++k) {
+            f32x4 a4[TF_RTC];
+            const int s = 4 * k + kk;
+#pragma unroll
+            for (int rt = 0; rt < TF_RTC; ++rt) a4[rt] = ld4(Ximg + tq_slot(xrow[rt], s, SPR));
+#pragma unroll
+            for (int e = 0; e < 4; ++e)
+#pragma unroll
+                for (int rt = 0; rt < TF_RTC; ++rt) acc[rt] = __builtin_amdgcn_mfma_f32_16x16x4f32(wf[k][e], a4[rt][e], acc[rt], 0, 0, 0);
+        }
+#pragma unroll
+        for (int rt = 0; rt < TF_RTC; ++rt)
+            if (dst[rt] >= 0) st4(tf_smem + dst[rt], acc[rt] + bv);
+        if (more) {
+#pragma unroll
+            for (int k = 0; k < KG; ++k) wf[k] = wn[k];
+        }
+    }
+    asm volatile("s_waitcnt vmcnt(0)" ::: "memory");
+    __syncthreads();
+
+    if (wave < g.NW) {
+        const T2Lane<F, TCAP> L = t2_lane<F, TCAP>(g, wave, lane, tq0, p0);
+        const float scale = rsqrtf((float)F);
+        const float* qrow = Qimg + (L.active ? L.jw * g.TGN + L.tq : 0) * F;
+        f32x4 q4[NQ];
+#pragma unroll
+        for (int u = 0; u < NQ; ++u) q4[u] = ld4(qrow + 4 * u) * scale;
+        t2_core<F, TCAP>(Rimg, KVimg, q4, L, mask, o, nullptr, g, b, h, scale);
+    }
+}
+
+inline int tf_tcap(int T) { return T <= 8 ? 8 : T <= 16 ? 16 : T <= 20 ? 20 : 24; }
+
+unsigned tf_geometry(T2Geom& g, TfGeom& f, size_t& lds) {
+    const int F = g.C / g.heads, RS = (tf_tcap(g.T) * (F / 4) + 15) / 16 * 16;
+    static const int cap = getenv("LFVDM_TF_NW") ? atoi(getenv("LFVDM_TF_NW")) : 0;
+    t2_frames(g);
+    g.NW = 0;
+    for (int NW = TF_WAVES; NW >= 1 && g.NW == 0; NW /= 2) {
+        if (cap > 0 && NW > cap) continue;
+        const int NPX = NW * g.PPW;
+        f.KVf = ((g.TGN * 3 * RS + 63) & ~63) * 4;
+        f.Qf = f.KVf + ((NPX * 2 * RS + 63) & ~63) * 4;
+        f.Xf = f.Qf + ((NPX * g.TGN + 15) & ~15) * F;
+        lds = ((size_t)f.Xf + (size_t)((NPX * g.T + 15) & ~15) * g.C) * 4;
+        if (lds <= 160 * 1024) g.NW = NW;
+    }
+    if (g.NW == 0) return 0;
+    return t2_place(g, F);
+}
+
+int tf_domain(int B, int T, int P, int C, int heads) {
+    if (B <= 0 || T <= 0 || P <= 0 || C <= 0 || heads <= 0 || C % heads) return LFVDM_E_SHAPE;
+    if (C != 64 && C != 128) return LFVDM_E_UNSUPPORTED;
+    const int F = C / heads;
+    if (F != 16 && F != 32) return LFVDM_E_UNSUPPORTED;
+    if (T > 24) return LFVDM_E_UNSUPPORTED;
+    if (lfvdm_gn_temporal_qkv_ok(B, T, P, C) != LFVDM_OK) return LFVDM_E_UNSUPPORTED;
+    if (!t2_small_launch(B, P, F)) return LFVDM_E_UNSUPPORTED;
+    T2Geom g = {T, P, C, heads, B};
+    TfGeom f;
+    size_t lds;
+    return tf_geometry(g, f, lds) ? LFVDM_OK : LFVDM_E_UNSUPPORTED;
+}
+
+template <int C_, int F, int TCAP>
+int launch_tf(const float* x, const float* gamma, const float* beta, float eps, float* xn_out, const float* W, const float* bias,
+              const TemporalFwd& a) {
+    T2Geom g = {a.T, a.P, a.C, a.heads, a.B};
+    TfGeom f;
+    size_t lds;
+    const unsigned grid = tf_geometry(g, f, lds);
+    if (!grid) return LFVDM_E_UNSUPPORTED;
+    static DynLdsLimit limit;
+    if (int rc = limit.ensure(reinterpret_cast<const void*>(&attn_temporal_fused_kernel<C_, F, TCAP>), lds)) return rc;
+    hipLaunchKernelGGL((attn_temporal_fused_kernel<C_, F, TCAP>), dim3(grid), dim3(64 * TF_WAVES), lds, a.s, x, gamma, beta, eps,
+                       xn_out, W, bias, a.Rq, a.Rk, a.Rv, a.mask, a.o, a.rsel, g, f);
+    LFVDM_CHECK_LAUNCH();
+    return LFVDM_OK;
+}
+
+template <int C_, int F, class... Args>
+int launch_tf_t(int T, Args... args) {
+    if (T <= 8) return launch_tf<C_, F, 8>(args...);
+    if (T <= 16) return launch_tf<C_, F, 16>(args...);
+    if (T <= 20) return launch_tf<C_, F, 20>(args...);
+    return launch_tf<C_, F, 24>(args...);
+}
+
+}
+
+extern "C" int lfvdm_attn_temporal_fused_ok(int B, int T, int P, int C, int heads) {
+    if (int rc = tf_domain(B, T, P, C, heads)) return rc;
+    const char* e = getenv("LFVDM_TF_ALWAYS");
+    if (e && e[0] == '1') return LFVDM_OK;
+    const char* c = getenv("LFVDM_TF_COLUMNS");
+    return (long)B * P <= (c ? atol(c) : TF_ADOPT_MAX_COLUMNS) ? LFVDM_OK : LFVDM_E_UNSUPPORTED;
+}
+
+extern "C" int lfvdm_attn_temporal_fused(const float* x, const float* gamma, const float* beta, float eps, float* xn_out,
+                                         const float* Wqkv, const float* bqkv, const float* Rq, const float* Rk, const float* Rv,
+                                         const float* mask, float* o, int B, int T, int P, int C, int heads,
+                                         const int64_t* rsel_p, int ring, void* stream) {
+    if (!x || !gamma || !beta || !Wqkv || !bqkv || !o || x == xn_out) return LFVDM_E_SHAPE;
+    if (!Rq || !Rk || !Rv || ring < 0 || (ring > 0 && !rsel_p)) return LFVDM_E_SHAPE;
+    if (int rc = tf_domain(B, T, P, C, heads)) return rc;
+    const TemporalFwd a = {nullptr, Rq, Rk, Rv, mask, o, nullptr, B, T, P, C, heads, RSel{rsel_p, ring}, (hipStream_t)stream};
+    const int F = C / heads;
+    if (C == 64 && F == 16) return launch_tf_t<64, 16>(T, x, gamma, beta, eps, xn_out, Wqkv, bqkv, a);
+    if (C == 64 && F == 32) return launch_tf_t<64, 32>(T, x, gamma, beta, eps, xn_out, Wqkv, bqkv, a);
+    if (C == 128 && F == 16) return launch_tf_t<128, 16>(T, x, gamma, beta, eps, xn_out, Wqkv, bqkv, a);
+    return launch_tf_t<128, 32>(T, x, gamma, beta, eps, xn_out, Wqkv, bqkv, a);
+}
diff --git a/latent-flexible-video-diffusion-modeling_amd/csrc/gn_temporal_qkv.hip b/latent-flexible-video-diffusion-modeling_amd/csrc/gn_temporal_qkv.hip
--- a/latent-flexible-video-diffusion-modeling_amd/csrc/gn_temporal_qkv.hip
+++ b/latent-flexible-video-diffusion-modeling_amd/csrc/gn_temporal_qkv.hip
@@ -1,11 +1,10 @@
 #include <cstdlib>
 #include <type_traits>
 
+#include "attention_temporal.h"
 #include "common_hip.h"
 
 namespace {
-
-constexpr int TQ_TF = 3;
 
 struct TqGeom {
     int B, T, P;
@@ -22,31 +21,6 @@
     static constexpr int KG = C_ / 16;
     static constexpr int CG = C_ / 32;
 };
-
-__device__ __forceinline__ float tq_dpp_b1(float v) { return __builtin_bit_cast(float, __builtin_amdgcn_mov_dpp(__builtin_bit_cast(int, v), 0xB1, 0xF, 0xF, true)); }
-__device__ __forceinline__ float tq_dpp_4e(float v) { return __builtin_bit_cast(float, __builtin_amdgcn_mov_dpp(__builtin_bit_cast(int, v), 0x4E, 0xF, 0xF, true)); }
-__device__ __forceinline__ float tq_dpp_hm(float v) { return __builtin_bit_cast(float, __builtin_amdgcn_mov_dpp(__builtin_bit_cast(int, v), 0x141, 0xF, 0xF, true)); }
-__device__ __forceinline__ float tq_dpp_r8(float v) { return __builtin_bit_cast(float, __builtin_amdgcn_mov_dpp(__builtin_bit_cast(int, v), 0x128, 0xF, 0xF, true)); }
-
-template <int CG>
-__device__ __forceinline__ float tq_reduce(float v) {
-    v += tq_dpp_b1(v);
-    v += tq_dpp_4e(v);
-    v += tq_dpp_hm(v);
-    if constexpr (CG == 8) v += tq_dpp_r8(v);
-    return v;
-}
-
-template <int CG>
-__device__ __forceinline__ f32x4 tq_group(f32x4 s) {
-    if constexpr (CG == 2) {
-        const float a = tq_reduce<CG>(s.x + s.y), b = tq_reduce<CG>(s.z + s.w);
-        return (f32x4){a, a, b, b};
-    } else {
-        const float a = tq_reduce<CG>((s.x + s.y) + (s.z + s.w));
-        return (f32x4){a, a, a, a};
-    }
-}
 
 template <int C_>
 __global__ __launch_bounds__(256) void gn_temporal_qkv_kernel(const float* __restrict__ x, const float* __restrict__ gamma,
@@ -100,31 +74,15 @@
     for (int sl = 0; sl < NSL; ++sl) {
         const int s = rest + 32 * sl;
         const int quad = s % SPR, pix = s / SPR;
-        f32x4 a = {0.f, 0.f, 0.f, 0.f};
-#pragma unroll
-        for (int i = 0; i < TQ_TF; ++i) a += xk[sl][i];
-        const f32x4 mu = tq_group<CG>(a) * inv;
-        f32x4 q = {0.f, 0.f, 0.f, 0.f};
-#pragma unroll
-        for (int i = 0; i < TQ_TF; ++i) {
-            if (tp + 8 * i < T) {
-                const f32x4 d = xk[sl][i] - mu;
-                q += d * d;
-            }
-        }
-        const f32x4 var = tq_group<CG>(q) * inv;
-        f32x4 rs;
-        rs.x = 1.0f / sqrtf(var.x + eps);
-        rs.z = CG == 2 ? 1.0f / sqrtf(var.z + eps) : rs.x;
-        rs.y = rs.x;
-        rs.w = rs.z;
+        f32x4 mu, rs;
+        tq_stats<CG>(xk[sl], tp, T, inv, eps, mu, rs);
 #pragma unroll
         for (int i = 0; i < TQ_TF; ++i) {
             const int t = tp + 8 * i;
             if (t < T) {
-                const f32x4 v = (xk[sl][i] - mu) * rs * gam[sl] + bet[sl];
+                const f32x4 v = tq_apply(xk[sl][i], mu, rs, gam[sl], bet[sl]);
                 const int row = pix * T + t;
-                st4(As + ((size_t)row * SPR + ((quad & ~15) | ((quad ^ row) & 15))) * 4, v);
+                st4(As + tq_slot(row, quad, SPR), v);
                 if (sp == 0 && xn_out != nullptr) st4(xn_out + ((size_t)(b * T + t) * P + p0 + pix) * C_ + 4 * quad, v);
             }
         }
diff --git a/latent-flexible-video-diffusion-modeling_amd/improved_diffusion/_engine.py b/latent-flexible-video-diffusion-modeling_amd/improved_diffusion/_engine.py
--- a/latent-flexible-video-diffusion-modeling_amd/improved_diffusion/_engine.py
+++ b/latent-flexible-video-diffusion-modeling_amd/improved_diffusion/_engine.py
@@ -32,6 +32,7 @@
 SPATIAL_FUSED = os.environ.get("LFVDM_SPATIAL_FUSED", "1") != "0"
 PROJ_GN = os.environ.get("LFVDM_PROJ_GN", "1") != "0"
 TEMPORAL_QKV = os.environ.get("LFVDM_TEMPORAL_QKV", "1") != "0"
+TEMPORAL_FUSED = os.environ.get("LFVDM_TEMPORAL_FUSED", "1") != "0"
 GN_EPILOGUE = os.environ.get("LFVDM_GN_EPILOGUE", "1") != "0"
 NEXT_GN_EPILOGUE = os.environ.get("LFVDM_NEXT_GN_EPILOGUE", "1") != "0"
 MAX_FRAMES = 64
@@ -529,7 +530,13 @@
         M = N * P
         heads = ab.num_heads
         ta, sa = ab.temporal_attention, ab.spatial_attention
-        if TEMPORAL_QKV and L.lfvdm_gn_temporal_qkv_ok(B, T, P, Cc) == 0:
+        fused_t = bool(TEMPORAL_FUSED and self.time_steps and not self.want_attn
+                       and L.lfvdm_attn_temporal_fused_ok(B, T, P, Cc, heads) == 0)
+        if fused_t:
+            self.add(L.lfvdm_attn_temporal_fused, _p(x), _p(ta.norm.weight), _p(ta.norm.bias), ta.norm.eps, _p(self.s_xn),
+                     _p(ta.qkv.weight), _p(ta.qkv.bias), _p(self.R[ta.rpe_q]), _p(self.R[ta.rpe_k]), _p(self.R[ta.rpe_v]),
+                     _p(self.mask), _p(self.s_o), B, T, P, Cc, heads, _p(self.t_sel), self.time_ring)
+        elif TEMPORAL_QKV and L.lfvdm_gn_temporal_qkv_ok(B, T, P, Cc) == 0:
             self.add(L.lfvdm_gn_temporal_qkv, _p(x), _p(ta.norm.weight), _p(ta.norm.bias), ta.norm.eps, _p(self.s_xn),
                      _p(ta.qkv.weight), _p(ta.qkv.bias), _p(self.s_qkv), B, T, P, Cc)
         else:
@@ -540,7 +547,9 @@
         if self.want_attn:
             at = self.buf(B * P, heads, T, T)
             self.attn_t.append(at)
-        if self.time_steps:
+        if fused_t:
+            pass
+        elif self.time_steps:
             self.add(L.lfvdm_attn_temporal_ring, _p(self.s_qkv), _p(self.R[ta.rpe_q]), _p(self.R[ta.rpe_k]), _p(self.R[ta.rpe_v]),
                      _p(self.mask), _p(self.s_o), _p(at) if at is not None else None, B, T, P, Cc, heads, _p(self.t_sel),
                      self.time_ring)
diff --git a/latent-flexible-video-diffusion-modeling_amd/improved_diffusion/_native.py b/latent-flexible-video-diffusion-modeling_amd/improved_diffusion/_native.py
--- a/latent-flexible-video-diffusion-modeling_amd/improved_diffusion/_native.py
+++ b/latent-flexible-video-diffusion-modeling_amd/improved_diffusion/_native.py
@@ -178,6 +178,8 @@
     "lfvdm_sampler_tick_fetch": ([c_fp, c_fp, c_fp, c_i, c_fp, c_i, c_fp, c_i, c_fp], c_i),
     "lfvdm_attn_temporal_sel": ([c_fp] * 7 + [c_i] * 5 + [c_fp, c_fp], c_i),
     "lfvdm_attn_temporal_ring": ([c_fp] * 7 + [c_i] * 5 + [c_fp, c_i, c_fp], c_i),
+    "lfvdm_attn_temporal_fused_ok": ([c_i] * 5, c_i),
+    "lfvdm_attn_temporal_fused": ([c_fp, c_fp, c_fp, C.c_float, c_fp] + [c_fp] * 7 + [c_i] * 5 + [c_fp, c_i, c_fp], c_i),
     "lfvdm_attn_temporal_bwd": ([c_fp] * 12 + [c_i] * 5 + [c_fp], c_i),
     "lfvdm_attn_spatial_bwd": ([c_fp] * 6 + [c_i, c_i, c_i, c_i, c_fp], c_i),
     "lfvdm_attn_temporal": ([c_fp] * 7 + [c_i] * 5 + [c_fp], c_i),
```
